# kscalelabs/kbot-joystick

Hardware: AMD Instinct MI355X
Metric: env-steps/sec (whole node), K-Bot joystick 8192 envs @1/2/4/8 MI355X (higher is better)
Workload: dtype f32; 1 GPU; kbot-headless, 8192 envs/GPU, flat ground, fixed joystick command (0.5,0,0), full iteration: 100-step rollout + PPO update (batch 512/GPU, 3 passes, LSTM hidden 256, depth 2); envs_per_gpu=8192, rollout_steps=100, batch_size_per_gpu=512, num_passes=3, hidden_size=256, deterministic_update=True, parallelism=env-sharded dp1, grad all-reduce per optimizer step

## Files before the change

kbot-joystick_amd/csrc/kbj_ctx.h:

```cpp
#pragma once
#include <hip/hip_runtime.h>
#include <string>
#include <vector>
#include <cstdio>
#include "kbj.h"

struct KbjKernelRec { int kind; double flops; hipEvent_t a, b; };
enum { KBJ_KIND_GEMM = 0 , KBJ_KIND_SEQ_FWD = 8, KBJ_KIND_SEQ_BWD = 9, KBJ_KIND_ENV_STEP = 10, KBJ_KIND_SEQ_FWD_FUSED = 11, KBJ_KIND_SEQ_FWD_OBS = 12, KBJ_KIND_LSTM_STEP = 13, KBJ_KIND_LSTM_STEP_OBS = 14,
       KBJ_KIND_GEMM_X3 = 15, KBJ_KIND_GEMM_X3_GEN = 19, KBJ_KIND_GEMM_X3_SMALL = 20, KBJ_KIND_GEMM_X3_SMALL_GEN = 21,
       KBJ_KIND_SEQ_BWD16 = 22 , KBJ_KIND_GEMM_64x128 = 23 ,
       KBJ_KIND_COUNT = 25 };
inline int kbj_kind_gemm_x3(int tm, bool a_kc, bool b_kc, bool gen) {
  if (tm == 2) return gen ? KBJ_KIND_GEMM_X3_GEN : KBJ_KIND_GEMM_X3 + (a_kc ? 2 : 0) + (b_kc ? 1 : 0);
  return gen ? KBJ_KIND_GEMM_X3_SMALL_GEN : KBJ_KIND_GEMM_X3_SMALL;
}

struct Sched {
  bool fold_actor = true;
  bool fold_critic = true;
  bool fuse_ih = true;
  bool fuse_obs = true;
  bool fused_critic_head = true;
  bool rollout_step = true;
  bool one_stream = false;
  bool debug_sync = false;
  bool deterministic = false;
  bool bwd16 = true;
  bool critic_on_caller = true;
  bool gemm_x3 = false;
};

struct KbjSettings {
  Sched sched;
  int seq_timeout_ms = 0;
  int seq_drop = 0, seq_drop_bwd = 0;
  bool seq_stamps = false; int stamp_sel = 1;
  bool seq_bstamps = false; int bstamp_sel = 0;
};

KbjSettings kbj_read_settings(const kbj_config& cfg);

struct kbj_ctx {
  int device = 0;
  hipStream_t stream = nullptr;
  hipStream_t stream2 = nullptr;
  hipEvent_t ev_fork = nullptr, ev_join = nullptr;
  hipStream_t side[2] = {nullptr, nullptr};
  hipEvent_t ev_dx[2] = {nullptr, nullptr};
  hipEvent_t ev_side[2] = {nullptr, nullptr};
  hipEvent_t ev_obs = nullptr;
  hipEvent_t ev_prefetch = nullptr;
  hipEvent_t ev_small = nullptr;
  hipEvent_t ev_actor_grad = nullptr;
  hipEvent_t ev_pool[32] = {};
  int ev_next = 0;
  kbj_model model_h;
  kbj_config cfg_h;
  KbjSettings set;
  kbj_model* model_d = nullptr;
  kbj_config* cfg_d = nullptr;
  void* pc_d = nullptr;
  float* mc_d = nullptr;
  float* ep_d = nullptr;
  float* es_d = nullptr;
  float* rcarry_d = nullptr;
  uint32_t seed = 0;
  int rollout_argmax = 0;
  float* qstate_next = nullptr;
  double* epst_part_d = nullptr;
  int epst_part_blocks = 0;
  void* nn_ws = nullptr;
  size_t nn_ws_bytes = 0;
  bool profiling = false;
  hipEvent_t ev0 = nullptr, ev1 = nullptr;
  float env_ms = 0, nn_ms = 0;
  int env_launches = 0, nn_launches = 0;
  std::vector<KbjKernelRec> krecs;
  kbj_kernel_stat kstats[KBJ_KIND_COUNT];
  std::string error;
};

extern thread_local std::string kbj_global_error;

inline int kbj_fail(kbj_ctx* ctx, const std::string& msg) {
  if (ctx) ctx->error = msg;
  kbj_global_error = msg;
  return -1;
}

#define KBJ_HIP(ctx, call)                                                                                   \
  do {                                                                                                       \
    hipError_t e_ = (call);                                                                                  \
    if (e_ != hipSuccess) return kbj_fail(ctx, std::string(#call) + ": " + hipGetErrorString(e_));           \
  } while (0)

#define KBJ_CHECK_LAUNCH(ctx, name)                                                                          \
  do {                                                                                                       \
    hipError_t e_ = hipGetLastError();                                                                       \
    if (e_ != hipSuccess) return kbj_fail(ctx, std::string("launch ") + name + ": " + hipGetErrorString(e_)); \
  } while (0)

extern thread_local kbj_ctx* kbj_prof_ctx;

struct KbjKernelTimer {
  kbj_ctx* c; hipStream_t s; hipEvent_t b = nullptr;
  KbjKernelTimer(hipStream_t st, int kind, double flops) : c(kbj_prof_ctx), s(st) {
    if (!c) return;
    hipEvent_t a;
    if (hipEventCreate(&a) != hipSuccess || hipEventCreate(&b) != hipSuccess) { c = nullptr; return; }
    c->krecs.push_back(KbjKernelRec{kind, flops, a, b});
    hipEventRecord(a, s);
  }
  ~KbjKernelTimer() { if (c) hipEventRecord(b, s); }
};

struct KbjTimed {
  kbj_ctx* ctx; bool nn;
  KbjTimed(kbj_ctx* c, bool is_nn) : ctx(c), nn(is_nn) { if (ctx->profiling) hipEventRecord(ctx->ev0, ctx->stream); }
  ~KbjTimed() {
    if (!ctx->profiling) return;
    hipEventRecord(ctx->ev1, ctx->stream);
    hipEventSynchronize(ctx->ev1);
    float ms = 0; hipEventElapsedTime(&ms, ctx->ev0, ctx->ev1);
    if (nn) { ctx->nn_ms += ms; ctx->nn_launches++; } else { ctx->env_ms += ms; ctx->env_launches++; }
  }
};
```

kbot-joystick_amd/csrc/kbj_lstm_bwd16.h:

```cpp
#pragma once
#include "kbj_lstm_seq.h"

namespace kbj {

constexpr int BWD16_ROWS = 16, BWD16_UNITS = 64, BWD16_NTH = 512;
#ifndef KBJ_BWD16_OWN_SPLIT
#define KBJ_BWD16_OWN_SPLIT 4
#endif

template <int H>
__global__ __launch_bounds__(BWD16_NTH) void lstm_seq_bwd16_kernel(SeqBwdArgs a) {
  static_assert(H % 64 == 0 && H >= 64 && H <= 256, "16 x 64 tiles: hidden sizes 64, 128, 192, 256");
  constexpr int NTH = BWD16_NTH, ROWS = BWD16_ROWS, UNITS = BWD16_UNITS;
  constexpr int NUG = H / UNITS;
  constexpr int KC = 4 * UNITS;
  constexpr int LDC = KC + 8;
  constexpr int KHALF = KC / 2, KS = KHALF / 4;
  typedef SeqK<KHALF> KK;
  __shared__ __attribute__((aligned(16))) float cbuf[2][ROWS * LDC];
  __shared__ float pbuf[2][ROWS][UNITS + 4];
  __shared__ int flag;
  const int tid = threadIdx.x, lane = tid & 63, wave = tid >> 6, nt = wave & 3, kh = wave >> 2;
  const int nblk = gridDim.x;
  const int lid = (nblk % 8 == 0) ? (int)(blockIdx.x % 8) * (nblk / 8) + (int)(blockIdx.x / 8) : (int)blockIdx.x;
  const int ug = lid % NUG, rg = lid / NUG;
  const int r0 = rg * ROWS, u0 = ug * UNITS;
  const int B = a.B, T = a.T;
  if (seq_aborted(a.err, &flag)) return;
  float wreg[NUG][KS];
#pragma unroll
  for (int j = 0; j < NUG; ++j) {
    const int p = (ug + j) % NUG;
#pragma unroll
    for (int s = 0; s < KS; ++s) {
      const int kl = KHALF * kh + KK::kidx(s, lane >> 4);
      wreg[j][s] = a.Whh[(size_t)((kl / UNITS) * H + UNITS * p + (kl % UNITS)) * H + u0 + 16 * nt + (lane & 15)];
    }
  }
  int erow[2], eunit[2];
#pragma unroll
  for (int i = 0; i < 2; ++i) { const int e = tid + NTH * i; erow[i] = e / UNITS; eunit[i] = e % UNITS; }
  float dcm[2] = {0.0f, 0.0f};
  float bsum[2][4] = {{0, 0, 0, 0}, {0, 0, 0, 0}};
  float actn[2][4], tcn[2], cprevn[2], dhan[2], kpn[2];
  int rcl[2];
#pragma unroll
  for (int i = 0; i < 2; ++i) { const int r = r0 + erow[i]; rcl[i] = r < B ? r : 0; }
  auto fetch_inputs = [&](int tt) {
    const int tq = tt < 0 ? 0 : tt;
#pragma unroll
    for (int i = 0; i < 2; ++i) {
      const size_t o1 = ((size_t)tq * B + rcl[i]) * H + u0 + eunit[i];
      const float* g = a.Gact + ((size_t)tq * B + rcl[i]) * 4 * H + u0 + eunit[i];
#pragma unroll
      for (int k = 0; k < 4; ++k) actn[i][k] = g[k * H];
      tcn[i] = a.TanhC[o1];
      cprevn[i] = a.Cm[o1];
      dhan[i] = a.dHabove[o1];
      kpn[i] = a.keep[(size_t)tq * B + rcl[i]];
    }
  };
  fetch_inputs(T - 1);
  struct Chunk { f32x4m v[2]; };
  auto chunk_load = [&](Chunk& c, const float* src, int p) {
    __amdgpu_buffer_rsrc_t rsrc = __builtin_amdgcn_make_buffer_rsrc(const_cast<float*>(src), 0, 0x7FFFFFFF, 0x00020000);
#pragma unroll
    for (int i = 0; i < 2; ++i) {
      const int q = tid + NTH * i, row = q >> 6, seg = q & 63, r = r0 + row;
      const unsigned off = (unsigned)(((size_t)(r < B ? r : 0) * 4 * H + (size_t)(seg >> 4) * H + UNITS * p + 4 * (seg & 15)) * sizeof(float));
      c.v[i] = __builtin_bit_cast(f32x4m, __builtin_amdgcn_raw_buffer_load_b128(rsrc, off, 0, 16));
    }
  };
  auto chunk_to_lds = [&](const Chunk& c, float* buf) {
#pragma unroll
    for (int i = 0; i < 2; ++i) {
      const int q = tid + NTH * i, row = q >> 6, seg = q & 63;
      *reinterpret_cast<f32x4m*>(buf + row * LDC + UNITS * (seg >> 4) + 4 * (seg & 15)) = c.v[i];
    }
  };
  auto mma = [&](const float* buf, const float* w, f32x4m& acc0, f32x4m& acc1, int jb, int je) {
    const float* p0 = buf + (lane & 15) * LDC + KHALF * kh + 4 * (lane >> 4);
#pragma unroll
    for (int j = jb; j < je; ++j) {
      const f32x4m f = *reinterpret_cast<const f32x4m*>(p0 + 16 * j);
      acc0 = __builtin_amdgcn_mfma_f32_16x16x4f32(f[0], w[4 * j + 0], acc0, 0, 0, 0);
      acc1 = __builtin_amdgcn_mfma_f32_16x16x4f32(f[1], w[4 * j + 1], acc1, 0, 0, 0);
      acc0 = __builtin_amdgcn_mfma_f32_16x16x4f32(f[2], w[4 * j + 2], acc0, 0, 0, 0);
      acc1 = __builtin_amdgcn_mfma_f32_16x16x4f32(f[3], w[4 * j + 3], acc1, 0, 0, 0);
    }
  };
  constexpr int OWN_SPLIT = NUG > 1 ? KBJ_BWD16_OWN_SPLIT : KK::NB;
  for (int t = T - 1; t >= 0; --t) {
    float dhm[2] = {0.0f, 0.0f};
    float act[2][4], tc[2], cprev[2], dha[2], kp[2];
    auto prefetch = [&]() {
#pragma unroll
      for (int i = 0; i < 2; ++i) { tc[i] = tcn[i]; cprev[i] = cprevn[i]; dha[i] = dhan[i]; kp[i] = kpn[i]; for (int k = 0; k < 4; ++k) act[i][k] = actn[i][k]; }
      fetch_inputs(t - 1);
    };
    if (t == T - 1) prefetch();
    else {
      f32x4m acc0 = {0, 0, 0, 0}, acc1 = {0, 0, 0, 0};
      mma(cbuf[0], wreg[0], acc0, acc1, 0, OWN_SPLIT);
      Chunk ch[NUG > 1 ? NUG - 1 : 1];
      if (NUG > 1) {
        if (!seq_wait(a.counters + rg * NUG, NUG, (unsigned)(T - 1 - t), a.err, &flag, a.timeout_ticks)) return;
        const float* src = a.dG + (size_t)(t + 1) * B * 4 * H;
#pragma unroll
        for (int j = 1; j < NUG; ++j) chunk_load(ch[j - 1], src, (ug + j) % NUG);
        __builtin_amdgcn_sched_barrier(0);
      }
      mma(cbuf[0], wreg[0], acc0, acc1, OWN_SPLIT, KK::NB);
      if (NUG == 1) prefetch();
#pragma unroll
      for (int j = 1; j < NUG; ++j) {
        float* buf = cbuf[j & 1];
        chunk_to_lds(ch[j - 1], buf);
        if (j == NUG - 1) prefetch();
        __syncthreads();
        mma(buf, wreg[j], acc0, acc1, 0, KK::NB);
      }
#pragma unroll
      for (int r = 0; r < 4; ++r) pbuf[kh][(lane >> 4) * 4 + r][16 * nt + (lane & 15)] = acc0[r] + acc1[r];
      __syncthreads();
#pragma unroll
      for (int i = 0; i < 2; ++i) dhm[i] = pbuf[0][erow[i]][eunit[i]] + pbuf[1][erow[i]][eunit[i]];
    }
#pragma unroll
    for (int i = 0; i < 2; ++i) {
      const int r = r0 + erow[i];
      const float ig = act[i][0], fg = act[i][1], gg = act[i][2], og = act[i][3];
      const float dh = dha[i] + kp[i] * dhm[i];
      const float dc = kp[i] * dcm[i] + dh * og * (1 - tc[i] * tc[i]);
      const float d0 = dc * gg * ig * (1 - ig), d1 = dc * cprev[i] * fg * (1 - fg), d2 = dc * ig * (1 - gg * gg), d3 = dh * tc[i] * og * (1 - og);
      float* own = cbuf[0] + erow[i] * LDC + eunit[i];
      own[0] = d0; own[UNITS] = d1; own[2 * UNITS] = d2; own[3 * UNITS] = d3;
      if (r < B) {
        float* dg = a.dG + ((size_t)t * B + r) * 4 * H + u0 + eunit[i];
        seq_store(dg, d0); seq_store(dg + H, d1); seq_store(dg + 2 * H, d2); seq_store(dg + 3 * H, d3);
        bsum[i][0] += d0; bsum[i][1] += d1; bsum[i][2] += d2; bsum[i][3] += d3;
      }
      dcm[i] = dc * fg;
    }
    seq_publish(a.counters + rg * NUG + ug, (unsigned)(T - t));
  }
  if (a.db || a.db_part) {
    __syncthreads();
#pragma unroll
    for (int i = 0; i < 2; ++i)
#pragma unroll
      for (int k = 0; k < 4; ++k) cbuf[0][erow[i] * LDC + k * UNITS + eunit[i]] = bsum[i][k];
    __syncthreads();
    if (tid < KC) {
      const int k = tid / UNITS, u = tid % UNITS;
      float s = 0;
      for (int r = 0; r < ROWS; ++r) s += cbuf[0][r * LDC + tid];
      if (a.db_part) a.db_part[(size_t)rg * 4 * H + k * H + u0 + u] = s;
      else atomicAdd(a.db + k * H + u0 + u, s);
    }
  }
}

}
```

kbot-joystick_amd/csrc/kbj_lstm_seq.h:

```cpp
#pragma once
#include <hip/hip_runtime.h>
#include <stdint.h>

namespace kbj {

typedef float f32x4m __attribute__((ext_vector_type(4)));

constexpr int SEQ_ROWS = 32;
constexpr int SEQ_UNITS = 16;
#ifdef KBJ_SEQ_BSTAMPS_BUILD
#define SEQ_BSTAMP(k) do { if (a.stamps && blockIdx.x == 0 && tid == 0) a.stamps[t * 10 + (k)] = clock64(); } while (0)
#define SEQ_BSTAMP_ON 1
#else
#define SEQ_BSTAMP(k) do { } while (0)
#define SEQ_BSTAMP_ON 0
#endif
constexpr unsigned SEQ_TIMEOUT_MS = 2000;

#ifndef KBJ_SEQ_BWD_NUM_VGPR
#define KBJ_SEQ_BWD_NUM_VGPR 88
#endif

struct SeqFwdArgs {
  float* G;
  const float* Whh;
  float* Hm;
  float* Cm;
  float* Hout;
  float* TanhC;
  const float* keep;
  unsigned* counters;
  unsigned* err;
  int T, B;
  long long* stamps;
  unsigned timeout_ticks = SEQ_TIMEOUT_MS * 100000u;
  const float* X = nullptr;
  const float* Wih = nullptr;
  const float* bias = nullptr;
  int ldx = 0, ldw = 0;
  int kx = 0;
};

struct SeqBwdArgs {
  const float* Gact;
  const float* TanhC;
  const float* Cm;
  const float* dHabove;
  const float* keep;
  const float* Whh;
  float* dG;
  unsigned* counters;
  unsigned* err;
  int T, B;
  float* db;
  float* db_part = nullptr;
  unsigned timeout_ticks = SEQ_TIMEOUT_MS * 100000u;
  long long* stamps = nullptr;
};

__device__ __forceinline__ float seq_sigmoid(float x) { return __builtin_amdgcn_rcpf(1.0f + __expf(-x)); }
__device__ __forceinline__ float seq_tanh(float x) { float xc = fminf(fmaxf(x, -15.0f), 15.0f); return 1.0f - 2.0f * __builtin_amdgcn_rcpf(1.0f + __expf(2.0f * xc)); }

__device__ __forceinline__ bool seq_wait(unsigned* flags, int nflags, unsigned target, unsigned* err, int* lds_flag, unsigned timeout_ticks) {
#ifdef KBJ_EXPERIMENT_NOWAIT
  __syncthreads();
  return true;
#endif
  if (threadIdx.x < 64) {
    unsigned spins = 0;
    unsigned long long t0 = 0;
    int ok = 1;
    const int l = threadIdx.x;
    for (;;) {
      bool mine = l >= nflags || __hip_atomic_load(flags + l, __ATOMIC_RELAXED, __HIP_MEMORY_SCOPE_AGENT) >= target;
      if (__all(mine)) break;
      __builtin_amdgcn_s_sleep(1);
      if ((++spins & 255u) == 0) {
        const unsigned long long now = wall_clock64();
        if (t0 == 0) t0 = now;
        const bool aborted = __hip_atomic_load(err, __ATOMIC_RELAXED, __HIP_MEMORY_SCOPE_AGENT) != 0;
        if (aborted || now - t0 > timeout_ticks) { ok = 0; if (l == 0) __hip_atomic_store(err, 1u, __ATOMIC_RELAXED, __HIP_MEMORY_SCOPE_AGENT); break; }
      }
    }
    if (l == 0) *lds_flag = ok;
  }
  __syncthreads();
  __builtin_amdgcn_fence(__ATOMIC_ACQUIRE, "wavefront");
  return *lds_flag != 0;
}
__device__ __forceinline__ bool seq_aborted(unsigned* err, int* lds_flag) {
  if (threadIdx.x == 0) *lds_flag = __hip_atomic_load(err, __ATOMIC_RELAXED, __HIP_MEMORY_SCOPE_AGENT) != 0;
  __syncthreads();
  const bool r = *lds_flag != 0;
  __syncthreads();
  return r;
}
__device__ __forceinline__ void seq_store(float* p, float v) { __hip_atomic_store(p, v, __ATOMIC_RELAXED, __HIP_MEMORY_SCOPE_AGENT); }
__device__ __forceinline__ void seq_publish(unsigned* my_flag, unsigned steps_done) {
#ifndef KBJ_EXPERIMENT_NODRAIN
  asm volatile("s_waitcnt vmcnt(0)" ::: "memory");
#endif
  __syncthreads();
  if (threadIdx.x == 0) __hip_atomic_store(my_flag, steps_done, __ATOMIC_RELAXED, __HIP_MEMORY_SCOPE_AGENT);
}
template <int K> struct SeqK {
  static_assert(K % 4 == 0, "row width must be a multiple of 4");
  static constexpr int NB = K / 16, REM = (K % 16) / 4, STEPS = 4 * NB + REM;
  static constexpr int LD = (K + 7) / 16 * 16 + 8;
  __host__ __device__ static constexpr int kidx(int s, int g) { return s < 4 * NB ? 16 * (s / 4) + 4 * g + (s % 4) : 16 * NB + 4 * (s - 4 * NB) + g; }
  template <bool TAIL>
  __device__ static __forceinline__ void mma(const float* lds, int lane, const float* w, f32x4m& acc0, f32x4m& acc1, int jb, int je) {
    const float* p0 = lds + (lane & 15) * LD + 4 * (lane >> 4);
    const float* p1 = p0 + 16 * LD;
#pragma unroll
    for (int j = jb; j < je; ++j) {
      const f32x4m a0 = *reinterpret_cast<const f32x4m*>(p0 + 16 * j), a1 = *reinterpret_cast<const f32x4m*>(p1 + 16 * j);
#pragma unroll
      for (int q = 0; q < 4; ++q) {
        acc0 = __builtin_amdgcn_mfma_f32_16x16x4f32(a0[q], w[4 * j + q], acc0, 0, 0, 0);
        acc1 = __builtin_amdgcn_mfma_f32_16x16x4f32(a1[q], w[4 * j + q], acc1, 0, 0, 0);
      }
    }
    if (TAIL) {
      const float* r0 = lds + (lane & 15) * LD + 16 * NB + (lane >> 4);
      const float* r1 = r0 + 16 * LD;
#pragma unroll
      for (int q = 0; q < REM; ++q) {
        acc0 = __builtin_amdgcn_mfma_f32_16x16x4f32(r0[4 * q], w[4 * NB + q], acc0, 0, 0, 0);
        acc1 = __builtin_amdgcn_mfma_f32_16x16x4f32(r1[4 * q], w[4 * NB + q], acc1, 0, 0, 0);
      }
    }
  }
};

template <int H, int NTH> struct SeqTile {
  static constexpr int NQ = SEQ_ROWS * (H / 4);
  static constexpr int NV = (NQ + NTH - 1) / NTH;
  static constexpr bool EXACT = NQ % NTH == 0;
  f32x4m v[NV];
  __device__ __forceinline__ void load(const float* src, int ld, int r0, int B) {
    typedef unsigned u32x4 __attribute__((ext_vector_type(4)));
    __amdgpu_buffer_rsrc_t rsrc = __builtin_amdgcn_make_buffer_rsrc(const_cast<float*>(src), 0, 0x7FFFFFFF, 0x00020000);
#pragma unroll
    for (int i = 0; i < NV; ++i) {
      int q = threadIdx.x + NTH * i, row = q / (H / 4), c4 = q % (H / 4), r = r0 + row;
      unsigned off = (unsigned)(((size_t)(r < B ? r : 0) * ld + 4 * c4) * sizeof(float));
      u32x4 u = __builtin_amdgcn_raw_buffer_load_b128(rsrc, off, 0, 16);
      v[i] = __builtin_bit_cast(f32x4m, u);
    }
  }
  __device__ __forceinline__ void load_plain(const float* src, int ld, int r0, int B) {
#pragma unroll
    for (int i = 0; i < NV; ++i) {
      int q = threadIdx.x + NTH * i;
      if (!EXACT && q >= NQ) q = 0;
      int row = q / (H / 4), c4 = q % (H / 4), r = r0 + row;
      v[i] = *reinterpret_cast<const f32x4m*>(src + (size_t)(r < B ? r : 0) * ld + 4 * c4);
    }
  }
  __device__ __forceinline__ void to_lds(float* lds, int r0, int B) const {
    if (r0 + SEQ_ROWS <= B) {
#pragma unroll
      for (int i = 0; i < NV; ++i) {
        int q = threadIdx.x + NTH * i, row = q / (H / 4), c4 = q % (H / 4);
        if (!EXACT && q >= NQ) continue;
        *reinterpret_cast<f32x4m*>(lds + row * SeqK<H>::LD + 4 * c4) = v[i];
      }
      return;
    }
#pragma unroll
    for (int i = 0; i < NV; ++i) {
      int q = threadIdx.x + NTH * i, row = q / (H / 4), c4 = q % (H / 4);
      if (!EXACT && q >= NQ) continue;
      *reinterpret_cast<f32x4m*>(lds + row * SeqK<H>::LD + 4 * c4) = r0 + row < B ? v[i] : f32x4m{0, 0, 0, 0};
    }
  }
  __device__ __forceinline__ void to_lds_cols(float* lds, int ldl, int r0, int B, int ncol) const {
#pragma unroll
    for (int i = 0; i < NV; ++i) {
      int q = threadIdx.x + NTH * i, row = q / (H / 4), c4 = q % (H / 4);
      if (!EXACT && q >= NQ) continue;
      f32x4m x = v[i];
#pragma unroll
      for (int j = 0; j < 4; ++j) if (r0 + row >= B || 4 * c4 + j >= ncol) x[j] = 0.0f;
      *reinterpret_cast<f32x4m*>(lds + row * ldl + 4 * c4) = x;
    }
  }
};

template <int H, int UW, bool FUSE = false, int KX = H>
__global__ __launch_bounds__(256 * UW) void lstm_seq_fwd_kernel(SeqFwdArgs a) {
  constexpr int NTH = 256 * UW, UNITS = SEQ_UNITS * UW;
  typedef SeqK<H> KH;
  typedef SeqK<KX> KXK;
  constexpr int LDH = KH::LD, KXS = KXK::STEPS, LDX = KXK::LD;
  constexpr int NUG = H / UNITS;
#ifndef KBJ_SEQ_XSPLIT_NUM
#define KBJ_SEQ_XSPLIT_NUM 4
#endif
  constexpr int XSPLIT = KXK::NB * KBJ_SEQ_XSPLIT_NUM / 8;
  __shared__ __attribute__((aligned(16))) float hs[SEQ_ROWS * LDH];
  __shared__ __attribute__((aligned(16))) float xs[FUSE ? SEQ_ROWS * LDX : 4];
  __shared__ float gbuf[4][SEQ_ROWS][UNITS + 4];
  __shared__ int flag;
  const int tid = threadIdx.x, lane = tid & 63, gate = (tid >> 6) & 3, uh = tid >> 8;
  const int nblk = gridDim.x;
  const int lid = (nblk % 8 == 0) ? (int)(blockIdx.x % 8) * (nblk / 8) + (int)(blockIdx.x / 8) : (int)blockIdx.x;
  const int ug = lid % NUG, rg = lid / NUG;
  const int r0 = rg * SEQ_ROWS, u0 = ug * UNITS;
  const int B = a.B, T = a.T;
  if (seq_aborted(a.err, &flag)) return;
  float wreg[H / 4];
  {
    const float* wrow = a.Whh + (size_t)(gate * H + u0 + SEQ_UNITS * uh + (lane & 15)) * H;
#pragma unroll
    for (int s = 0; s < H / 4; ++s) wreg[s] = wrow[KH::kidx(s, lane >> 4)];
  }
  float wxreg[FUSE ? KXS : 1];
  float bias_col = 0.0f;
  const int ldx = a.ldx ? a.ldx : H, kxv = a.kx ? a.kx : KX;
  if (FUSE) {
    const int grow = gate * H + u0 + SEQ_UNITS * uh + (lane & 15);
    const float* wrow = a.Wih + (size_t)grow * (a.ldw ? a.ldw : H);
#pragma unroll
    for (int s = 0; s < KXS; ++s) { const int k = KXK::kidx(s, lane >> 4); wxreg[s] = k < kxv ? wrow[k] : 0.0f; }
    bias_col = a.bias[grow];
  }
  int erow[2], eunit[2];
  float cm[2];
#pragma unroll
  for (int i = 0; i < 2; ++i) {
    int e = tid + NTH * i;
    erow[i] = e / UNITS; eunit[i] = e % UNITS;
    int r = r0 + erow[i];
    cm[i] = r < B ? a.Cm[(size_t)r * H + u0 + eunit[i]] : 0.0f;
  }
  float ig[2], fg[2], gg[2], og[2], tc[2], hh[2];
#ifdef KBJ_SEQ_BSTAMPS_BUILD
#define SEQ_STAMP(k) do { if (a.stamps && blockIdx.x == 0 && tid == 0) a.stamps[t * 6 + (k)] = clock64(); } while (0)
#else
#define SEQ_STAMP(k) do { } while (0)
#endif
  float gxn[2][4], kpn[2];
  int rcl[2];
#pragma unroll
  for (int i = 0; i < 2; ++i) { const int r = r0 + erow[i]; rcl[i] = r < B ? r : 0; }
  auto fetch_inputs = [&](int tt) {
    const int tq = tt < T ? tt : T - 1;
#pragma unroll
    for (int i = 0; i < 2; ++i) {
      if (!FUSE) {
        const float* g = a.G + ((size_t)tq * B + rcl[i]) * 4 * H + u0 + eunit[i];
#pragma unroll
        for (int k = 0; k < 4; ++k) gxn[i][k] = g[k * H];
      } else {
#pragma unroll
        for (int k = 0; k < 4; ++k) gxn[i][k] = 0.0f;
      }
      kpn[i] = a.keep[(size_t)tq * B + rcl[i]];
    }
  };
  fetch_inputs(0);
  if (FUSE) {
    SeqTile<KX, NTH> xt;
    xt.load_plain(a.X, ldx, r0, B);
    if (KX == H) xt.to_lds(xs, r0, B); else xt.to_lds_cols(xs, LDX, r0, B, kxv);
    __syncthreads();
  }
  for (int t = 0; t < T; ++t) {
    SEQ_STAMP(0);
    float gx[2][4], kp[2];
#pragma unroll
    for (int i = 0; i < 2; ++i) { kp[i] = kpn[i]; for (int k = 0; k < 4; ++k) gx[i][k] = gxn[i][k]; }
    f32x4m acc0 = {bias_col, bias_col, bias_col, bias_col}, acc1 = acc0;
    if (FUSE) {
      KXK::template mma<false>(xs, lane, wxreg, acc0, acc1, 0, XSPLIT);
    }
    if (t > 0) { if (!seq_wait(a.counters + rg * NUG, NUG, (unsigned)t, a.err, &flag, a.timeout_ticks)) return; }
    SEQ_STAMP(1);
    SeqTile<H, NTH> tile;
    tile.load(a.Hm + (size_t)t * B * H, H, r0, B);
    if (FUSE) {
      __builtin_amdgcn_sched_barrier(0);
      KXK::template mma<true>(xs, lane, wxreg, acc0, acc1, XSPLIT, KXK::NB);
      __builtin_amdgcn_sched_barrier(0);
    }
    tile.to_lds(hs, r0, B);
    fetch_inputs(t + 1);
    if (t > 0) {
#pragma unroll
      for (int i = 0; i < 2; ++i) {
        int r = r0 + erow[i];
        if (r >= B) continue;
        size_t o1 = ((size_t)(t - 1) * B + r) * H + u0 + eunit[i];
        float* g = a.G + ((size_t)(t - 1) * B + r) * 4 * H + u0 + eunit[i];
        g[0] = ig[i]; g[H] = fg[i]; g[2 * H] = gg[i]; g[3 * H] = og[i];
        a.Hout[o1] = hh[i]; a.TanhC[o1] = tc[i];
        a.Cm[o1 + (size_t)B * H] = cm[i];
      }
    }
    SeqTile<KX, NTH> xt;
    if (FUSE && t + 1 < T) xt.load_plain(a.X + (size_t)(t + 1) * B * ldx, ldx, r0, B);
    __syncthreads();
    SEQ_STAMP(2);
    KH::template mma<false>(hs, lane, wreg, acc0, acc1, 0, KH::NB);
#pragma unroll
    for (int r = 0; r < 4; ++r) {
      gbuf[gate][(lane >> 4) * 4 + r][SEQ_UNITS * uh + (lane & 15)] = acc0[r];
      gbuf[gate][16 + (lane >> 4) * 4 + r][SEQ_UNITS * uh + (lane & 15)] = acc1[r];
    }
    if (FUSE && t + 1 < T) { if (KX == H) xt.to_lds(xs, r0, B); else xt.to_lds_cols(xs, LDX, r0, B, kxv); }
    __syncthreads();
    SEQ_STAMP(3);
#pragma unroll
    for (int i = 0; i < 2; ++i) {
      int row = erow[i], u = eunit[i];
      ig[i] = seq_sigmoid(gbuf[0][row][u] + gx[i][0]); fg[i] = seq_sigmoid(gbuf[1][row][u] + gx[i][1]);
      gg[i] = seq_tanh(gbuf[2][row][u] + gx[i][2]); og[i] = seq_sigmoid(gbuf[3][row][u] + gx[i][3]);
      float c = fg[i] * cm[i] + ig[i] * gg[i];
      tc[i] = seq_tanh(c); hh[i] = og[i] * tc[i];
      cm[i] = c * kp[i];
      if (r0 + row < B) seq_store(a.Hm + ((size_t)(t + 1) * B + r0 + row) * H + u0 + u, hh[i] * kp[i]);
    }
    SEQ_STAMP(4);
    seq_publish(a.counters + rg * NUG + ug, (unsigned)(t + 1));
    SEQ_STAMP(5);
  }
#pragma unroll
  for (int i = 0; i < 2; ++i) {
    int r = r0 + erow[i];
    if (r >= B) continue;
    size_t o1 = ((size_t)(T - 1) * B + r) * H + u0 + eunit[i];
    float* g = a.G + ((size_t)(T - 1) * B + r) * 4 * H + u0 + eunit[i];
    g[0] = ig[i]; g[H] = fg[i]; g[2 * H] = gg[i]; g[3 * H] = og[i];
    a.Hout[o1] = hh[i]; a.TanhC[o1] = tc[i];
    a.Cm[o1 + (size_t)B * H] = cm[i];
  }
}

template <int H, int UW>
__device__ __forceinline__ void lstm_seq_bwd_body(const SeqBwdArgs a) {
  constexpr int NTH = 256 * UW, UNITS = SEQ_UNITS * UW;
  typedef SeqK<H> KH;
  constexpr int LDH = KH::LD;
  constexpr int NUG = H / UNITS;
  __shared__ __attribute__((aligned(16))) float ds[SEQ_ROWS * LDH];
  __shared__ float pbuf[4][SEQ_ROWS][UNITS + 4];
  __shared__ int flag;
  const int tid = threadIdx.x, lane = tid & 63, wave = (tid >> 6) & 3, uh = tid >> 8;
  const int nblk = gridDim.x;
  const int lid = (nblk % 8 == 0) ? (int)(blockIdx.x % 8) * (nblk / 8) + (int)(blockIdx.x / 8) : (int)blockIdx.x;
  const int ug = lid % NUG, rg = lid / NUG;
  const int r0 = rg * SEQ_ROWS, u0 = ug * UNITS;
  const int B = a.B, T = a.T;
  if (seq_aborted(a.err, &flag)) return;
  if (SEQ_BSTAMP_ON && a.stamps && tid == 0 && blockIdx.x < 256) a.stamps[T * 10 + 3 * blockIdx.x] = wall_clock64();
  constexpr int KW = H / 4;
  constexpr int KS = KW / 4;
  typedef SeqK<KW> KWK;
  static_assert(KW % 16 == 0, "the backward recurrence fetches its fragments in 16-k blocks");
  float wreg[4][KS];
#pragma unroll
  for (int c = 0; c < 4; ++c)
#pragma unroll
    for (int s = 0; s < KS; ++s) wreg[c][s] = a.Whh[(size_t)(c * H + wave * KW + KWK::kidx(s, lane >> 4)) * H + u0 + SEQ_UNITS * uh + (lane & 15)];
  int erow[2], eunit[2];
  float dcm[2] = {0.0f, 0.0f};
  float bsum[2][4] = {{0, 0, 0, 0}, {0, 0, 0, 0}};
#pragma unroll
  for (int i = 0; i < 2; ++i) { int e = tid + NTH * i; erow[i] = e / UNITS; eunit[i] = e % UNITS; }
  float actn[2][4], tcn[2], cprevn[2], dhan[2], kpn[2];
  auto fetch_inputs = [&](int tt) {
#pragma unroll
    for (int i = 0; i < 2; ++i) {
      int r = r0 + erow[i];
      bool ok = r < B && tt >= 0;
      size_t o1 = ((size_t)(ok ? tt : 0) * B + (ok ? r : 0)) * H + u0 + eunit[i];
      const float* g = a.Gact + ((size_t)(ok ? tt : 0) * B + (ok ? r : 0)) * 4 * H + u0 + eunit[i];
#pragma unroll
      for (int k = 0; k < 4; ++k) actn[i][k] = ok ? g[k * H] : 0.0f;
      tcn[i] = ok ? a.TanhC[o1] : 0.0f;
      cprevn[i] = ok ? a.Cm[o1] : 0.0f;
      dhan[i] = ok ? a.dHabove[o1] : 0.0f;
      kpn[i] = ok ? a.keep[(size_t)tt * B + r] : 0.0f;
    }
  };
  fetch_inputs(T - 1);
  if (SEQ_BSTAMP_ON && a.stamps && tid == 0 && blockIdx.x < 256) a.stamps[T * 10 + 3 * blockIdx.x + 1] = wall_clock64();
  for (int t = T - 1; t >= 0; --t) {
    const bool last = t == T - 1;
    SEQ_BSTAMP(0);
    if (SEQ_BSTAMP_ON && a.stamps && blockIdx.x == 0 && tid == 0) a.stamps[t * 10 + 9] = wall_clock64();
    float dhm[2] = {0.0f, 0.0f};
    float act[2][4], tc[2], cprev[2], dha[2], kp[2];
    auto prefetch = [&]() {
#pragma unroll
      for (int i = 0; i < 2; ++i) { tc[i] = tcn[i]; cprev[i] = cprevn[i]; dha[i] = dhan[i]; kp[i] = kpn[i]; for (int k = 0; k < 4; ++k) act[i][k] = actn[i][k]; }
      fetch_inputs(t - 1);
    };
    if (last) prefetch();
    else {
      if (!seq_wait(a.counters + rg * NUG, NUG, (unsigned)(T - 1 - t), a.err, &flag, a.timeout_ticks)) return;
      SEQ_BSTAMP(1);
      f32x4m acc0 = {0, 0, 0, 0}, acc1 = {0, 0, 0, 0};
      const float* src = a.dG + (size_t)(t + 1) * B * 4 * H;
      SeqTile<H, NTH> tile;
      tile.load(src, 4 * H, r0, B);
#pragma unroll
      for (int c = 0; c < 4; ++c) {
        float* buf = ds;
        if (c) __syncthreads();
        tile.to_lds(buf, r0, B);
        if (c < 3) tile.load(src + (c + 1) * H, 4 * H, r0, B);
        else prefetch();
        __syncthreads();
        SEQ_BSTAMP(2 + c);
        const float* a0p = buf + (lane & 15) * LDH + wave * KW + 4 * (lane >> 4);
        const float* a1p = a0p + 16 * LDH;
#pragma unroll
        for (int j = 0; j < KW / 16; ++j) {
          const f32x4m f0 = *reinterpret_cast<const f32x4m*>(a0p + 16 * j), f1 = *reinterpret_cast<const f32x4m*>(a1p + 16 * j);
#pragma unroll
          for (int q = 0; q < 4; ++q) {
            acc0 = __builtin_amdgcn_mfma_f32_16x16x4f32(f0[q], wreg[c][4 * j + q], acc0, 0, 0, 0);
            acc1 = __builtin_amdgcn_mfma_f32_16x16x4f32(f1[q], wreg[c][4 * j + q], acc1, 0, 0, 0);
          }
        }
      }
#pragma unroll
      for (int r = 0; r < 4; ++r) {
        pbuf[wave][(lane >> 4) * 4 + r][SEQ_UNITS * uh + (lane & 15)] = acc0[r];
        pbuf[wave][16 + (lane >> 4) * 4 + r][SEQ_UNITS * uh + (lane & 15)] = acc1[r];
      }
      __syncthreads();
      SEQ_BSTAMP(6);
#pragma unroll
      for (int i = 0; i < 2; ++i) dhm[i] = pbuf[0][erow[i]][eunit[i]] + pbuf[1][erow[i]][eunit[i]] + pbuf[2][erow[i]][eunit[i]] + pbuf[3][erow[i]][eunit[i]];
    }
#pragma unroll
    for (int i = 0; i < 2; ++i) {
      int r = r0 + erow[i];
      if (r >= B) continue;
      float ig = act[i][0], fg = act[i][1], gg = act[i][2], og = act[i][3];
      float dh = dha[i] + kp[i] * dhm[i];
      float dc = kp[i] * dcm[i] + dh * og * (1 - tc[i] * tc[i]);
      float* dg = a.dG + ((size_t)t * B + r) * 4 * H + u0 + eunit[i];
      float d0 = dc * gg * ig * (1 - ig), d1 = dc * cprev[i] * fg * (1 - fg), d2 = dc * ig * (1 - gg * gg), d3 = dh * tc[i] * og * (1 - og);
      seq_store(dg, d0);
      seq_store(dg + H, d1);
      seq_store(dg + 2 * H, d2);
      seq_store(dg + 3 * H, d3);
      bsum[i][0] += d0; bsum[i][1] += d1; bsum[i][2] += d2; bsum[i][3] += d3;
      dcm[i] = dc * fg;
    }
    SEQ_BSTAMP(7);
    seq_publish(a.counters + rg * NUG + ug, (unsigned)(T - t));
    SEQ_BSTAMP(8);
  }
  if (a.db || a.db_part) {
    __syncthreads();
#pragma unroll
    for (int k = 0; k < 4; ++k) {
      pbuf[k][erow[0]][eunit[0]] = bsum[0][k];
      pbuf[k][erow[1]][eunit[1]] = bsum[1][k];
    }
    __syncthreads();
    if (tid < 4 * UNITS) {
      int k = tid / UNITS, u = tid % UNITS;
      float s = 0;
      for (int r = 0; r < SEQ_ROWS; ++r) s += pbuf[k][r][u];
      if (a.db_part) a.db_part[(size_t)rg * 4 * H + k * H + u0 + u] = s;
      else atomicAdd(a.db + k * H + u0 + u, s);
    }
  }
  if (SEQ_BSTAMP_ON && a.stamps && tid == 0 && blockIdx.x < 256) a.stamps[T * 10 + 3 * blockIdx.x + 2] = wall_clock64();
}
template <int H, int UW>
__global__ __launch_bounds__(256 * UW) __attribute__((amdgpu_num_vgpr(KBJ_SEQ_BWD_NUM_VGPR))) void lstm_seq_bwd_kernel(SeqBwdArgs a) { lstm_seq_bwd_body<H, UW>(a); }
template <int H, int UW>
__global__ __launch_bounds__(256 * UW) void lstm_seq_bwd_wide_kernel(SeqBwdArgs a) { lstm_seq_bwd_body<H, UW>(a); }

struct StepArgs {
  const float* X; int ldx, kx;
  const float* Wih; int ldw;
  const float* Whh;
  const float* bias;
  const float* Hin;
  float* Hout;
  float* C;
  int M;
};
template <int H, int UW, int KX = H>
__global__ __launch_bounds__(256 * UW) void lstm_step_kernel(StepArgs a) {
  constexpr int NTH = 256 * UW, UNITS = SEQ_UNITS * UW;
  typedef SeqK<H> KH;
  typedef SeqK<KX> KXK;
  constexpr int LDH = KH::LD, KXS = KXK::STEPS, LDX = KXK::LD, NUG = H / UNITS;
  __shared__ __attribute__((aligned(16))) float hs[SEQ_ROWS * LDH];
  __shared__ __attribute__((aligned(16))) float xs[SEQ_ROWS * LDX];
  __shared__ float gbuf[4][SEQ_ROWS][UNITS + 4];
  const int tid = threadIdx.x, lane = tid & 63, gate = (tid >> 6) & 3, uh = tid >> 8;
  const int ug = blockIdx.x % NUG, chunk = blockIdx.x / NUG, nchunk = gridDim.x / NUG;
  const int u0 = ug * UNITS, M = a.M, nrg = (M + SEQ_ROWS - 1) / SEQ_ROWS;
  const int kxv = a.kx ? a.kx : KX;
  const int grow = gate * H + u0 + SEQ_UNITS * uh + (lane & 15);
  float wreg[H / 4], wxreg[KXS];
  {
    const float* wrow = a.Whh + (size_t)grow * H + 4 * (lane >> 4);
#pragma unroll
    for (int j = 0; j < KH::NB; ++j) {
      const f32x4m q = *reinterpret_cast<const f32x4m*>(wrow + 16 * j);
#pragma unroll
      for (int e = 0; e < 4; ++e) wreg[4 * j + e] = q[e];
    }
    const float* xrow = a.Wih + (size_t)grow * a.ldw;
    if (a.kx == 0 && (a.ldw & 3) == 0) {
#pragma unroll
      for (int j = 0; j < KXK::NB; ++j) {
        const f32x4m q = *reinterpret_cast<const f32x4m*>(xrow + 4 * (lane >> 4) + 16 * j);
#pragma unroll
        for (int e = 0; e < 4; ++e) wxreg[4 * j + e] = q[e];
      }
#pragma unroll
      for (int s = 4 * KXK::NB; s < KXS; ++s) wxreg[s] = xrow[KXK::kidx(s, lane >> 4)];
    } else {
#pragma unroll
      for (int s = 0; s < KXS; ++s) { const int k = KXK::kidx(s, lane >> 4); wxreg[s] = k < kxv ? xrow[k] : 0.0f; }
    }
  }
  const float bias_col = a.bias[grow];
  int erow[2], eunit[2];
#pragma unroll
  for (int i = 0; i < 2; ++i) { int e = tid + NTH * i; erow[i] = e / UNITS; eunit[i] = e % UNITS; }
  SeqTile<KX, NTH> xt;
  SeqTile<H, NTH> ht;
  float cn[2] = {0.0f, 0.0f};
  auto fetch = [&](int rg) {
    const int r0 = rg * SEQ_ROWS;
    xt.load_plain(a.X, a.ldx, r0, M);
    ht.load_plain(a.Hin, H, r0, M);
#pragma unroll
    for (int i = 0; i < 2; ++i) { int r = r0 + erow[i]; cn[i] = r < M ? a.C[(size_t)r * H + u0 + eunit[i]] : 0.0f; }
  };
  int rg = chunk;
  if (rg < nrg) fetch(rg);
  for (; rg < nrg; rg += nchunk) {
    const int r0 = rg * SEQ_ROWS;
    if (KX == H) xt.to_lds(xs, r0, M); else xt.to_lds_cols(xs, LDX, r0, M, kxv);
    ht.to_lds(hs, r0, M);
    const float cp[2] = {cn[0], cn[1]};
    __syncthreads();
    if (rg + nchunk < nrg) fetch(rg + nchunk);
    f32x4m acc0 = {bias_col, bias_col, bias_col, bias_col}, acc1 = acc0;
    KXK::template mma<true>(xs, lane, wxreg, acc0, acc1, 0, KXK::NB);
    KH::template mma<false>(hs, lane, wreg, acc0, acc1, 0, KH::NB);
#pragma unroll
    for (int r = 0; r < 4; ++r) {
      gbuf[gate][(lane >> 4) * 4 + r][SEQ_UNITS * uh + (lane & 15)] = acc0[r];
      gbuf[gate][16 + (lane >> 4) * 4 + r][SEQ_UNITS * uh + (lane & 15)] = acc1[r];
    }
    __syncthreads();
#pragma unroll
    for (int i = 0; i < 2; ++i) {
      const int row = erow[i], u = eunit[i], r = r0 + row;
      float ig = seq_sigmoid(gbuf[0][row][u]), fg = seq_sigmoid(gbuf[1][row][u]), gg = seq_tanh(gbuf[2][row][u]), og = seq_sigmoid(gbuf[3][row][u]);
      float c = fg * cp[i] + ig * gg;
      if (r < M) { a.Hout[(size_t)r * H + u0 + u] = og * seq_tanh(c); a.C[(size_t)r * H + u0 + u] = c; }
    }
  }
}

}
```

kbot-joystick_amd/csrc/kbj_nn.hip:

```cpp
#include <hip/hip_runtime.h>
#include <vector>
#include <cmath>
#include <cstdlib>
#include <algorithm>
#include <type_traits>
#include "kbj_ctx.h"
#include "kbj_gemm.h"
#include "kbj_nn_kernels.h"
#include "kbj_lstm_seq.h"
#include "kbj_lstm_bwd16.h"

using namespace kbj;

namespace {

constexpr int MAXD = KBJ_MAX_DEPTH;

struct NetOff {
  size_t w_in, b_in, w_ih[MAXD], w_hh[MAXD], b[MAXD], w_out, b_out;
  int nin, nout, ld_obs;
};

struct TrainBufs {
  float *obs, *X0, *G[MAXD], *Hm[MAXD], *Hout[MAXD], *Cm[MAXD], *TanhC[MAXD], *Out, *dOut, *dHa, *dHb, *dGl[MAXD];
};

struct ParamLayout {
  NetOff net[2];
  size_t nparams = 0, nactor = 0;
  int D = 2;
};

struct NnWs : ParamLayout {
  Sched& sched;
  explicit NnWs(Sched& s) : sched(s) {}
  int H = 0, N = 0, B = 0, T = 0;
  int Hu = 0;
  ParamLayout user;
  PadDesc* pad_desc = nullptr; int npad = 0;
  float *pparams = nullptr, *pgrad = nullptr;
  float *phc[4] = {nullptr, nullptr, nullptr, nullptr}, *pc0[4] = {nullptr, nullptr, nullptr, nullptr};
  bool padded() const { return Hu != H; }
  float* skws[4] = {nullptr, nullptr, nullptr, nullptr};
  size_t skws_cap[4] = {0, 0, 0, 0};
  float* detp[4] = {nullptr, nullptr, nullptr, nullptr};
  double* detd = nullptr;
  float *rX[4] = {nullptr, nullptr, nullptr, nullptr}, *rG[4] = {nullptr, nullptr, nullptr, nullptr}, *rOut[4] = {nullptr, nullptr, nullptr, nullptr};
  float* joint_bias_d = nullptr;
  bool mirror = false;
  int nnets = 2;
  MirrorEntry* mtab[2] = {nullptr, nullptr};
  float *rObsM[2] = {nullptr, nullptr};
  float* rH[4][MAXD] = {};
  float* tail_hc = nullptr;
  float *y_m = nullptr, *sd_m = nullptr, *value_m = nullptr, *lpf0_m = nullptr, *dy = nullptr, *dy_m = nullptr, *dvalue_m = nullptr, *zeroR = nullptr;
  TrainBufs tb[4];
  float *keep = nullptr, *act = nullptr, *logp_old = nullptr, *val_old = nullptr, *adv = nullptr, *target = nullptr;
  float *y = nullptr, *sd = nullptr, *logp = nullptr, *ent = nullptr, *value = nullptr, *dlogp = nullptr, *dvalue = nullptr, *lpf0 = nullptr;
  float *Weff = nullptr, *beff = nullptr, *Zeff[4] = {nullptr, nullptr, nullptr, nullptr};
  float* WinP[2] = {nullptr, nullptr};
  double* stats = nullptr;
  const int32_t* prefetched_idx = nullptr;
  const kbj_traj* prefetched_traj = nullptr;
  const double* ext_adv_sums = nullptr;
  unsigned* seq_counters = nullptr;
  unsigned* seq_err = nullptr;
  unsigned seq_timeout_ticks = 0;
  bool counters_clean = false;
  bool sumsq_clean = false;
  int seq_grid = 0, seq_slots = 0;
  long long* seq_stamps = nullptr;
  long long* seq_bstamps = nullptr;
  std::vector<void*> allocs;
};

NnWs* ws_of(kbj_ctx* ctx) { return reinterpret_cast<NnWs*>(ctx->nn_ws); }

ParamLayout layout_params(const kbj_config& c, int H) {
  ParamLayout p;
  const int D = p.D = c.depth;
  size_t off = 0;
  for (int n = 0; n < 2; ++n) {
    NetOff& o = p.net[n];
    o.nin = n == 0 ? KBJ_NOBS_ACTOR + c.extra_obs_actor : KBJ_NOBS_CRITIC + c.extra_obs_critic;
    o.ld_obs = KBJ_LD_OF(o.nin);
    o.nout = n == 0 ? 2 * KBJ_NU : 1;
    o.w_in = off; off += (size_t)H * o.nin;
    o.b_in = off; off += H;
    for (int l = 0; l < D; ++l) {
      o.w_ih[l] = off; off += (size_t)4 * H * H;
      o.w_hh[l] = off; off += (size_t)4 * H * H;
      o.b[l] = off; off += (size_t)4 * H;
    }
    o.w_out = off; off += (size_t)o.nout * H;
    o.b_out = off; off += o.nout;
    if (n == 0) p.nactor = off;
  }
  p.nparams = off;
  return p;
}

template <class C> auto& carry_hc(C& c, int n) { return n == 0 ? c.actor_hc_d : n == 1 ? c.critic_hc_d : n == 2 ? c.actor_mirror_hc_d : c.critic_mirror_hc_d; }
template <class T> auto& traj_carry0(T& t, int n) { return n == 0 ? t.carry0_actor_hc_d : n == 1 ? t.carry0_critic_hc_d : n == 2 ? t.carry0_actor_mirror_hc_d : t.carry0_critic_mirror_hc_d; }

void build_mirror_tables(const kbj_model& m, std::vector<MirrorEntry>& ta, std::vector<MirrorEntry>& tc, int extra_actor = 0, int extra_critic = 0) {
  auto swp = [](int i) { return i < 5 ? i + 5 : (i < 10 ? i - 5 : i); };
  tc.assign(KBJ_LD_CRITIC, MirrorEntry{0, 0.0f, 0.0f});
  for (int k = 0; k < KBJ_LD_CRITIC; ++k) tc[k].src = k;
  auto keep = [&](int k, float sgn) { tc[k] = MirrorEntry{k, sgn, 0.0f}; };
  for (int i = 0; i < KBJ_NU; ++i) {
    int s = swp(i);
    auto rng = [&](int j) { return std::fmax(m.joint_bias[j] - m.joint_lo[j], m.joint_hi[j] - m.joint_bias[j]); };
    tc[KBJ_OBS_JPOS + i] = MirrorEntry{KBJ_OBS_JPOS + s, -rng(s) / rng(i), (-m.joint_bias[s] - m.joint_bias[i]) / rng(i)};
    tc[KBJ_OBS_JVEL + i] = MirrorEntry{KBJ_OBS_JVEL + s, -1.0f, 0.0f};
    tc[KBJ_OBS_ACTFRC + i] = MirrorEntry{KBJ_OBS_ACTFRC + s, -1.0f, 0.0f};
  }
  keep(KBJ_OBS_PG, -1); keep(KBJ_OBS_PG + 1, 1); keep(KBJ_OBS_PG + 2, 1); keep(KBJ_OBS_PG + 3, -1); keep(KBJ_OBS_PG + 4, 1);
  keep(KBJ_OBS_GYRO, -1); keep(KBJ_OBS_GYRO + 1, 1); keep(KBJ_OBS_GYRO + 2, -1);
  keep(KBJ_OBS_ZEROCMD, 1);
  const float cs[16] = {1, -1, -1, 1, -1, 1, -1, -1, -1, -1, -1, -1, -1, -1, -1, -1};
  for (int k = 0; k < 16; ++k) keep(KBJ_OBS_CMD + k, cs[k]);
  ta.assign(tc.begin(), tc.begin() + KBJ_LD_ACTOR);
  for (int k = KBJ_NOBS_ACTOR; k < KBJ_LD_ACTOR; ++k) ta[k] = MirrorEntry{k, 0.0f, 0.0f};
  tc[KBJ_OBS_TOUCH] = MirrorEntry{KBJ_OBS_TOUCH + 1, 1, 0}; tc[KBJ_OBS_TOUCH + 1] = MirrorEntry{KBJ_OBS_TOUCH, 1, 0};
  const float fs[3] = {1, -1, 1};
  for (int k = 0; k < 3; ++k) { tc[KBJ_OBS_FEETPOS + k] = MirrorEntry{KBJ_OBS_FEETPOS + 3 + k, fs[k], 0}; tc[KBJ_OBS_FEETPOS + 3 + k] = MirrorEntry{KBJ_OBS_FEETPOS + k, fs[k], 0}; }
  keep(KBJ_OBS_BASEPOS, 1); keep(KBJ_OBS_BASEPOS + 1, 1); keep(KBJ_OBS_BASEPOS + 2, 1);
  keep(KBJ_OBS_BASEQUAT, 1); keep(KBJ_OBS_BASEQUAT + 1, -1); keep(KBJ_OBS_BASEQUAT + 2, -1); keep(KBJ_OBS_BASEQUAT + 3, 1);
  const float ci[10] = {1, 1, -1, 1, 1, 1, 1, -1, 1, -1}, cv[6] = {1, -1, 1, -1, 1, -1};
  for (int b = 0; b < 23; ++b) {
    for (int k = 0; k < 10; ++k) keep(KBJ_OBS_CINERT + 10 * b + k, ci[k]);
    for (int k = 0; k < 6; ++k) keep(KBJ_OBS_CVEL + 6 * b + k, cv[k]);
  }
  keep(KBJ_OBS_LINVEL, 1); keep(KBJ_OBS_LINVEL + 1, -1); keep(KBJ_OBS_LINVEL + 2, 1);
  keep(KBJ_OBS_ANGVEL, -1); keep(KBJ_OBS_ANGVEL + 1, 1); keep(KBJ_OBS_ANGVEL + 2, -1);
  keep(KBJ_OBS_HEIGHT, 1);
  for (int k = KBJ_NOBS_CRITIC; k < KBJ_LD_CRITIC; ++k) tc[k] = MirrorEntry{k, 0.0f, 0.0f};
  auto widen = [](std::vector<MirrorEntry>& t, int nobs, int extra) {
    t.resize(KBJ_LD_OF(nobs + extra));
    for (int k = nobs; k < (int)t.size(); ++k) t[k] = MirrorEntry{k, k < nobs + extra ? 1.0f : 0.0f, 0.0f};
  };
  if (extra_actor > 0) widen(ta, KBJ_NOBS_ACTOR, extra_actor);
  if (extra_critic > 0) widen(tc, KBJ_NOBS_CRITIC, extra_critic);
}

template <class T> int dalloc(kbj_ctx* ctx, NnWs& w, T** p, size_t count) {
  void* q = nullptr;
  hipError_t e = hipMalloc(&q, count * sizeof(T));
  if (e != hipSuccess) return kbj_fail(ctx, std::string("hipMalloc (nn workspace): ") + hipGetErrorString(e));
  w.allocs.push_back(q);
  *p = reinterpret_cast<T*>(q);
  return 0;
}

constexpr int g_fold_sk = 8;
#ifndef KBJ_SPLITK_WGS
#define KBJ_SPLITK_WGS 768
#endif
constexpr int g_splitk_wgs = KBJ_SPLITK_WGS;
constexpr int DETP_ROWS = 512, DETP_COLS = 4 * 512;

int lane_of(kbj_ctx* ctx, hipStream_t s) { return s == ctx->stream ? 0 : (s == ctx->stream2 ? 1 : (s == ctx->side[0] ? 2 : 3)); }
float* sk_workspace(kbj_ctx* ctx, hipStream_t s, size_t floats) {
  NnWs& w = *ws_of(ctx);
  if (!w.sched.deterministic) return nullptr;
  const int l = lane_of(ctx, s);
  if (w.skws_cap[l] < floats) {
    hipDeviceSynchronize();
    if (w.skws[l]) hipFree(w.skws[l]);
    w.skws[l] = nullptr; w.skws_cap[l] = 0;
    void* q = nullptr;
    if (hipMalloc(&q, floats * sizeof(float)) != hipSuccess) { kbj_fail(ctx, "hipMalloc (deterministic split-K workspace)"); return nullptr; }
    w.skws[l] = reinterpret_cast<float*>(q); w.skws_cap[l] = floats;
  }
  return w.skws[l];
}
float* det_partials(kbj_ctx* ctx, hipStream_t s) {
  NnWs& w = *ws_of(ctx);
  return w.sched.deterministic ? w.detp[lane_of(ctx, s)] : nullptr;
}

inline dim3 g1(size_t n, int bs = 256) { return dim3((unsigned)((n + bs - 1) / bs)); }

void linear_fwd(hipStream_t s, const float* x, int lda, const float* W, int ldw, const float* bias, float* y, int ldy, int M, int N, int K, int beta) {
  GemmArgs g{x, W, y, bias, M, N, K, lda, ldw, ldy, beta, 1, nullptr};
  gemm_launch<true, true>(s, g);
}
void linear_bwd_input(hipStream_t s, bool x3, const float* dy, int lddy, const float* W, int ldw, float* dx, int lddx, int M, int N, int K, int beta, int tile = -1) {
  GemmArgs g{dy, W, dx, nullptr, M, N, K, lddy, ldw, lddx, beta, 1, nullptr};
  g.x3 = x3;
  gemm_launch<true, false>(s, g, x3 ? -1 : tile);
}
void linear_bwd_weight(kbj_ctx* ctx, hipStream_t s, bool x3, const float* dy, int lddy, const float* x, int ldx, float* dW, int lddw, int Nout, int Nin, int R) {
  bool big = Nout >= 128 && Nin >= 128;
  int ts = big ? 128 : 64;
  int tiles = ((Nout + ts - 1) / ts) * ((Nin + ts - 1) / ts);
  int sk = std::max(2, std::min(256, g_splitk_wgs / std::max(1, tiles)));
  sk = std::max(2, std::min(sk, (R + 255) / 256));
  GemmArgs g{dy, x, dW, nullptr, Nout, Nin, R, lddy, ldx, lddw, 1, sk, nullptr};
  g.skws = sk_workspace(ctx, s, (size_t)sk * Nout * Nin);
  g.x3 = x3;
  gemm_launch<false, false>(s, g, big ? 1 : 0);
}

void linear_bwd_weight2(kbj_ctx* ctx, hipStream_t s, bool x3, const float* dy, int lddy, const float* x1, const float* x2, int ldx, float* dW1, float* dW2, int lddw, int Nout, int Nin, int R) {
  bool big = Nout >= 128 && Nin >= 128;
  int ts = big ? 128 : 64;
  if (Nin % ts != 0) {
    linear_bwd_weight(ctx, s, x3, dy, lddy, x1, ldx, dW1, lddw, Nout, Nin, R);
    linear_bwd_weight(ctx, s, x3, dy, lddy, x2, ldx, dW2, lddw, Nout, Nin, R);
    return;
  }
  int tiles = ((Nout + ts - 1) / ts) * (2 * Nin / ts);
  int sk = std::max(2, std::min(256, g_splitk_wgs / std::max(1, tiles)));
  sk = std::max(2, std::min(sk, (R + 255) / 256));
  GemmArgs g{dy, x1, dW1, nullptr, Nout, 2 * Nin, R, lddy, ldx, lddw, 1, sk, nullptr};
  g.B2 = x2; g.C2 = dW2; g.n1 = Nin;
  g.skws = sk_workspace(ctx, s, (size_t)sk * Nout * 2 * Nin);
  g.x3 = x3;
  gemm_launch<false, false>(s, g, big ? 1 : 0);
}
void colsum_acc(kbj_ctx* ctx, hipStream_t s, const float* X, int M, int N, int ld, float* out) {
  float* part = det_partials(ctx, s);
  hipLaunchKernelGGL(colsum_kernel, dim3((N + 63) / 64, DETP_ROWS), dim3(256), 0, s, X, M, N, ld, out, part);
  if (part) reduce_rows_launch(s, part, DETP_ROWS, N, out);
}

constexpr int SEQ_UW = 2;
constexpr int SEQ_FUSED_MAX_H = 256;
constexpr int SEQ_MAX_H = 512;
constexpr int SEQ_COUNTER_WORDS = 256;
constexpr int SEQ_COUNTER_TOTAL = 2 * MAXD * 4 * SEQ_COUNTER_WORDS;

template <int HC = 64, class F> bool dispatch_hidden(int H, F&& f) {
  if constexpr (HC > SEQ_MAX_H) return false;
  else return H == HC ? f(std::integral_constant<int, HC>()) : dispatch_hidden<HC + 64>(H, f);
}

int seq_fwd(kbj_ctx* ctx, hipStream_t st, int H, const SeqFwdArgs& a0) {
  SeqFwdArgs a = a0;
  a.timeout_ticks = ws_of(ctx)->seq_timeout_ticks;
  KbjKernelTimer timer(st, a.X ? (a.ldx == KBJ_LD_ACTOR ? KBJ_KIND_SEQ_FWD_OBS : KBJ_KIND_SEQ_FWD_FUSED) : KBJ_KIND_SEQ_FWD, 2.0 * a.T * a.B * 4.0 * H * (H + (a.X ? (a.kx ? a.kx : H) : 0)));
  const bool built = dispatch_hidden(H, [&](auto hc) {
    constexpr int HC = decltype(hc)::value, UW = SEQ_UW;
    int grid = (HC / (SEQ_UNITS * UW)) * ((a.B + SEQ_ROWS - 1) / SEQ_ROWS);
    if (ctx->set.seq_drop > 0 && grid > 1) { --ctx->set.seq_drop; --grid; }
    const dim3 block(256 * UW);
    if constexpr (HC <= SEQ_FUSED_MAX_H) {
      if (a.X && a.ldx == KBJ_LD_ACTOR) { hipLaunchKernelGGL((lstm_seq_fwd_kernel<HC, UW, true, KBJ_LD_ACTOR>), dim3(grid), block, 0, st, a); return true; }
      if (a.X) { hipLaunchKernelGGL((lstm_seq_fwd_kernel<HC, UW, true>), dim3(grid), block, 0, st, a); return true; }
    }
    hipLaunchKernelGGL((lstm_seq_fwd_kernel<HC, UW, false>), dim3(grid), block, 0, st, a);
    return true;
  });
  return built ? 0 : kbj_fail(ctx, "seq_fwd: the persistent LSTM kernels are built for hidden sizes 64, 128, ..., 512");
}
int seq_bwd_row_groups(int B, bool tiles16) { return tiles16 ? (B + BWD16_ROWS - 1) / BWD16_ROWS : (B + SEQ_ROWS - 1) / SEQ_ROWS; }
int seq_bwd(kbj_ctx* ctx, hipStream_t st, int H, const SeqBwdArgs& a0, bool tiles16 = false) {
  SeqBwdArgs a = a0;
  a.timeout_ticks = ws_of(ctx)->seq_timeout_ticks;
  KbjKernelTimer timer(st, tiles16 ? KBJ_KIND_SEQ_BWD16 : KBJ_KIND_SEQ_BWD, 2.0 * a.T * a.B * 4.0 * H * H);
  const bool built = dispatch_hidden(H, [&](auto hc) {
    constexpr int HC = decltype(hc)::value, UW = SEQ_UW;
    if (tiles16) {
      if constexpr (HC <= SEQ_FUSED_MAX_H) {
        int grid = (HC / BWD16_UNITS) * ((a.B + BWD16_ROWS - 1) / BWD16_ROWS);
        if (ctx->set.seq_drop_bwd > 0 && grid > 1 && HC > BWD16_UNITS) { --ctx->set.seq_drop_bwd; --grid; }
        hipLaunchKernelGGL((lstm_seq_bwd16_kernel<HC>), dim3(grid), dim3(BWD16_NTH), 0, st, a);
        return true;
      } else return false;
    }
    const dim3 grid((HC / (SEQ_UNITS * UW)) * ((a.B + SEQ_ROWS - 1) / SEQ_ROWS)), block(256 * UW);
    if constexpr (HC <= SEQ_FUSED_MAX_H) hipLaunchKernelGGL((lstm_seq_bwd_kernel<HC, UW>), grid, block, 0, st, a);
    else hipLaunchKernelGGL((lstm_seq_bwd_wide_kernel<HC, UW>), grid, block, 0, st, a);
    return true;
  });
  return built ? 0 : kbj_fail(ctx, "seq_bwd: the persistent LSTM kernels are built for hidden sizes 64, 128, ..., 512 (lstm_seq_bwd16_kernel: up to 256)");
}

template <int H> hipError_t seq_min_blocks_per_cu(int* out) {
  constexpr int threads = 256 * SEQ_UW;
  int n[4] = {0, 0, 0, 0};
  hipError_t e = hipOccupancyMaxActiveBlocksPerMultiprocessor(&n[2], lstm_seq_fwd_kernel<H, SEQ_UW, false, H>, threads, 0);
  if constexpr (H <= SEQ_FUSED_MAX_H) {
    if (e == hipSuccess) e = hipOccupancyMaxActiveBlocksPerMultiprocessor(&n[0], lstm_seq_fwd_kernel<H, SEQ_UW, true, H>, threads, 0);
    if (e == hipSuccess) e = hipOccupancyMaxActiveBlocksPerMultiprocessor(&n[1], lstm_seq_fwd_kernel<H, SEQ_UW, true, KBJ_LD_ACTOR>, threads, 0);
    if (e == hipSuccess) e = hipOccupancyMaxActiveBlocksPerMultiprocessor(&n[3], lstm_seq_bwd_kernel<H, SEQ_UW>, threads, 0);
    int n16 = 0;
    if (e == hipSuccess) e = hipOccupancyMaxActiveBlocksPerMultiprocessor(&n16, lstm_seq_bwd16_kernel<H>, BWD16_NTH, 0);
    n[3] = std::min(n[3], n16);
  } else {
    if (e == hipSuccess) e = hipOccupancyMaxActiveBlocksPerMultiprocessor(&n[3], lstm_seq_bwd_wide_kernel<H, SEQ_UW>, threads, 0);
    n[0] = n[1] = n[2];
  }
  *out = std::min(std::min(n[0], n[1]), std::min(n[2], n[3]));
  return e;
}

int lstm_step(kbj_ctx* ctx, hipStream_t st, int H, const StepArgs& a) {
  const bool obs = a.ldx == KBJ_LD_ACTOR && a.ldw == KBJ_LD_ACTOR;
  KbjKernelTimer timer(st, obs ? KBJ_KIND_LSTM_STEP_OBS : KBJ_KIND_LSTM_STEP, 2.0 * a.M * 4.0 * H * (H + (a.kx ? a.kx : H)));
  const int nug = H / (SEQ_UNITS * 2), nrg = (a.M + SEQ_ROWS - 1) / SEQ_ROWS;
  const int nch = std::max(1, std::min(nrg, 256 / nug));
  dim3 grid(nug * nch), block(512);
  const bool built = dispatch_hidden(H, [&](auto hc) {
    constexpr int HC = decltype(hc)::value;
    if constexpr (HC <= SEQ_FUSED_MAX_H) {
      if (obs) hipLaunchKernelGGL((lstm_step_kernel<HC, 2, KBJ_LD_ACTOR>), grid, block, 0, st, a);
      else hipLaunchKernelGGL((lstm_step_kernel<HC, 2>), grid, block, 0, st, a);
      return true;
    } else return false;
  });
  return built ? 0 : kbj_fail(ctx, "lstm_step: the LSTM step kernels are built for hidden_size 64, 128, 192, 256");
}

}

int kbj_nn_check_errors(kbj_ctx* ctx) {
  NnWs* w = ws_of(ctx);
  if (!w) return 0;
  if (w->seq_stamps) {
    std::vector<long long> st((size_t)w->T * 6);
    if (hipMemcpy(st.data(), w->seq_stamps, st.size() * sizeof(long long), hipMemcpyDeviceToHost) == hipSuccess && w->T > 2) {
      double d[6] = {0, 0, 0, 0, 0, 0};
      for (int t = 1; t < w->T - 1; ++t) { for (int k = 0; k < 5; ++k) d[k] += (double)(st[t * 6 + k + 1] - st[t * 6 + k]); d[5] += (double)(st[(t + 1) * 6] - st[t * 6 + 5]); }
      fprintf(stderr, "[kbj seq_fwd stamps, cycles/step] prefetch+wait %.0f stage %.0f mfma %.0f cell %.0f publish %.0f bulk-store %.0f\n",
              d[0] / (w->T - 2), d[1] / (w->T - 2), d[2] / (w->T - 2), d[3] / (w->T - 2), d[4] / (w->T - 2), d[5] / (w->T - 2));
    }
  }
  if (w->seq_bstamps) {
    std::vector<long long> st((size_t)w->T * 10 + 768);
    if (hipMemcpy(st.data(), w->seq_bstamps, st.size() * sizeof(long long), hipMemcpyDeviceToHost) == hipSuccess && w->T > 3) {
      double d[9] = {0, 0, 0, 0, 0, 0, 0, 0, 0};
      int cnt = 0;
      for (int t = w->T - 3; t >= 1; --t, ++cnt) { for (int k = 0; k < 8; ++k) d[k] += (double)(st[t * 10 + k + 1] - st[t * 10 + k]); d[8] += (double)(st[(t - 1) * 10] - st[t * 10 + 8]); }
      fprintf(stderr, "[kbj seq_bwd stamps, cycles/step] wait %.0f chunk0-staged %.0f chunk1 %.0f chunk2 %.0f chunk3 %.0f last-mfma+reduce %.0f cell %.0f publish %.0f loop %.0f\n",
              d[0] / cnt, d[1] / cnt, d[2] / cnt, d[3] / cnt, d[4] / cnt, d[5] / cnt, d[6] / cnt, d[7] / cnt, d[8] / cnt);
      double ticks = (double)(st[1 * 10] - st[(w->T - 3) * 10]), wall = (double)(st[1 * 10 + 9] - st[(w->T - 3) * 10 + 9]);
      int wall_khz = 0;
      hipDeviceGetAttribute(&wall_khz, hipDeviceAttributeWallClockRate, ctx->device);
      if (wall_khz > 0) {
        const long long* g = st.data() + (size_t)w->T * 10;
        int nwg = ((w->B + SEQ_ROWS - 1) / SEQ_ROWS) * (w->H / (SEQ_UNITS * SEQ_UW));
        if (nwg > 256) nwg = 256;
        long long e0 = g[0], e1 = g[0], l1 = g[1], x0 = g[2], x1 = g[2];
        for (int i = 1; i < nwg; ++i) { e0 = std::min(e0, g[3 * i]); e1 = std::max(e1, g[3 * i]); l1 = std::max(l1, g[3 * i + 1]); x0 = std::min(x0, g[3 * i + 2]); x1 = std::max(x1, g[3 * i + 2]); }
        const double us = 1e3 / wall_khz;
        fprintf(stderr, "[kbj seq_bwd stamps] %d workgroups: last entry +%.1f us, last loop start +%.1f us, first exit +%.1f us, last exit +%.1f us (from the first entry)\n", nwg,
                (e1 - e0) * us, (l1 - e0) * us, (x0 - e0) * us, (x1 - e0) * us);
      }
      if (wall > 0 && wall_khz > 0) fprintf(stderr, "[kbj seq_bwd stamps] %.2f us/step, stamp counter at %.0f MHz\n", wall / wall_khz * 1e3 / cnt, ticks / wall * wall_khz * 1e-3);
    }
  }
  unsigned e[2] = {0, 0};
  if (hipMemcpy(e, w->seq_err, sizeof(e), hipMemcpyDeviceToHost) != hipSuccess) return kbj_fail(ctx, "hipMemcpy seq_err");
  if (e[0] || e[1]) {
    hipMemset(w->seq_err, 0, sizeof(e));
    if (e[0]) return kbj_fail(ctx, "persistent LSTM kernel: inter-workgroup wait timed out (grid not fully resident?); the optimizer steps fed by it were skipped");
    return kbj_fail(ctx, "non-finite gradient norm: the optimizer step was skipped (parameters and moments unchanged)");
  }
  return 0;
}

void kbj_nn_drop_prefetch(kbj_ctx* ctx) {
  NnWs* w = ws_of(ctx);
  if (!w || !w->prefetched_idx) return;
  hipStreamWaitEvent(ctx->stream, ctx->ev_prefetch, 0);
  w->prefetched_idx = nullptr; w->prefetched_traj = nullptr;
}

KbjSettings kbj_read_settings(const kbj_config& c) {
  auto flag = [](const char* name, bool dflt) { const char* v = getenv(name); return v ? atoi(v) != 0 : dflt; };
  auto number = [](const char* name, int dflt) { const char* v = getenv(name); return v ? atoi(v) : dflt; };
  KbjSettings set;
  Sched& sc = set.sched;
  const bool wide = c.hidden_size > SEQ_FUSED_MAX_H;
  sc.fold_actor = flag("KBJ_FOLD_ACTOR", true); sc.fold_critic = flag("KBJ_FOLD_CRITIC", true);
  sc.fuse_ih = flag("KBJ_SEQ_FUSE", true); sc.fuse_obs = sc.fuse_ih && flag("KBJ_SEQ_FUSE_OBS", true);
  sc.fused_critic_head = flag("KBJ_FUSED_CRITIC_HEAD", true); sc.rollout_step = flag("KBJ_ROLLOUT_STEP", true);
  sc.one_stream = flag("KBJ_ONE_STREAM", false); sc.debug_sync = flag("KBJ_DEBUG", false);
  sc.deterministic = c.deterministic != 0 || flag("KBJ_DETERMINISTIC", false);
  { const char* cl = getenv("KBJ_CRITIC_LANE"); sc.critic_on_caller = !(cl && std::string(cl) == "2nd"); }
  sc.bwd16 = flag("KBJ_BWD16", true) && !wide;
  sc.gemm_x3 = (c.gemm_bf16x3 != 0 || flag("KBJ_GEMM_X3", false)) && !sc.deterministic;
  if (wide) sc.fuse_ih = sc.fuse_obs = sc.rollout_step = false;
  set.seq_drop = number("KBJ_DEBUG_DROP_SEQ_WG", 0);
  set.seq_drop_bwd = number("KBJ_DEBUG_DROP_SEQ_BWD_WG", 0);
  set.seq_timeout_ms = (set.seq_drop > 0 || set.seq_drop_bwd > 0) ? 20 : (int)SEQ_TIMEOUT_MS;
  if (getenv("KBJ_SEQ_TIMEOUT_MS")) set.seq_timeout_ms = std::max(1, std::min(30000, number("KBJ_SEQ_TIMEOUT_MS", 0)));
  set.seq_stamps = getenv("KBJ_SEQ_STAMPS") != nullptr; set.stamp_sel = number("KBJ_SEQ_STAMPS", 1);
  set.seq_bstamps = getenv("KBJ_SEQ_BSTAMPS") != nullptr; set.bstamp_sel = number("KBJ_SEQ_BSTAMPS", 0);
  return set;
}

namespace {

int nn_layouts(kbj_ctx* ctx, NnWs* w) {
  const kbj_config& c = ctx->cfg_h;
  w->Hu = c.hidden_size; w->H = (c.hidden_size + 63) / 64 * 64; w->N = c.num_envs; w->B = c.batch_size; w->T = c.rollout_len;
  if (w->B <= 0 || w->B > w->N) return kbj_fail(ctx, "kbj_create: batch_size must be in [1, num_envs]");
  static_cast<ParamLayout&>(*w) = layout_params(c, w->H);
  w->user = layout_params(c, w->Hu);
  w->mirror = c.actor_mirror_loss_scale != 0.0f || c.critic_mirror_loss_scale != 0.0f;
  w->nnets = w->mirror ? 4 : 2;
  return 0;
}

int nn_padding(kbj_ctx* ctx, NnWs* w) {
  if (!w->padded()) return 0;
  std::vector<PadDesc> pd;
  const int Hu = w->Hu, Hi = w->H;
  for (int n = 0; n < 2; ++n) {
    const NetOff &a = w->user.net[n], &b = w->net[n];
    pd.push_back(PadDesc{a.w_in, b.w_in, 1, Hu, Hi, a.nin, a.nin});
    pd.push_back(PadDesc{a.b_in, b.b_in, 1, Hu, Hi, 1, 1});
    for (int l = 0; l < w->D; ++l) {
      pd.push_back(PadDesc{a.w_ih[l], b.w_ih[l], 4, Hu, Hi, Hu, Hi});
      pd.push_back(PadDesc{a.w_hh[l], b.w_hh[l], 4, Hu, Hi, Hu, Hi});
      pd.push_back(PadDesc{a.b[l], b.b[l], 4, Hu, Hi, 1, 1});
    }
    pd.push_back(PadDesc{a.w_out, b.w_out, 1, a.nout, a.nout, Hu, Hi});
    pd.push_back(PadDesc{a.b_out, b.b_out, 1, a.nout, a.nout, 1, 1});
  }
  w->npad = (int)pd.size();
  if (dalloc(ctx, *w, &w->pad_desc, pd.size())) return -1;
  if (hipMemcpy(w->pad_desc, pd.data(), pd.size() * sizeof(PadDesc), hipMemcpyHostToDevice) != hipSuccess) return kbj_fail(ctx, "hipMemcpy pad descriptors");
  if (dalloc(ctx, *w, &w->pparams, w->nparams) || dalloc(ctx, *w, &w->pgrad, w->nparams)) return -1;
  for (int k = 0; k < w->nnets; ++k)
    if (dalloc(ctx, *w, &w->phc[k], (size_t)2 * w->D * w->N * w->H) || dalloc(ctx, *w, &w->pc0[k], (size_t)2 * w->D * w->N * w->H)) return -1;
  return 0;
}

int nn_rollout_scratch(kbj_ctx* ctx, NnWs* w) {
  const size_t N = w->N, H = w->H;
  for (int n = 0; n < w->nnets; ++n) {
    if (dalloc(ctx, *w, &w->rX[n], N * H)) return -1;
    if (dalloc(ctx, *w, &w->rG[n], N * 4 * H)) return -1;
    if (dalloc(ctx, *w, &w->rOut[n], N * 40)) return -1;
    for (int l = 0; l < w->D; ++l) if (dalloc(ctx, *w, &w->rH[n][l], N * H)) return -1;
  }
  if (ctx->cfg_h.gae_tail_value && dalloc(ctx, *w, &w->tail_hc, 2 * (size_t)w->D * N * H)) return -1;
  if (dalloc(ctx, *w, &w->joint_bias_d, KBJ_NU)) return -1;
  if (hipMemcpy(w->joint_bias_d, ctx->model_h.joint_bias, KBJ_NU * sizeof(float), hipMemcpyHostToDevice) != hipSuccess) return kbj_fail(ctx, "hipMemcpy joint_bias");
  return 0;
}

int nn_training_buffers(kbj_ctx* ctx, NnWs* w) {
  const size_t N = w->N, H = w->H, B = w->B, T = w->T, R = T * B;
  if (w->mirror) {
    std::vector<MirrorEntry> ta, tc;
    build_mirror_tables(ctx->model_h, ta, tc, ctx->cfg_h.extra_obs_actor, ctx->cfg_h.extra_obs_critic);
    if (dalloc(ctx, *w, &w->mtab[0], ta.size()) || dalloc(ctx, *w, &w->mtab[1], tc.size())) return -1;
    if (hipMemcpy(w->mtab[0], ta.data(), ta.size() * sizeof(MirrorEntry), hipMemcpyHostToDevice) != hipSuccess ||
        hipMemcpy(w->mtab[1], tc.data(), tc.size() * sizeof(MirrorEntry), hipMemcpyHostToDevice) != hipSuccess) return kbj_fail(ctx, "hipMemcpy mirror tables");
    if (dalloc(ctx, *w, &w->rObsM[0], N * w->net[0].ld_obs) || dalloc(ctx, *w, &w->rObsM[1], N * w->net[1].ld_obs)) return -1;
    float** rs[] = {&w->value_m, &w->dvalue_m, &w->zeroR};
    for (float** p : rs) if (dalloc(ctx, *w, p, R)) return -1;
    float** r20[] = {&w->y_m, &w->sd_m, &w->dy, &w->dy_m};
    for (float** p : r20) if (dalloc(ctx, *w, p, R * KBJ_NU)) return -1;
    if (dalloc(ctx, *w, &w->lpf0_m, B * KBJ_NU)) return -1;
    if (hipMemset(w->zeroR, 0, R * sizeof(float)) != hipSuccess) return kbj_fail(ctx, "hipMemset zeroR");
  }
  for (int n = 0; n < w->nnets; ++n) {
    TrainBufs& t = w->tb[n];
    if (dalloc(ctx, *w, &t.obs, R * w->net[n & 1].ld_obs)) return -1;
    if (dalloc(ctx, *w, &t.X0, R * H)) return -1;
    for (int l = 0; l < w->D; ++l) {
      if (dalloc(ctx, *w, &t.dGl[l], R * 4 * H)) return -1;
      if (dalloc(ctx, *w, &t.G[l], R * 4 * H)) return -1;
      if (dalloc(ctx, *w, &t.Hm[l], (T + 1) * B * H)) return -1;
      if (dalloc(ctx, *w, &t.Hout[l], R * H)) return -1;
      if (dalloc(ctx, *w, &t.Cm[l], (T + 1) * B * H)) return -1;
      if (dalloc(ctx, *w, &t.TanhC[l], R * H)) return -1;
    }
    if (dalloc(ctx, *w, &t.Out, R * 40)) return -1;
    if (dalloc(ctx, *w, &t.dOut, R * 40)) return -1;
    if (dalloc(ctx, *w, &t.dHa, R * H)) return -1;
    if (dalloc(ctx, *w, &t.dHb, R * H)) return -1;
  }
  float** small[] = {&w->keep, &w->logp_old, &w->val_old, &w->adv, &w->target, &w->logp, &w->ent, &w->value, &w->dlogp, &w->dvalue};
  for (float** p : small) if (dalloc(ctx, *w, p, R)) return -1;
  if (dalloc(ctx, *w, &w->act, R * KBJ_NU)) return -1;
  if (dalloc(ctx, *w, &w->y, R * KBJ_NU)) return -1;
  if (dalloc(ctx, *w, &w->sd, R * KBJ_NU)) return -1;
  if (dalloc(ctx, *w, &w->lpf0, B * KBJ_NU)) return -1;
  if (dalloc(ctx, *w, &w->stats, 16)) return -1;
  if (dalloc(ctx, *w, &w->Weff, (size_t)4 * H * w->net[0].ld_obs) || dalloc(ctx, *w, &w->beff, 4 * H)) return -1;
  for (int n = 0; n < w->nnets; ++n) if (dalloc(ctx, *w, &w->Zeff[n], 4 * H * w->net[n & 1].ld_obs)) return -1;
  for (int k = 0; k < 2; ++k) if (dalloc(ctx, *w, &w->WinP[k], H * w->net[k].ld_obs)) return -1;
  if (hipMemset(w->Weff, 0, (size_t)4 * H * w->net[0].ld_obs * sizeof(float)) != hipSuccess) return kbj_fail(ctx, "hipMemset Weff");
  if (dalloc(ctx, *w, &w->seq_counters, SEQ_COUNTER_TOTAL)) return -1;
  if (dalloc(ctx, *w, &w->seq_err, 4)) return -1;
  if (ctx->set.seq_stamps && dalloc(ctx, *w, &w->seq_stamps, (size_t)T * 6)) return -1;
  if (ctx->set.seq_bstamps && dalloc(ctx, *w, &w->seq_bstamps, (size_t)T * 10 + 768)) return -1;
  if (hipMemset(w->seq_err, 0, 4 * sizeof(unsigned)) != hipSuccess) return kbj_fail(ctx, "hipMemset seq_err");
  return 0;
}

int nn_deterministic_workspaces(kbj_ctx* ctx, NnWs* w) {
  if (!w->sched.deterministic) return 0;
  for (int l = 0; l < 4; ++l) if (dalloc(ctx, *w, &w->detp[l], (size_t)DETP_ROWS * DETP_COLS)) return -1;
  return dalloc(ctx, *w, &w->detd, 2 * 512);
}

int nn_residency_check(kbj_ctx* ctx, NnWs* w) {
  const int H = w->H, B = w->B;
  const int grid = ((B + SEQ_ROWS - 1) / SEQ_ROWS) * (H / (SEQ_UNITS * SEQ_UW));
  hipDeviceProp_t prop;
  if (hipGetDeviceProperties(&prop, ctx->device) != hipSuccess) return kbj_fail(ctx, "hipGetDeviceProperties");
  const int cus = prop.multiProcessorCount;
  int per_cu = 0;
  hipError_t oe = hipSuccess;
  if (!dispatch_hidden(H, [&](auto hc) { oe = seq_min_blocks_per_cu<decltype(hc)::value>(&per_cu); return true; }))
    return kbj_fail(ctx, "kbj_create: hidden_size above 512 (persistent LSTM kernels)");
  if (oe != hipSuccess || per_cu < 1) return kbj_fail(ctx, "kbj_create: occupancy query of the persistent LSTM kernels failed");
  const long slots = (long)per_cu * cus;
  w->seq_grid = grid; w->seq_slots = (int)slots;
  char msg[320];
  if (grid > SEQ_COUNTER_WORDS) {
    snprintf(msg, sizeof(msg), "kbj_create: a persistent LSTM launch would need %d workgroups (batch_size / 32 x hidden_size / 32), the hand-off "
             "counters hold %d per launch: lower batch_size", grid, SEQ_COUNTER_WORDS);
    return kbj_fail(ctx, msg);
  }
  if (H > SEQ_FUSED_MAX_H && 2L * grid > slots) w->sched.one_stream = true;
  if ((w->sched.one_stream ? 1L : 2L) * grid > slots) {
    snprintf(msg, sizeof(msg), "kbj_create: %s persistent LSTM launches need %ld resident workgroups, the device holds %ld "
             "(%d per CU x %d CUs): lower batch_size", w->sched.one_stream ? "the" : "two concurrent", (w->sched.one_stream ? 1L : 2L) * grid, slots, per_cu, cus);
    return kbj_fail(ctx, msg);
  }
  return 0;
}

}

int kbj_nn_create(kbj_ctx* ctx) {
  NnWs* w = new NnWs(ctx->set.sched);
  ctx->nn_ws = w;
  if (nn_layouts(ctx, w) || nn_padding(ctx, w) || nn_rollout_scratch(ctx, w) || nn_training_buffers(ctx, w) || nn_deterministic_workspaces(ctx, w)) return -1;
  int wall_khz = 0;
  if (hipDeviceGetAttribute(&wall_khz, hipDeviceAttributeWallClockRate, ctx->device) != hipSuccess || wall_khz <= 0) wall_khz = 100000;
  w->seq_timeout_ticks = (unsigned)std::min<long long>(0xFFFFFFFFll, (long long)ctx->set.seq_timeout_ms * wall_khz);
  return nn_residency_check(ctx, w);
}

void kbj_nn_destroy(kbj_ctx* ctx) {
  NnWs* w = ws_of(ctx);
  if (!w) return;
  for (void* p : w->allocs) hipFree(p);
  for (int l = 0; l < 4; ++l) if (w->skws[l]) hipFree(w->skws[l]);
  delete w;
  ctx->nn_ws = nullptr;
}


int kbj_env_step_range(kbj_ctx* ctx, hipStream_t s, int env0, int count, const float* action_d, float* aux_t_d, float* actor_next_d, float* critic_next_d,
                       float* aux_next_d, float* qstate_t_d);

namespace {

bool net_uses_step_kernel(const NnWs& w, int n) { return w.sched.rollout_step && n == 0; }
float* h_plane(NnWs& w, float* hc, int n, int l, int n0, bool partner) {
  if (!net_uses_step_kernel(w, n)) partner = false;
  return (partner ? w.rH[n][l] : hc + (size_t)(2 * l) * w.N * w.H) + (size_t)n0 * w.H;
}

const float* fold_actor_weights(kbj_ctx* ctx, hipStream_t s, const float* params_d) {
  NnWs& w = *ws_of(ctx);
  const int H = w.H;
  if (!w.sched.rollout_step || w.net[0].ld_obs != KBJ_LD_ACTOR || !w.sched.fold_actor) return nullptr;
  const NetOff& oa = w.net[0];
  GemmArgs g{params_d + oa.w_ih[0], params_d + oa.w_in, w.Weff, nullptr, 4 * H, oa.nin, H, H, oa.nin, oa.ld_obs, 0, 1, nullptr};
  gemm_launch<true, false>(s, g);
  hipLaunchKernelGGL(matvec_kernel, dim3((4 * H + 3) / 4), dim3(256), 0, s, params_d + oa.w_ih[0], params_d + oa.b_in, params_d + oa.b[0], 4 * H, H, w.beff);
  return w.Weff;
}

void repitch_input_weights(kbj_ctx* ctx, hipStream_t s, const float* params_d, int k_lo = 0, int k_hi = 2) {
  NnWs& w = *ws_of(ctx);
  for (int k = k_lo; k < k_hi; ++k) {
    const NetOff& o = w.net[k];
    if (o.nin == o.ld_obs) continue;
    hipLaunchKernelGGL(repitch_rows_kernel, g1((size_t)w.H * o.ld_obs), dim3(256), 0, s, params_d + o.w_in, w.H, o.nin, o.ld_obs, w.WinP[k]);
  }
}

int policy_nets(kbj_ctx* ctx, hipStream_t s, const float* params_d, int net_lo, int net_hi, int n0, int cnt, const float* actor_obs_d, const float* critic_obs_d,
                kbj_carry* carry, uint32_t seed, uint32_t step_index, int argmax, float* action_d, float* logp_d, float* value_d, int parity, const float* weff) {
  NnWs& w = *ws_of(ctx);
  const kbj_config& c = ctx->cfg_h;
  const int N = w.N, H = w.H;
  const bool fused_any = w.sched.rollout_step;
  const float* obs_base[2] = {actor_obs_d, critic_obs_d};
  HeadParams hp{c.min_std, c.max_std, c.var_scale, c.lpf_alpha, w.net[0].ld_obs};
  for (int n = net_lo; n < net_hi; ++n) {
    const int k = n & 1;
    float* const hc = carry_hc(*carry, n);
    const NetOff& o = w.net[k];
    const float* obs = obs_base[k] + (size_t)n0 * o.ld_obs;
    float* obs_m = n >= 2 ? w.rObsM[k] + (size_t)n0 * o.ld_obs : nullptr;
    float* X = w.rX[n] + (size_t)n0 * H;
    float* G = w.rG[n] + (size_t)n0 * 4 * H;
    float* Out = w.rOut[n] + (size_t)n0 * 40;
    if (n >= 2) {
      hipLaunchKernelGGL(mirror_rows_kernel, g1((size_t)cnt * o.ld_obs), dim3(256), 0, s, obs, obs_m, (size_t)cnt, o.ld_obs, w.mtab[k]);
      obs = obs_m;
    }
    const bool fused = fused_any && net_uses_step_kernel(w, n);
    const bool folded = fused && weff && k == 0 && o.ld_obs == KBJ_LD_ACTOR;
    if (!folded) {
      if (o.nin != o.ld_obs) linear_fwd(s, obs, o.ld_obs, w.WinP[k], o.ld_obs, params_d + o.b_in, X, H, cnt, H, o.ld_obs, 0);
      else linear_fwd(s, obs, o.ld_obs, params_d + o.w_in, o.nin, params_d + o.b_in, X, H, cnt, H, o.nin, 0);
    }
    const float* x = X;
    for (int l = 0; l < w.D; ++l) {
      float* cc = hc + (size_t)(2 * l + 1) * N * H + (size_t)n0 * H;
      if (fused) {
        const float* h_in = h_plane(w, hc, n, l, n0, parity != 0);
        float* h_out = h_plane(w, hc, n, l, n0, parity == 0);
        StepArgs sa{x, H, 0, params_d + o.w_ih[l], H, params_d + o.w_hh[l], params_d + o.b[l], h_in, h_out, cc, cnt};
        if (l == 0 && folded) { sa.X = obs; sa.ldx = o.ld_obs; sa.kx = o.nin; sa.Wih = weff; sa.ldw = o.ld_obs; sa.bias = w.beff; }
        if (lstm_step(ctx, s, H, sa)) return -1;
        x = h_out;
        continue;
      }
      float* h = hc + (size_t)(2 * l) * N * H + (size_t)n0 * H;
      {
        GemmArgs g{x, params_d + o.w_ih[l], G, params_d + o.b[l], cnt, 4 * H, 2 * H, H, H, 4 * H, 0, 1, nullptr};
        g.A2 = h; g.B2 = params_d + o.w_hh[l]; g.k1 = H;
        g.x3 = w.sched.gemm_x3 ? 1 : 0;
        gemm_launch<true, true>(s, g, (n > 0 && w.sched.rollout_step) ? 0 : -1);
      }
      CellFwdArgs2 ca;
      ca.a[0] = CellFwdArgs{G, cc, h, cc, nullptr, nullptr, nullptr, nullptr, cnt, H};
      hipLaunchKernelGGL(lstm_cell_fwd_kernel, dim3((cnt * H + 255) / 256, 1), dim3(256), 0, s, ca);
      x = h;
    }
    if (n == 3) continue;
    if (n == 0) {
      hipLaunchKernelGGL(actor_head_fused_kernel, dim3((cnt + HEAD_ENVS * HEAD_WAVES - 1) / (HEAD_ENVS * HEAD_WAVES)), dim3(64 * HEAD_WAVES), 0, s, x, H,
                         params_d + o.w_out, params_d + o.b_out, obs, carry->lpf_d + (size_t)n0 * KBJ_NU, w.joint_bias_d, hp, seed, (uint32_t)(c.env_id_offset + n0),
                         step_index, argmax, cnt, action_d + (size_t)n0 * KBJ_NU, logp_d + n0);
      continue;
    }
    if (n == 1 && o.nout == 1) {
      hipLaunchKernelGGL(critic_value_fused_kernel, g1((size_t)cnt * 32), dim3(256), 0, s, x, H, params_d + o.w_out, params_d + o.b_out, cnt, value_d + n0);
      continue;
    }
    linear_fwd(s, x, H, params_d + o.w_out, H, params_d + o.b_out, Out, 40, cnt, o.nout, H, 0);
    hipLaunchKernelGGL(actor_head_lpf_kernel, g1((size_t)cnt * KBJ_NU), dim3(256), 0, s, Out, obs, carry->lpf_mirror_d + (size_t)n0 * KBJ_NU, w.joint_bias_d, c.lpf_alpha, cnt, w.net[0].ld_obs);
  }
  return 0;
}

void carry_reset_nets(kbj_ctx* ctx, hipStream_t s, int net_lo, int net_hi, int n0, int cnt, kbj_carry* carry, const float* done_d, int done_stride, int parity) {
  NnWs& w = *ws_of(ctx);
  float* lpf[4] = {carry->lpf_d, nullptr, carry->lpf_mirror_d, nullptr};
  const bool partner = parity != 0 && w.sched.rollout_step;
  for (int k = net_lo; k < net_hi; ++k) {
    float* const hc = carry_hc(*carry, k);
    CarryPlanes cp;
    cp.n = 2 * w.D;
    for (int l = 0; l < w.D; ++l) {
      cp.p[2 * l] = h_plane(w, hc, k, l, n0, partner);
      cp.p[2 * l + 1] = hc + (size_t)(2 * l + 1) * w.N * w.H + (size_t)n0 * w.H;
    }
    hipLaunchKernelGGL(carry_reset_kernel, dim3((cnt + 3) / 4), dim3(256), 0, s, cp, cnt, w.H, lpf[k] ? lpf[k] + (size_t)n0 * KBJ_NU : nullptr, done_d + (size_t)n0 * done_stride, done_stride);
  }
}

int carry_h_home(kbj_ctx* ctx, hipStream_t s, int net_lo, int net_hi, kbj_carry* carry) {
  NnWs& w = *ws_of(ctx);
  for (int k = net_lo; k < net_hi; ++k)
    for (int l = 0; l < w.D && net_uses_step_kernel(w, k); ++l)
      KBJ_HIP(ctx, hipMemcpyAsync(carry_hc(*carry, k) + (size_t)(2 * l) * w.N * w.H, w.rH[k][l], (size_t)w.N * w.H * sizeof(float), hipMemcpyDeviceToDevice, s));
  return 0;
}

void pad_params(kbj_ctx* ctx, hipStream_t s, const float* user, float* internal) {
  NnWs& w = *ws_of(ctx);
  hipLaunchKernelGGL(pad_params_kernel, g1(w.nparams), dim3(256), 0, s, w.pad_desc, w.npad, const_cast<float*>(user), internal, w.nparams, 0);
}
void unpad_params(kbj_ctx* ctx, hipStream_t s, const float* internal, float* user) {
  NnWs& w = *ws_of(ctx);
  hipLaunchKernelGGL(pad_params_kernel, g1(w.nparams), dim3(256), 0, s, w.pad_desc, w.npad, user, const_cast<float*>(internal), w.nparams, 1);
}
void repitch_hc(kbj_ctx* ctx, hipStream_t s, const float* src, float* dst, int ws, int wd) {
  NnWs& w = *ws_of(ctx);
  const size_t rows = (size_t)2 * w.D * w.N;
  hipLaunchKernelGGL(repitch_pad_kernel, g1(rows * wd), dim3(256), 0, s, src, dst, rows, ws, wd);
}
kbj_carry pad_carry(kbj_ctx* ctx, hipStream_t s, const kbj_carry& c) {
  NnWs& w = *ws_of(ctx);
  kbj_carry p = c;
  for (int k = 0; k < 4; ++k)
    if (carry_hc(c, k) && w.phc[k]) { repitch_hc(ctx, s, carry_hc(c, k), w.phc[k], w.Hu, w.H); carry_hc(p, k) = w.phc[k]; }
  return p;
}
void unpad_carry(kbj_ctx* ctx, hipStream_t s, const kbj_carry& c) {
  NnWs& w = *ws_of(ctx);
  for (int k = 0; k < 4; ++k)
    if (carry_hc(c, k) && w.phc[k]) repitch_hc(ctx, s, w.phc[k], carry_hc(c, k), w.H, w.Hu);
}
kbj_traj pad_traj_carry0(kbj_ctx* ctx, hipStream_t s, const kbj_traj& tr) {
  NnWs& w = *ws_of(ctx);
  kbj_traj p = tr;
  for (int k = 0; k < 4; ++k)
    if (traj_carry0(tr, k) && w.pc0[k]) { repitch_hc(ctx, s, traj_carry0(tr, k), w.pc0[k], w.Hu, w.H); traj_carry0(p, k) = w.pc0[k]; }
  return p;
}

int critic_tail(kbj_ctx* ctx, hipStream_t s, const float* params_d, const float* critic_obs_d, const float* critic_hc_d, int hc_width, float* value_d) {
  NnWs& w = *ws_of(ctx);
  if (hc_width == w.H) KBJ_HIP(ctx, hipMemcpyAsync(w.tail_hc, critic_hc_d, (size_t)2 * w.D * w.N * w.H * sizeof(float), hipMemcpyDeviceToDevice, s));
  else repitch_hc(ctx, s, critic_hc_d, w.tail_hc, hc_width, w.H);
  kbj_carry sc = {};
  sc.critic_hc_d = w.tail_hc;
  return policy_nets(ctx, s, params_d, 1, 2, 0, w.N, nullptr, critic_obs_d, &sc, 0, 0, 0, nullptr, nullptr, value_d, 0, nullptr);
}

int policy_step_body(kbj_ctx* ctx, const float* params_d, const float* actor_obs_d, const float* critic_obs_d, kbj_carry* carry, uint32_t seed,
                     uint32_t step_index, int argmax, float* action_d, float* logp_d, float* value_d) {
  NnWs& w = *ws_of(ctx);
  kbj_nn_drop_prefetch(ctx);
  KbjTimed timed(ctx, true);
  repitch_input_weights(ctx, ctx->stream, params_d);
  if (policy_nets(ctx, ctx->stream, params_d, 0, w.nnets, 0, w.N, actor_obs_d, critic_obs_d, carry, seed, step_index, argmax, action_d, logp_d, value_d, 0,
                  fold_actor_weights(ctx, ctx->stream, params_d))) return -1;
  if (w.sched.rollout_step && carry_h_home(ctx, ctx->stream, 0, w.nnets, carry)) return -1;
  KBJ_CHECK_LAUNCH(ctx, "kbj_policy_step");
  return 0;
}

int rollout_body(kbj_ctx* ctx, const float* params_d, kbj_carry* carry, uint32_t seed, uint32_t first_step_index, kbj_traj* tr) {
  NnWs& w = *ws_of(ctx);
  const int N = w.N, H = w.H, T = tr->T;
  hipStream_t s = ctx->stream;
  kbj_nn_drop_prefetch(ctx);
  size_t la = w.net[0].ld_obs, lc = w.net[1].ld_obs, lx = KBJ_AUX_SIZE;
  KBJ_HIP(ctx, hipMemcpyAsync(tr->actor_obs_d, tr->actor_obs_d + (size_t)T * N * la, N * la * sizeof(float), hipMemcpyDeviceToDevice, s));
  KBJ_HIP(ctx, hipMemcpyAsync(tr->critic_obs_d, tr->critic_obs_d + (size_t)T * N * lc, N * lc * sizeof(float), hipMemcpyDeviceToDevice, s));
  KBJ_HIP(ctx, hipMemcpyAsync(tr->aux_d, tr->aux_d + (size_t)T * N * lx, N * lx * sizeof(float), hipMemcpyDeviceToDevice, s));
  size_t hcb = (size_t)2 * w.D * N * H * sizeof(float);
  KBJ_HIP(ctx, hipMemcpyAsync(tr->carry0_actor_hc_d, carry->actor_hc_d, hcb, hipMemcpyDeviceToDevice, s));
  KBJ_HIP(ctx, hipMemcpyAsync(tr->carry0_critic_hc_d, carry->critic_hc_d, hcb, hipMemcpyDeviceToDevice, s));
  KBJ_HIP(ctx, hipMemcpyAsync(tr->carry0_lpf_d, carry->lpf_d, (size_t)N * KBJ_NU * sizeof(float), hipMemcpyDeviceToDevice, s));
  if (w.mirror) {
    if (!tr->carry0_actor_mirror_hc_d || !tr->carry0_critic_mirror_hc_d || !tr->carry0_lpf_mirror_d || !carry->actor_mirror_hc_d || !carry->critic_mirror_hc_d || !carry->lpf_mirror_d)
      return kbj_fail(ctx, "kbj_rollout: the mirror losses are enabled, carry and trajectory need the mirror-branch arrays");
    KBJ_HIP(ctx, hipMemcpyAsync(tr->carry0_actor_mirror_hc_d, carry->actor_mirror_hc_d, hcb, hipMemcpyDeviceToDevice, s));
    KBJ_HIP(ctx, hipMemcpyAsync(tr->carry0_critic_mirror_hc_d, carry->critic_mirror_hc_d, hcb, hipMemcpyDeviceToDevice, s));
    KBJ_HIP(ctx, hipMemcpyAsync(tr->carry0_lpf_mirror_d, carry->lpf_mirror_d, (size_t)N * KBJ_NU * sizeof(float), hipMemcpyDeviceToDevice, s));
  }
  const char* pipe_env = getenv("KBJ_ROLLOUT_PIPELINE");
  const bool serial = pipe_env && atoi(pipe_env) == 0;
  hipStream_t cs = serial ? s : ctx->side[0];
  const float* weff = fold_actor_weights(ctx, s, params_d);
  repitch_input_weights(ctx, s, params_d);
  if (!serial) {
    KBJ_HIP(ctx, hipEventRecord(ctx->ev_fork, s));
    KBJ_HIP(ctx, hipStreamWaitEvent(cs, ctx->ev_fork, 0));
  }
  for (int t = 0; t < T; ++t) {
    const float* ao = tr->actor_obs_d + (size_t)t * N * la;
    const float* co = tr->critic_obs_d + (size_t)t * N * lc;
    float* aux_t = tr->aux_d + (size_t)t * N * lx;
    float* act = tr->action_d + (size_t)t * N * KBJ_NU;
    if (policy_nets(ctx, s, params_d, 0, 1, 0, N, ao, co, carry, seed, first_step_index + (uint32_t)t, ctx->rollout_argmax, act, tr->logp_d + (size_t)t * N, tr->value_d + (size_t)t * N, t & 1, weff)) return -1;
    if (policy_nets(ctx, cs, params_d, 1, w.nnets, 0, N, ao, co, carry, seed, first_step_index + (uint32_t)t, 0, act, tr->logp_d + (size_t)t * N, tr->value_d + (size_t)t * N, t & 1, weff)) return -1;
    int rc = kbj_env_step_range(ctx, s, 0, N, act, aux_t, tr->actor_obs_d + (size_t)(t + 1) * N * la, tr->critic_obs_d + (size_t)(t + 1) * N * lc,
                                tr->aux_d + (size_t)(t + 1) * N * lx, tr->qstate_d ? tr->qstate_d + (size_t)t * N * KBJ_QSTATE_SIZE : nullptr);
    if (rc) return rc;
    carry_reset_nets(ctx, s, 0, 1, 0, N, carry, aux_t + KBJ_AUX_DONE, KBJ_AUX_SIZE, (t + 1) & 1);
    if (!serial) {
      KBJ_HIP(ctx, hipEventRecord(ctx->ev_side[0], s));
      KBJ_HIP(ctx, hipStreamWaitEvent(cs, ctx->ev_side[0], 0));
    }
    carry_reset_nets(ctx, cs, 1, w.nnets, 0, N, carry, aux_t + KBJ_AUX_DONE, KBJ_AUX_SIZE, (t + 1) & 1);
  }
  if (ctx->cfg_h.gae_tail_value && tr->value_tail_d && critic_tail(ctx, cs, params_d, tr->critic_obs_d + (size_t)T * N * lc, carry->critic_hc_d, H, tr->value_tail_d)) return -1;
  KBJ_CHECK_LAUNCH(ctx, "kbj_rollout");
  if (!serial) {
    KBJ_HIP(ctx, hipEventRecord(ctx->ev_side[0], cs));
    KBJ_HIP(ctx, hipStreamWaitEvent(s, ctx->ev_side[0], 0));
  }
  if (w.sched.rollout_step && (T & 1) && carry_h_home(ctx, s, 0, w.nnets, carry)) return -1;
  return kbj_rewards(ctx, tr->aux_d, T, tr->reward_d, tr->reward_comps_d);
}

}

extern "C" {

int kbj_mirror_table(const void* model_blob, size_t model_bytes, int critic, int32_t* src_h, float* mul_h, float* add_h) {
  if (!model_blob || !src_h || !mul_h || !add_h || model_bytes != sizeof(kbj_model)) return kbj_fail(nullptr, "kbj_mirror_table: bad argument");
  std::vector<MirrorEntry> ta, tc;
  build_mirror_tables(*reinterpret_cast<const kbj_model*>(model_blob), ta, tc);
  const std::vector<MirrorEntry>& t = critic ? tc : ta;
  for (size_t k = 0; k < t.size(); ++k) { src_h[k] = t[k].src; mul_h[k] = t[k].mul; add_h[k] = t[k].add; }
  return (int)t.size();
}

size_t kbj_param_count(const kbj_config* cfg) { return layout_params(*cfg, cfg->hidden_size).nparams; }
size_t kbj_actor_param_count(const kbj_config* cfg) { return layout_params(*cfg, cfg->hidden_size).nactor; }

int kbj_init_params(kbj_ctx* ctx, uint32_t seed, float* params_d) {
  if (!ctx || !params_d) return kbj_fail(ctx, "kbj_init_params: null argument");
  KBJ_HIP(ctx, hipSetDevice(ctx->device));
  NnWs& w = *ws_of(ctx);
  const ParamLayout& u = w.user;
  int H = w.Hu;
  uint32_t leaf = 0;
  auto fill = [&](size_t off, size_t n, int fan_in) {
    hipLaunchKernelGGL(init_uniform_kernel, g1(n), dim3(256), 0, ctx->stream, params_d + off, n, 1.0f / std::sqrt((float)fan_in), seed, leaf++);
  };
  for (int n = 0; n < 2; ++n) {
    const NetOff& o = u.net[n];
    fill(o.w_in, (size_t)H * o.nin, o.nin); fill(o.b_in, H, o.nin);
    for (int l = 0; l < w.D; ++l) { fill(o.w_ih[l], (size_t)4 * H * H, H); fill(o.w_hh[l], (size_t)4 * H * H, H); fill(o.b[l], (size_t)4 * H, H); }
    fill(o.w_out, (size_t)o.nout * H, H); fill(o.b_out, o.nout, H);
  }
  KBJ_CHECK_LAUNCH(ctx, "init_uniform_kernel");
  return 0;
}

int kbj_policy_step(kbj_ctx* ctx, const float* params_d, const float* actor_obs_d, const float* critic_obs_d, kbj_carry* carry, uint32_t seed,
                    uint32_t step_index, int argmax, float* action_d, float* logp_d, float* value_d) {
  if (!ctx || !params_d || !actor_obs_d || !critic_obs_d || !carry || !action_d || !logp_d || !value_d) return kbj_fail(ctx, "kbj_policy_step: null argument");
  KBJ_HIP(ctx, hipSetDevice(ctx->device));
  NnWs& w = *ws_of(ctx);
  if (w.mirror && (!carry->actor_mirror_hc_d || !carry->critic_mirror_hc_d || !carry->lpf_mirror_d))
    return kbj_fail(ctx, "kbj_policy_step: the mirror losses are enabled, the carry needs the mirror-branch arrays");
  if (!w.padded()) return policy_step_body(ctx, params_d, actor_obs_d, critic_obs_d, carry, seed, step_index, argmax, action_d, logp_d, value_d);
  pad_params(ctx, ctx->stream, params_d, w.pparams);
  kbj_carry pc = pad_carry(ctx, ctx->stream, *carry);
  const int rc = policy_step_body(ctx, w.pparams, actor_obs_d, critic_obs_d, &pc, seed, step_index, argmax, action_d, logp_d, value_d);
  unpad_carry(ctx, ctx->stream, *carry);
  return rc;
}

int kbj_carry_reset(kbj_ctx* ctx, kbj_carry* carry, const float* done_d, int done_stride) {
  if (!ctx || !carry || !done_d) return kbj_fail(ctx, "kbj_carry_reset: null argument");
  KBJ_HIP(ctx, hipSetDevice(ctx->device));
  NnWs& w = *ws_of(ctx);
  if (w.mirror && (!carry->actor_mirror_hc_d || !carry->critic_mirror_hc_d || !carry->lpf_mirror_d)) return kbj_fail(ctx, "kbj_carry_reset: mirror-branch carry arrays are NULL");
  kbj_carry pc = w.padded() ? pad_carry(ctx, ctx->stream, *carry) : *carry;
  carry_reset_nets(ctx, ctx->stream, 0, w.nnets, 0, w.N, &pc, done_d, done_stride, 0);
  if (w.padded()) unpad_carry(ctx, ctx->stream, *carry);
  KBJ_CHECK_LAUNCH(ctx, "carry_reset_kernel");
  return 0;
}

int kbj_critic_value(kbj_ctx* ctx, const float* params_d, const float* critic_obs_d, const kbj_carry* carry, float* value_d) {
  if (!ctx || !params_d || !critic_obs_d || !carry || !carry->critic_hc_d || !value_d) return kbj_fail(ctx, "kbj_critic_value: null argument");
  KBJ_HIP(ctx, hipSetDevice(ctx->device));
  NnWs& w = *ws_of(ctx);
  if (!w.tail_hc) return kbj_fail(ctx, "kbj_critic_value: the context was created with kbj_config.gae_tail_value = 0 (the carry copy it steps is allocated for 1 only)");
  kbj_nn_drop_prefetch(ctx);
  const float* p = params_d;
  if (w.padded()) { pad_params(ctx, ctx->stream, params_d, w.pparams); p = w.pparams; }
  repitch_input_weights(ctx, ctx->stream, p, 1, 2);
  if (critic_tail(ctx, ctx->stream, p, critic_obs_d, carry->critic_hc_d, w.Hu, value_d)) return -1;
  KBJ_CHECK_LAUNCH(ctx, "kbj_critic_value");
  return 0;
}

int kbj_rollout(kbj_ctx* ctx, const float* params_d, kbj_carry* carry, uint32_t seed, uint32_t first_step_index, kbj_traj* tr) {
  if (!ctx || !params_d || !carry || !tr) return kbj_fail(ctx, "kbj_rollout: null argument");
  KBJ_HIP(ctx, hipSetDevice(ctx->device));
  NnWs& w = *ws_of(ctx);
  if (tr->N != w.N || tr->T <= 0) return kbj_fail(ctx, "kbj_rollout: trajectory shape does not match the context");
  if (!w.padded()) return rollout_body(ctx, params_d, carry, seed, first_step_index, tr);
  const size_t ub = (size_t)2 * w.D * w.N * w.Hu * sizeof(float);
  for (int k = 0; k < w.nnets; ++k) {
    if (!traj_carry0(*tr, k) || !carry_hc(*carry, k)) return kbj_fail(ctx, "kbj_rollout: carry / trajectory start-carry array is NULL");
    KBJ_HIP(ctx, hipMemcpyAsync(traj_carry0(*tr, k), carry_hc(*carry, k), ub, hipMemcpyDeviceToDevice, ctx->stream));
  }
  pad_params(ctx, ctx->stream, params_d, w.pparams);
  kbj_carry pc = pad_carry(ctx, ctx->stream, *carry);
  kbj_traj pt = *tr;
  for (int k = 0; k < 4; ++k) traj_carry0(pt, k) = w.pc0[k];
  const int rc = rollout_body(ctx, w.pparams, &pc, seed, first_step_index, &pt);
  unpad_carry(ctx, ctx->stream, *carry);
  return rc;
}

int kbj_gae(kbj_ctx* ctx, const kbj_traj* tr, float* adv_d, float* target_d) {
  if (!ctx || !tr || !adv_d || !target_d) return kbj_fail(ctx, "kbj_gae: null argument");
  KBJ_HIP(ctx, hipSetDevice(ctx->device));
  const kbj_config& c = ctx->cfg_h;
  if (c.gae_tail_value && !tr->value_tail_d)
    return kbj_fail(ctx, "kbj_gae: kbj_config.gae_tail_value = 1 needs kbj_traj.value_tail_d (kbj_rollout / kbj_critic_value fill it), it is NULL");
  kbj_nn_drop_prefetch(ctx);
  if (c.gae_bootstrap_truncation || c.gae_tail_value) {
    hipLaunchKernelGGL(gae_boundary_kernel, g1(tr->N, 64), dim3(64), 0, ctx->stream, tr->value_d, tr->reward_d, tr->aux_d, c.gae_tail_value ? tr->value_tail_d : nullptr,
                       tr->T, tr->N, c.gamma, c.lam, (int)c.gae_bootstrap_truncation, adv_d, target_d);
    KBJ_CHECK_LAUNCH(ctx, "gae_boundary_kernel");
    return 0;
  }
  hipLaunchKernelGGL(gae_kernel, g1(tr->N, 64), dim3(64), 0, ctx->stream, tr->value_d, tr->reward_d, tr->aux_d, tr->T, tr->N, c.gamma, c.lam, adv_d, target_d);
  KBJ_CHECK_LAUNCH(ctx, "gae_kernel");
  return 0;
}

}

namespace {

int head_gathers(kbj_ctx* ctx, hipStream_t st, const kbj_traj* tr, const int32_t* idx) {
  NnWs& w = *ws_of(ctx);
  const int T = tr->T, N = tr->N, H = w.H, B = w.B, R = T * B, D = w.D;
  const int lda = w.net[0].ld_obs;
  if (lda % 4 == 0 && ((size_t)tr->actor_obs_d & 15) == 0)
    hipLaunchKernelGGL(gather_rows4_kernel, g1((size_t)R * (lda / 4)), dim3(256), 0, st, reinterpret_cast<const float4*>(tr->actor_obs_d), idx, T, N, B, lda / 4, lda / 4, lda / 4,
                       reinterpret_cast<float4*>(w.tb[0].obs));
  else hipLaunchKernelGGL(gather_rows_kernel, g1((size_t)R * lda), dim3(256), 0, st, tr->actor_obs_d, idx, T, N, B, lda, lda, lda, w.tb[0].obs);
  GatherSmallArgs gs{tr->action_d, nullptr, nullptr, nullptr, nullptr, tr->aux_d, w.act, w.logp_old, w.val_old, w.adv, w.target, w.keep};
  hipLaunchKernelGGL(gather_small_kernel, g1((size_t)R), dim3(256), 0, st, gs, idx, T, N, B, KBJ_NU + 4, KBJ_NU + 5);
  if (w.mirror && (!traj_carry0(*tr, 2) || !traj_carry0(*tr, 3) || !tr->carry0_lpf_mirror_d))
    return kbj_fail(ctx, "PPO pass: the mirror losses are enabled, the trajectory needs the mirror-branch carries");
  GatherCarryArgs gc;
  gc.nplanes = 0;
  for (int n = 0; n < w.nnets; ++n)
    for (int l = 0; l < D; ++l) {
      gc.src[gc.nplanes] = traj_carry0(*tr, n) + (size_t)(2 * l) * N * H; gc.dst[gc.nplanes++] = w.tb[n].Hm[l];
      gc.src[gc.nplanes] = traj_carry0(*tr, n) + (size_t)(2 * l + 1) * N * H; gc.dst[gc.nplanes++] = w.tb[n].Cm[l];
    }
  gc.nlpf = 0;
  gc.src[gc.nplanes] = tr->carry0_lpf_d; gc.dst[gc.nplanes] = w.lpf0; gc.nlpf++;
  if (w.mirror) { gc.src[gc.nplanes + 1] = tr->carry0_lpf_mirror_d; gc.dst[gc.nplanes + 1] = w.lpf0_m; gc.nlpf++; }
  hipLaunchKernelGGL(gather_carry_kernel, dim3((B * H + 255) / 256, gc.nplanes + gc.nlpf), dim3(256), 0, st, gc, idx, B, H);
  return 0;
}

int ppo_forward_nets(kbj_ctx* ctx, const float* params_d, const kbj_traj* tr, const int32_t* idx, const float* adv_d, const float* target_d, float* grad_d,
                     bool grad, hipStream_t ns[2]) {
  NnWs& w = *ws_of(ctx);
  const Sched& sc = w.sched;
  const int T = tr->T, N = tr->N, H = w.H, B = w.B, R = T * B, D = w.D;
  ns[0] = (sc.one_stream || !sc.critic_on_caller) ? ctx->stream : ctx->stream2;
  ns[1] = (sc.one_stream || sc.critic_on_caller) ? ctx->stream : ctx->stream2;
  hipStream_t s = ns[0];
  if (!w.counters_clean) KBJ_HIP(ctx, hipMemsetAsync(w.seq_counters, 0, SEQ_COUNTER_TOTAL * sizeof(unsigned), ctx->stream));
  w.counters_clean = false;
  KBJ_HIP(ctx, hipEventRecord(ctx->ev_fork, ctx->stream));
  KBJ_HIP(ctx, hipStreamWaitEvent(ctx->stream2, ctx->ev_fork, 0));
  if (sc.fold_actor) {
    const NetOff& oa = w.net[0];
    GemmArgs g{params_d + oa.w_ih[0], params_d + oa.w_in, w.Weff, nullptr, 4 * H, oa.nin, H, H, oa.nin, oa.ld_obs, 0, 1, nullptr};
    gemm_launch<true, false>(s, g);
    hipLaunchKernelGGL(matvec_kernel, dim3((4 * H + 3) / 4), dim3(256), 0, s, params_d + oa.w_ih[0], params_d + oa.b_in, params_d + oa.b[0], 4 * H, H, w.beff);
  }
  auto gather = [&](hipStream_t st, const float* src, int wdt, int lds, float* dst, int ldd) {
    if (wdt % 4 == 0 && lds % 4 == 0 && ldd % 4 == 0 && ((size_t)src & 15) == 0 && ((size_t)dst & 15) == 0)
      hipLaunchKernelGGL(gather_rows4_kernel, g1((size_t)R * (wdt / 4)), dim3(256), 0, st, reinterpret_cast<const float4*>(src), idx, T, N, B, wdt / 4, lds / 4, ldd / 4,
                         reinterpret_cast<float4*>(dst));
    else hipLaunchKernelGGL(gather_rows_kernel, g1((size_t)R * wdt), dim3(256), 0, st, src, idx, T, N, B, wdt, lds, ldd, dst);
  };
  const bool gather_late = !sc.one_stream && !w.mirror && sc.fold_actor;
  if (!gather_late) gather(ns[1], tr->critic_obs_d, w.net[1].ld_obs, w.net[1].ld_obs, w.tb[1].obs, w.net[1].ld_obs);
  GatherSmallArgs gs{tr->action_d, grad ? tr->logp_d : nullptr, grad ? tr->value_d : nullptr, adv_d, target_d, tr->aux_d, w.act, w.logp_old, w.val_old, w.adv, w.target, w.keep};
  const bool pending = w.prefetched_idx != nullptr;
  const bool prefetched = pending && w.prefetched_idx == idx && w.prefetched_traj == tr && !sc.one_stream;
  w.prefetched_idx = nullptr; w.prefetched_traj = nullptr;
  if (pending) KBJ_HIP(ctx, hipStreamWaitEvent(s, ctx->ev_prefetch, 0));
  if (!prefetched && head_gathers(ctx, s, tr, idx)) return -1;
  {
    hipStream_t sm = sc.one_stream ? s : ctx->side[0];
    if (!sc.one_stream) KBJ_HIP(ctx, hipStreamWaitEvent(sm, ctx->ev_fork, 0));
    hipLaunchKernelGGL(gather_small_kernel, g1((size_t)R * (KBJ_NU + 4)), dim3(256), 0, sm, gs, idx, T, N, B, 0, KBJ_NU + 4);
    if (grad) {
      KBJ_HIP(ctx, hipMemsetAsync(w.stats, 0, 16 * sizeof(double), sm));
#ifndef KBJ_NO_TAIL_CLEAN
      w.sumsq_clean = true;
#endif
      if (w.ext_adv_sums) {
        KBJ_HIP(ctx, hipMemcpyAsync(w.stats, w.ext_adv_sums, 2 * sizeof(double), hipMemcpyDeviceToDevice, sm));
        KBJ_HIP(ctx, hipMemcpyAsync(w.stats + 11, w.ext_adv_sums + 2, sizeof(double), hipMemcpyDeviceToDevice, sm));
      } else {
        hipLaunchKernelGGL(adv_stats_kernel, dim3(32), dim3(256), 0, sm, w.adv, R, w.stats, sc.deterministic ? w.detd : (double*)nullptr);
        if (sc.deterministic) reduce_double_launch(sm, w.detd, 32, 2, w.stats);
      }
      KBJ_HIP(ctx, hipMemsetAsync(grad_d, 0, w.nparams * sizeof(float), sm));
      if (sc.fold_actor)
        for (int n = 0; n < w.nnets; ++n)
          if ((n & 1) == 0 || sc.fold_critic) KBJ_HIP(ctx, hipMemsetAsync(w.Zeff[n], 0, (size_t)4 * H * w.net[n & 1].ld_obs * sizeof(float), sm));
    }
    if (!sc.one_stream) KBJ_HIP(ctx, hipEventRecord(ctx->ev_small, sm));
  }
  KBJ_HIP(ctx, hipEventRecord(ctx->ev_join, ns[0]));
  if (w.mirror)
    for (int k = 0; k < 2; ++k)
      hipLaunchKernelGGL(mirror_rows_kernel, g1((size_t)R * w.net[k].ld_obs), dim3(256), 0, ns[k], w.tb[k].obs, w.tb[2 + k].obs, (size_t)R, w.net[k].ld_obs, w.mtab[k]);
  const int stamp_sel = ctx->set.stamp_sel;
  const int stamp_net = (stamp_sel - 1) & 1, stamp_layer = ((stamp_sel - 1) >> 1) & 1;
  const bool fuse_ih = sc.fuse_ih;
  const bool fuse_obs = sc.fuse_obs && w.net[0].ld_obs == KBJ_LD_ACTOR;
  for (int n = 0; n < w.nnets; ++n) {
    const NetOff& o = w.net[n & 1];
    if (sc.fold_actor && (n & 1) == 0) continue;
    if (n < 2) hipLaunchKernelGGL(repitch_rows_kernel, g1((size_t)H * o.ld_obs), dim3(256), 0, ns[n & 1], params_d + o.w_in, H, o.nin, o.ld_obs, w.WinP[n & 1]);
    if (n == 1 && gather_late) {
      GemmArgs g{tr->critic_obs_d, w.WinP[1], w.tb[1].X0, params_d + o.b_in, R, H, o.ld_obs, o.ld_obs, o.ld_obs, H, 0, 1, nullptr};
      g.a_idx = idx; g.a_B = B; g.a_N = N;
      g.x3 = sc.gemm_x3 ? 1 : 0;
      gemm_launch<true, true>(ns[1], g, sc.gemm_x3 ? -1 : 2);
      KBJ_HIP(ctx, hipStreamWaitEvent(ctx->side[1], ctx->ev_join, 0));
      KBJ_HIP(ctx, hipStreamWaitEvent(ctx->side[1], ctx->ev_small, 0));
      if (grad) gather(ctx->side[1], tr->critic_obs_d, w.net[1].ld_obs, w.net[1].ld_obs, w.tb[1].obs, w.net[1].ld_obs);
      KBJ_HIP(ctx, hipEventRecord(ctx->ev_obs, ctx->side[1]));
      continue;
    }
    linear_fwd(ns[n & 1], w.tb[n].obs, o.ld_obs, w.WinP[n & 1], o.ld_obs, params_d + o.b_in, w.tb[n].X0, H, R, H, o.ld_obs, 0);
  }
  if (!sc.one_stream) KBJ_HIP(ctx, hipStreamWaitEvent(ns[1], ctx->ev_join, 0));
  for (int l = 0; l < D; ++l) {
    for (int n = 0; n < w.nnets; ++n) {
      const NetOff& o = w.net[n & 1];
      TrainBufs& t = w.tb[n];
      if (sc.fold_actor && (n & 1) == 0 && l == 0) { if (!fuse_obs) linear_fwd(ns[0], t.obs, o.ld_obs, w.Weff, o.ld_obs, w.beff, t.G[0], 4 * H, R, 4 * H, o.nin, 0); }
      else if (!fuse_ih) linear_fwd(ns[n & 1], l == 0 ? t.X0 : t.Hout[l - 1], H, params_d + o.w_ih[l], H, params_d + o.b[l], t.G[l], 4 * H, R, 4 * H, H, 0);
    }
    for (int n = 0; n < w.nnets; ++n) {
      const NetOff& o = w.net[n & 1];
      TrainBufs& t = w.tb[n];
      SeqFwdArgs fa{t.G[l], params_d + o.w_hh[l], t.Hm[l], t.Cm[l], t.Hout[l], t.TanhC[l], w.keep, w.seq_counters + SEQ_COUNTER_WORDS * (4 * l + n), w.seq_err, T, B, (n == stamp_net && l == stamp_layer) ? w.seq_stamps : nullptr};
      if (sc.fold_actor && (n & 1) == 0 && l == 0) {
        if (fuse_obs) { fa.X = t.obs; fa.ldx = o.ld_obs; fa.Wih = w.Weff; fa.ldw = o.ld_obs; fa.bias = w.beff; fa.kx = o.nin; }
      } else if (fuse_ih) {
        fa.X = l == 0 ? t.X0 : t.Hout[l - 1]; fa.Wih = params_d + o.w_ih[l]; fa.bias = params_d + o.b[l];
      }
      if (seq_fwd(ctx, ns[n & 1], H, fa)) return -1;
    }
  }
  if (!sc.one_stream) {
    KBJ_HIP(ctx, hipStreamWaitEvent(ns[0], ctx->ev_small, 0));
    KBJ_HIP(ctx, hipStreamWaitEvent(ns[1], gather_late ? ctx->ev_obs : ctx->ev_small, 0));
  }
  return 0;
}

int ppo_forward_body(kbj_ctx* ctx, const float* params_d, const kbj_traj* tr, const int32_t* env_idx_d, kbj_ppo_vars* out) {
  NnWs& w = *ws_of(ctx);
  const kbj_config& c = ctx->cfg_h;
  const int T = tr->T, H = w.H, B = w.B, R = T * B, D = w.D;
  hipStream_t ns[2];
  if (ppo_forward_nets(ctx, params_d, tr, env_idx_d, nullptr, nullptr, nullptr, false, ns)) return -1;
  hipStream_t s = ns[0];
  for (int n = 0; n < 2; ++n) {
    const NetOff& o = w.net[n];
    linear_fwd(ns[n], w.tb[n].Hout[D - 1], H, params_d + o.w_out, H, params_d + o.b_out, w.tb[n].Out, 40, R, o.nout, H, 0);
  }
  HeadParams hp{c.min_std, c.max_std, c.var_scale, c.lpf_alpha, w.net[0].ld_obs};
  hipLaunchKernelGGL(actor_head_pre_kernel, g1((size_t)R * KBJ_NU), dim3(256), 0, s, w.tb[0].Out, w.tb[0].obs, w.joint_bias_d, hp, R, w.y, w.sd);
  hipLaunchKernelGGL(actor_head_train_fwd_kernel, g1((size_t)B * KBJ_NU, 64), dim3(64), 0, s, w.keep, w.lpf0, hp, T, B, w.y);
  hipLaunchKernelGGL(gaussian_logp_kernel, g1(R), dim3(256), 0, s, w.y, w.sd, w.act, R, out->logp_d, out->entropy_d ? out->entropy_d : w.ent);
  if (out->action_std_d) KBJ_HIP(ctx, hipMemcpyAsync(out->action_std_d, w.sd, (size_t)R * KBJ_NU * sizeof(float), hipMemcpyDeviceToDevice, s));
  if (out->action_mean_d) KBJ_HIP(ctx, hipMemcpyAsync(out->action_mean_d, w.y, (size_t)R * KBJ_NU * sizeof(float), hipMemcpyDeviceToDevice, s));
  hipLaunchKernelGGL(critic_value_kernel, g1(R), dim3(256), 0, ns[1], w.tb[1].Out, 40, R, out->value_d);
  if (!w.sched.one_stream) {
    KBJ_HIP(ctx, hipEventRecord(ctx->ev_join, ctx->stream2));
    KBJ_HIP(ctx, hipStreamWaitEvent(ctx->stream, ctx->ev_join, 0));
  }
  hipLaunchKernelGGL(poison_vars_kernel, dim3(1), dim3(1), 0, ctx->stream, w.seq_err, out->logp_d, out->value_d);
  KBJ_CHECK_LAUNCH(ctx, "kbj_ppo_forward");
  if (w.sched.debug_sync) return kbj_synchronize(ctx);
  return 0;
}

int ppo_grad_body(kbj_ctx* ctx, const float* params_d, const kbj_traj* tr, const int32_t* env_idx_d, const float* adv_d, const float* target_d,
                  float* grad_d, float* metrics_d) {
  NnWs& w = *ws_of(ctx);
  const kbj_config& c = ctx->cfg_h;
  const Sched& sc = w.sched;
  const int T = tr->T, H = w.H, B = w.B, R = T * B, D = w.D;
  KbjTimed timed(ctx, true);
  const bool one_stream = sc.one_stream, fold_actor = sc.fold_actor, fold_critic = sc.fold_critic;
  hipStream_t ns[2];
  if (ppo_forward_nets(ctx, params_d, tr, env_idx_d, adv_d, target_d, grad_d, true, ns)) return -1;
  hipStream_t s = ns[0];
  const int bstamp_sel = ctx->set.bstamp_sel;
  const bool fused_critic_head = sc.fused_critic_head && !w.mirror && w.net[1].nout == 1;
  for (int n = 0; n < w.nnets; ++n) {
    const NetOff& o = w.net[n & 1];
    if (n == 1 && fused_critic_head) continue;
    linear_fwd(ns[n & 1], w.tb[n].Hout[D - 1], H, params_d + o.w_out, H, params_d + o.b_out, w.tb[n].Out, 40, R, o.nout, H, 0);
  }
  HeadParams hp{c.min_std, c.max_std, c.var_scale, c.lpf_alpha, w.net[0].ld_obs};
  PpoParams pp{c.clip_param, c.value_clip, c.value_loss_coef, c.entropy_coef, c.log_ratio_clip, c.adv_eps};
  hipLaunchKernelGGL(actor_head_pre_kernel, g1((size_t)R * KBJ_NU), dim3(256), 0, s, w.tb[0].Out, w.tb[0].obs, w.joint_bias_d, hp, R, w.y, w.sd);
  hipLaunchKernelGGL(actor_head_train_fwd_kernel, g1((size_t)B * KBJ_NU, 64), dim3(64), 0, s, w.keep, w.lpf0, hp, T, B, w.y);
  hipLaunchKernelGGL(gaussian_logp_kernel, g1(R), dim3(256), 0, s, w.y, w.sd, w.act, R, w.logp, w.ent);
  hipLaunchKernelGGL(ppo_loss_kernel, g1(R), dim3(256), 0, s, w.logp, w.value, w.ent, w.logp_old, w.val_old, w.adv, w.target, w.stats, pp, R, w.dlogp, w.dvalue,
                     w.stats + 2, one_stream ? 0 : 1);
  if (fused_critic_head) {
    const NetOff& oc = w.net[1];
    TrainBufs& tc = w.tb[1];
    const dim3 grid(2048), block(256);
    const bool built = dispatch_hidden(H, [&](auto hc) {
      hipLaunchKernelGGL((critic_head_kernel<decltype(hc)::value / 64>), grid, block, 0, ns[1], tc.Hout[D - 1], params_d + oc.w_out, params_d + oc.b_out, w.val_old, w.target,
                         pp, R, w.value, w.dvalue, tc.dOut, tc.dHa, w.stats + 2);
      return true;
    });
    if (!built) return kbj_fail(ctx, "kbj_ppo_grad: critic_head_kernel is built for hidden sizes 64, 128, ..., 512");
    if (one_stream) hipLaunchKernelGGL(ppo_loss_kernel, g1(R), dim3(256), 0, s, w.logp, w.value, w.ent, w.logp_old, w.val_old, w.adv, w.target, w.stats, pp, R, w.dlogp, w.dvalue,
                                       w.stats + 2, 1);
  } else {
    hipLaunchKernelGGL(critic_value_kernel, g1(R), dim3(256), 0, ns[1], w.tb[1].Out, 40, R, w.value);
    hipLaunchKernelGGL(ppo_loss_kernel, g1(R), dim3(256), 0, ns[1], w.logp, w.value, w.ent, w.logp_old, w.val_old, w.adv, w.target, w.stats, pp, R, w.dlogp, w.dvalue,
                       w.stats + 2, one_stream ? 3 : 2);
  }
  if (w.mirror) {
    hipLaunchKernelGGL(actor_head_pre_kernel, g1((size_t)R * KBJ_NU), dim3(256), 0, s, w.tb[2].Out, w.tb[2].obs, w.joint_bias_d, hp, R, w.y_m, w.sd_m);
    hipLaunchKernelGGL(actor_head_train_fwd_kernel, g1((size_t)B * KBJ_NU, 64), dim3(64), 0, s, w.keep, w.lpf0_m, hp, T, B, w.y_m);
    hipLaunchKernelGGL(mirror_loss_kernel, g1(R), dim3(256), 0, s, w.y, w.y_m, w.value, w.value_m, c.actor_mirror_loss_scale, c.critic_mirror_loss_scale, R, w.dy, w.dy_m,
                       w.dvalue, w.dvalue_m, w.stats + 2, one_stream ? 0 : 1);
    hipLaunchKernelGGL(critic_value_kernel, g1(R), dim3(256), 0, ns[1], w.tb[3].Out, 40, R, w.value_m);
    hipLaunchKernelGGL(mirror_loss_kernel, g1(R), dim3(256), 0, ns[1], w.y, w.y_m, w.value, w.value_m, c.actor_mirror_loss_scale, c.critic_mirror_loss_scale, R, w.dy, w.dy_m,
                       w.dvalue, w.dvalue_m, w.stats + 2, one_stream ? 3 : 2);
  }
  const bool critic_fork_recorded = !one_stream && fused_critic_head;
  hipEvent_t ev_critic_loss = critic_fork_recorded ? ctx->ev_side[1] : ctx->ev_pool[ctx->ev_next++ & 31];
  if (!one_stream) hipEventRecord(ev_critic_loss, ns[1]);
  hipLaunchKernelGGL(actor_head_bwd_pre_kernel, g1((size_t)R * KBJ_NU), dim3(256), 0, s, w.tb[0].Out, w.y, w.sd, w.act, w.dlogp,
                     w.mirror ? w.dy : (const float*)nullptr, -c.entropy_coef / (float)R, hp, R, w.tb[0].dOut);
  hipLaunchKernelGGL(actor_head_train_bwd_kernel, g1((size_t)B * KBJ_NU, 64), dim3(64), 0, s, w.keep, hp, T, B, w.tb[0].dOut);
  if (!fused_critic_head) KBJ_HIP(ctx, hipMemcpy2DAsync(w.tb[1].dOut, 40 * sizeof(float), w.dvalue, sizeof(float), sizeof(float), R, hipMemcpyDeviceToDevice, ns[1]));
  if (w.mirror) {
    hipLaunchKernelGGL(actor_head_bwd_pre_kernel, g1((size_t)R * KBJ_NU), dim3(256), 0, s, w.tb[2].Out, w.y_m, w.sd_m, w.y_m, w.zeroR, w.dy_m, 0.0f, hp, R, w.tb[2].dOut);
    hipLaunchKernelGGL(actor_head_train_bwd_kernel, g1((size_t)B * KBJ_NU, 64), dim3(64), 0, s, w.keep, hp, T, B, w.tb[2].dOut);
    KBJ_HIP(ctx, hipMemcpy2DAsync(w.tb[3].dOut, 40 * sizeof(float), w.dvalue_m, sizeof(float), sizeof(float), R, hipMemcpyDeviceToDevice, ns[1]));
  }
  auto side_of = [&](int n) { return one_stream ? ns[n & 1] : ctx->side[n & 1]; };
  auto fork_side = [&](int n) { if (!one_stream) { hipEventRecord(ctx->ev_side[n & 1], ns[n & 1]); hipStreamWaitEvent(ctx->side[n & 1], ctx->ev_side[n & 1], 0); } };
  float *dh_above[4], *dx_out[4];
  for (int n = 0; n < w.nnets; ++n) {
    const NetOff& o = w.net[n & 1];
    TrainBufs& t = w.tb[n];
    if (!(n == 1 && fused_critic_head)) linear_bwd_input(ns[n & 1], sc.gemm_x3, t.dOut, 40, params_d + o.w_out, H, t.dHa, H, R, H, o.nout, 0);
    if (n == 1 && critic_fork_recorded) hipStreamWaitEvent(ctx->side[1], ctx->ev_side[1], 0);
    else fork_side(n);
    linear_bwd_weight(ctx, side_of(n), sc.gemm_x3, t.dOut, 40, t.Hout[D - 1], H, grad_d + o.w_out, H, o.nout, H, R);
    colsum_acc(ctx, side_of(n), t.dOut, R, o.nout, 40, grad_d + o.b_out);
    dh_above[n] = t.dHa; dx_out[n] = t.dHb;
  }
  auto fold_bias_terms = [&](int k, hipStream_t st) {
    const NetOff& oa = w.net[k];
    float* part = det_partials(ctx, st);
    hipLaunchKernelGGL(matvec_t_acc_kernel, dim3((H + 63) / 64, 16), dim3(256), 0, st, params_d + oa.w_ih[0], grad_d + oa.b[0], 4 * H, H, grad_d + oa.b_in, part);
    if (part) reduce_rows_launch(st, part, 16, H, grad_d + oa.b_in);
    hipLaunchKernelGGL(outer_acc_kernel, g1((size_t)4 * H * H), dim3(256), 0, st, grad_d + oa.w_ih[0], grad_d + oa.b[0], params_d + oa.b_in, 4 * H, H);
  };
  bool bias_done[2] = {false, false};
  struct PendingDW { int n, l; };
  std::vector<PendingDW> pending_dw;
  auto launch_dw_pair = [&](hipStream_t st, int n, int l) {
    const NetOff& o = w.net[n & 1];
    TrainBufs& t = w.tb[n];
    linear_bwd_weight2(ctx, st, sc.gemm_x3, t.dGl[l], 4 * H, t.Hm[l], l == 0 ? t.X0 : t.Hout[l - 1], H, grad_d + o.w_hh[l], grad_d + o.w_ih[l], H, 4 * H, H, R);
  };
  for (int l = D - 1; l >= 0; --l) {
    for (int n = 0; n < w.nnets; ++n) {
      const NetOff& o = w.net[n & 1];
      TrainBufs& t = w.tb[n];
      SeqBwdArgs ba{t.G[l], t.TanhC[l], t.Cm[l], dh_above[n], w.keep, params_d + o.w_hh[l], t.dGl[l], w.seq_counters + SEQ_COUNTER_WORDS * (4 * (D + l) + n), w.seq_err, T, B, grad_d + o.b[l]};
      ba.db_part = det_partials(ctx, ns[n & 1]);
      if (w.seq_bstamps && bstamp_sel == 1 + n + 2 * l) ba.stamps = w.seq_bstamps;
      const bool tiles16 = sc.bwd16;
      if (seq_bwd(ctx, ns[n & 1], H, ba, tiles16)) return -1;
      if (ba.db_part) reduce_rows_launch(ns[n & 1], ba.db_part, seq_bwd_row_groups(B, tiles16), 4 * H, grad_d + o.b[l]);
    }
    const bool tail_on_own_lane = l == 0 && !w.mirror && fold_actor;
    for (const PendingDW& p : pending_dw) {
      if (one_stream) { launch_dw_pair(ns[p.n & 1], p.n, p.l); continue; }
      if (tail_on_own_lane && ((p.n & 1) == 0 || fold_critic)) continue;
      hipStream_t ws = side_of(p.n);
      hipEventRecord(ctx->ev_dx[p.n & 1], ns[p.n & 1]);
      hipStreamWaitEvent(ws, ctx->ev_dx[p.n & 1], 0);
      launch_dw_pair(ws, p.n, p.l);
    }
    for (int n = 0; n < w.nnets; ++n) {
      const NetOff& o = w.net[n & 1];
      TrainBufs& t = w.tb[n];
      hipStream_t s = ns[n & 1], ws = side_of(n);
      const bool folded = fold_actor && l == 0 && ((n & 1) == 0 || fold_critic);
      const bool own_lane = l == 0 && !w.mirror && folded;
      if (folded) {
        if (own_lane) ws = s;
        else fork_side(n);
        float* Z = w.Zeff[n];
        const int ts = H % 128 == 0 ? 128 : 64;
        int sk = std::max(2, std::min(g_splitk_wgs / ((4 * H / ts) * (H / ts + (o.nin + ts - 1) / ts)), (R + 255) / 256));
        GemmArgs g{t.dGl[0], t.Hm[0], grad_d + o.w_hh[0], nullptr, 4 * H, H + o.nin, R, 4 * H, H, H, 1, sk, nullptr};
        g.B2 = t.obs; g.C2 = Z; g.n1 = H; g.ldb2 = o.ld_obs; g.ldc2 = o.ld_obs;
        g.skws = sk_workspace(ctx, ws, (size_t)sk * 4 * H * (H + o.nin));
        g.x3 = sc.gemm_x3;
        gemm_launch<false, false>(ws, g, ts == 128 ? 1 : 0);
        GemmArgs g1a{params_d + o.w_ih[0], Z, grad_d + o.w_in, nullptr, H, o.nin, 4 * H, H, o.ld_obs, o.nin, 1, g_fold_sk, nullptr};
        g1a.skws = sk_workspace(ctx, ws, (size_t)g_fold_sk * H * o.nin);
        gemm_launch<false, false>(ws, g1a);
        GemmArgs g2a{Z, params_d + o.w_in, grad_d + o.w_ih[0], nullptr, 4 * H, H, o.nin, o.ld_obs, o.nin, H, 1, 1, nullptr};
        gemm_launch<true, true>(ws, g2a);
        if (own_lane && n < 2) { fold_bias_terms(n, ws); bias_done[n] = true; }
        if (own_lane && !one_stream)
          for (const PendingDW& p : pending_dw) if (p.n == n && p.l > l) launch_dw_pair(s, p.n, p.l);
        continue;
      }
      linear_bwd_input(s, sc.gemm_x3, t.dGl[l], 4 * H, params_d + o.w_ih[l], H, dx_out[n], H, R, H, 4 * H, 0, H <= 256 ? 2 : -1);
      if (l > 0) pending_dw.push_back(PendingDW{n, l});
      else {
        fork_side(n);
        launch_dw_pair(ws, n, l);
      }
      std::swap(dh_above[n], dx_out[n]);
    }
    pending_dw.erase(std::remove_if(pending_dw.begin(), pending_dw.end(), [&](const PendingDW& p) { return p.l > l; }), pending_dw.end());
  }
  for (int n = 0; n < w.nnets; ++n) {
    const NetOff& o = w.net[n & 1];
    TrainBufs& t = w.tb[n];
    hipStream_t s = ns[n & 1];
    if (!(fold_actor && ((n & 1) == 0 || fold_critic))) {
      linear_bwd_weight(ctx, s, sc.gemm_x3, dh_above[n], H, t.obs, o.ld_obs, grad_d + o.w_in, o.nin, H, o.nin, R);
      colsum_acc(ctx, s, dh_above[n], R, H, H, grad_d + o.b_in);
    }
    if (!one_stream) {
      hipStream_t joiner = ((n & 1) == 1 && sc.critic_on_caller && bias_done[1]) ? ns[0] : s;
      hipEventRecord(ctx->ev_side[n & 1], ctx->side[n & 1]); hipStreamWaitEvent(joiner, ctx->ev_side[n & 1], 0);
    }
  }
  if (fold_actor && !bias_done[0]) fold_bias_terms(0, ns[0]);
  if (!one_stream) hipStreamWaitEvent(ns[0], ev_critic_loss, 0);
  hipLaunchKernelGGL(ppo_metrics_kernel, dim3(1), dim3(1), 0, ns[0], w.stats + 2, w.stats, pp, R, metrics_d);
  if (one_stream) {
    if (fold_actor && fold_critic && !bias_done[1]) fold_bias_terms(1, ns[1]);
    hipLaunchKernelGGL(lane_tail_kernel, dim3(2 * MAXD * 4), dim3(SEQ_COUNTER_WORDS), 0, ctx->stream, w.seq_counters, -1, w.seq_err, grad_d, grad_d + w.nactor);
    KBJ_HIP(ctx, hipEventRecord(ctx->ev_actor_grad, ctx->stream));
  } else {
    hipLaunchKernelGGL(lane_tail_kernel, dim3(2 * MAXD * 4), dim3(SEQ_COUNTER_WORDS), 0, ns[0], w.seq_counters, 0, w.seq_err, grad_d, (float*)nullptr);
    KBJ_HIP(ctx, hipEventRecord(ctx->ev_actor_grad, ns[0]));
    if (fold_actor && fold_critic && !bias_done[1]) fold_bias_terms(1, ns[1]);
    hipLaunchKernelGGL(lane_tail_kernel, dim3(2 * MAXD * 4), dim3(SEQ_COUNTER_WORDS), 0, ns[1], w.seq_counters, 1, w.seq_err, grad_d + w.nactor, (float*)nullptr);
    KBJ_HIP(ctx, hipEventRecord(ctx->ev_join, ctx->stream2));
    KBJ_HIP(ctx, hipStreamWaitEvent(ctx->stream, ctx->ev_join, 0));
  }
#ifndef KBJ_NO_TAIL_CLEAN
  w.counters_clean = true;
#endif
  KBJ_CHECK_LAUNCH(ctx, "kbj_ppo_grad");
  if (sc.debug_sync) return kbj_synchronize(ctx);
  return 0;
}

}

extern "C" {

int kbj_ppo_forward(kbj_ctx* ctx, const float* params_d, const kbj_traj* tr, const int32_t* env_idx_d, int B, kbj_ppo_vars* out) {
  if (!ctx || !params_d || !tr || !env_idx_d || !out || !out->logp_d || !out->value_d) return kbj_fail(ctx, "kbj_ppo_forward: null argument");
  KBJ_HIP(ctx, hipSetDevice(ctx->device));
  NnWs& w = *ws_of(ctx);
  if (B != w.B) return kbj_fail(ctx, "kbj_ppo_forward: B must equal config.batch_size");
  if (tr->T != w.T || tr->N != w.N) return kbj_fail(ctx, "kbj_ppo_forward: trajectory shape does not match the context");
  if (!w.padded()) return ppo_forward_body(ctx, params_d, tr, env_idx_d, out);
  pad_params(ctx, ctx->stream, params_d, w.pparams);
  kbj_traj pt = pad_traj_carry0(ctx, ctx->stream, *tr);
  return ppo_forward_body(ctx, w.pparams, &pt, env_idx_d, out);
}

int kbj_ppo_grad(kbj_ctx* ctx, const float* params_d, const kbj_traj* tr, const int32_t* env_idx_d, int B, const float* adv_d, const float* target_d,
                 float* grad_d, float* metrics_d) {
  if (!ctx || !params_d || !tr || !env_idx_d || !adv_d || !target_d || !grad_d || !metrics_d) return kbj_fail(ctx, "kbj_ppo_grad: null argument");
  KBJ_HIP(ctx, hipSetDevice(ctx->device));
  NnWs& w = *ws_of(ctx);
  if (B != w.B) return kbj_fail(ctx, "kbj_ppo_grad: B must equal config.batch_size");
  if (tr->T != w.T || tr->N != w.N) return kbj_fail(ctx, "kbj_ppo_grad: trajectory shape does not match the context");
  if (!w.padded()) return ppo_grad_body(ctx, params_d, tr, env_idx_d, adv_d, target_d, grad_d, metrics_d);
  hipStream_t s = ctx->stream;
  pad_params(ctx, s, params_d, w.pparams);
  kbj_traj pt = pad_traj_carry0(ctx, s, *tr);
  const int rc = ppo_grad_body(ctx, w.pparams, &pt, env_idx_d, adv_d, target_d, w.pgrad, metrics_d);
  if (rc) return rc;
  unpad_params(ctx, s, w.pgrad, grad_d);
  KBJ_HIP(ctx, hipEventRecord(ctx->ev_actor_grad, s));
  KBJ_CHECK_LAUNCH(ctx, "pad_params_kernel");
  return 0;
}

int kbj_ppo_prefetch(kbj_ctx* ctx, const kbj_traj* traj, const int32_t* env_idx_d) {
  if (!ctx || !ctx->nn_ws || !traj || !env_idx_d) return kbj_fail(ctx, "kbj_ppo_prefetch: null argument");
  KBJ_HIP(ctx, hipSetDevice(ctx->device));
  NnWs& w = *ws_of(ctx);
  if (traj->T != w.T || traj->N != w.N) return kbj_fail(ctx, "kbj_ppo_prefetch: trajectory shape does not match the context");
  if (w.sched.one_stream || w.padded()) return 0;
  hipStream_t lane = ctx->side[1];
  KBJ_HIP(ctx, hipEventRecord(ctx->ev_fork, ctx->stream));
  KBJ_HIP(ctx, hipStreamWaitEvent(lane, ctx->ev_fork, 0));
  if (head_gathers(ctx, lane, traj, env_idx_d)) return -1;
  KBJ_HIP(ctx, hipEventRecord(ctx->ev_prefetch, lane));
  w.prefetched_idx = env_idx_d; w.prefetched_traj = traj;
  KBJ_CHECK_LAUNCH(ctx, "kbj_ppo_prefetch");
  return 0;
}

int kbj_recurrence_residency(kbj_ctx* ctx, int* grid_wgs, int* concurrent, int* slots) {
  if (!ctx || !ctx->nn_ws || !grid_wgs || !concurrent || !slots) return kbj_fail(ctx, "kbj_recurrence_residency: null argument");
  const NnWs& w = *ws_of(ctx);
  *grid_wgs = w.seq_grid; *concurrent = w.sched.one_stream ? 1 : 2; *slots = w.seq_slots;
  return 0;
}

int kbj_set_rollout_argmax(kbj_ctx* ctx, int argmax) {
  if (!ctx) return kbj_fail(nullptr, "kbj_set_rollout_argmax: null ctx");
  ctx->rollout_argmax = argmax != 0;
  return 0;
}

int kbj_set_advantage_sums(kbj_ctx* ctx, const double* sums_d) {
  if (!ctx || !ctx->nn_ws) return kbj_fail(ctx, "kbj_set_advantage_sums: null ctx");
  ws_of(ctx)->ext_adv_sums = sums_d;
  return 0;
}

int kbj_stream_wait_actor_grad(kbj_ctx* ctx, void* hip_stream) {
  if (!ctx) return kbj_fail(nullptr, "kbj_stream_wait_actor_grad: null ctx");
  KBJ_HIP(ctx, hipSetDevice(ctx->device));
  KBJ_HIP(ctx, hipStreamWaitEvent((hipStream_t)hip_stream, ctx->ev_actor_grad, 0));
  return 0;
}

int kbj_set_learning_rate(kbj_ctx* ctx, float learning_rate) {
  if (!ctx || !std::isfinite(learning_rate)) return kbj_fail(ctx, "kbj_set_learning_rate: bad argument");
  ctx->cfg_h.learning_rate = learning_rate;
  return 0;
}

int kbj_adamw_step(kbj_ctx* ctx, float* params_d, float* m_d, float* v_d, const float* grad_d, int64_t step, float grad_scale) {
  if (!ctx || !params_d || !m_d || !v_d || !grad_d || step < 1) return kbj_fail(ctx, "kbj_adamw_step: bad argument");
  KBJ_HIP(ctx, hipSetDevice(ctx->device));
  NnWs& w = *ws_of(ctx);
  const kbj_config& c = ctx->cfg_h;
  hipStream_t s = ctx->stream;
  double* sumsq = w.stats + 10;
  if (!w.sumsq_clean) KBJ_HIP(ctx, hipMemsetAsync(sumsq, 0, sizeof(double), s));
  w.sumsq_clean = false;
  double* part = w.sched.deterministic ? w.detd : nullptr;
  hipLaunchKernelGGL(sumsq_kernel, dim3(512), dim3(256), 0, s, grad_d, w.user.nparams, grad_scale, sumsq, part);
  if (part) reduce_double_launch(s, part, 512, 1, sumsq);
  AdamParams ap{c.learning_rate, c.adam_b1, c.adam_b2, c.adam_eps, c.weight_decay, c.max_grad_norm,
                (float)(1.0 - std::pow((double)c.adam_b1, (double)step)), (float)(1.0 - std::pow((double)c.adam_b2, (double)step)), grad_scale};
  hipLaunchKernelGGL(adamw_kernel, g1(w.user.nparams), dim3(256), 0, s, params_d, m_d, v_d, grad_d, w.user.nparams, sumsq, ap, w.seq_err);
  KBJ_CHECK_LAUNCH(ctx, "adamw_kernel");
  return 0;
}

}
```

kbot-joystick_amd/csrc/kbj_nn_kernels.h:

```cpp
#pragma once
#include <hip/hip_runtime.h>
#include <stdint.h>
#include "kbj_model.h"

namespace kbj {

constexpr float kLog2Pi = 1.8378770664093453f;

__device__ __forceinline__ float sigmoidf_(float x) { return __builtin_amdgcn_rcpf(1.0f + __expf(-x)); }
__device__ __forceinline__ float tanhf_(float x) { float xc = fminf(fmaxf(x, -15.0f), 15.0f); return 1.0f - 2.0f * __builtin_amdgcn_rcpf(1.0f + __expf(2.0f * xc)); }
__device__ __forceinline__ float softplusf_(float x) { return x > 20.0f ? x : log1pf(expf(x)); }

struct CellFwdArgs {
  float* G; const float* c_prev; float* h_out; float* c_out; float* hm_next; float* cm_next; float* tanhc; const float* keep;
  int M, H;
};
struct CellFwdArgs2 { CellFwdArgs a[2]; };
__global__ void lstm_cell_fwd_kernel(CellFwdArgs2 args) {
  const CellFwdArgs& a = args.a[blockIdx.y];
  int idx = blockIdx.x * blockDim.x + threadIdx.x;
  if (idx >= a.M * a.H) return;
  int m = idx / a.H, u = idx - m * a.H;
  float* g = a.G + (size_t)m * 4 * a.H;
  float i = sigmoidf_(g[u]), f = sigmoidf_(g[a.H + u]), gg = tanhf_(g[2 * a.H + u]), o = sigmoidf_(g[3 * a.H + u]);
  float c = f * a.c_prev[idx] + i * gg;
  float tc = tanhf_(c), h = o * tc;
  g[u] = i; g[a.H + u] = f; g[2 * a.H + u] = gg; g[3 * a.H + u] = o;
  a.h_out[idx] = h;
  a.c_out[idx] = c;
  if (a.hm_next) { float k = a.keep[m]; a.hm_next[idx] = h * k; a.cm_next[idx] = c * k; a.tanhc[idx] = tc; }
}

__device__ __forceinline__ uint32_t nn_rotl32(uint32_t x, int r) { return (x << r) | (x >> (32 - r)); }
__device__ __forceinline__ void nn_threefry(uint32_t k0, uint32_t k1, uint32_t c0, uint32_t c1, uint32_t& o0, uint32_t& o1) {
  const int rot[8] = {13, 15, 26, 6, 17, 29, 16, 24};
  uint32_t ks[3] = {k0, k1, k0 ^ k1 ^ 0x1BD11BDAu};
  uint32_t x0 = c0 + ks[0], x1 = c1 + ks[1];
#pragma unroll
  for (int g = 0; g < 5; ++g) {
#pragma unroll
    for (int r = 0; r < 4; ++r) { x0 += x1; x1 = nn_rotl32(x1, rot[(g & 1) * 4 + r]); x1 ^= x0; }
    x0 += ks[(g + 1) % 3]; x1 += ks[(g + 2) % 3] + (uint32_t)(g + 1);
  }
  o0 = x0; o1 = x1;
}

struct HeadParams { float min_std, max_std, var_scale, alpha; int ld_obs; };
constexpr int HEAD_ENVS = 16;
constexpr int HEAD_WAVES = 4;
typedef float head_f32x4 __attribute__((ext_vector_type(4)));
__global__ __launch_bounds__(64 * HEAD_WAVES) void actor_head_fused_kernel(const float* __restrict__ hin , int H, const float* __restrict__ Wout ,
                                                                          const float* __restrict__ bout, const float* __restrict__ obs ,
                                                                          float* __restrict__ lpf, const float* __restrict__ joint_bias, HeadParams hp, uint32_t seed,
                                                                          uint32_t env_off, uint32_t step, int argmax, int N, float* __restrict__ action,
                                                                          float* __restrict__ logp) {
  __shared__ float outs[HEAD_WAVES][HEAD_ENVS][49];
  __shared__ float lps[HEAD_WAVES][HEAD_ENVS][KBJ_NU + 1];
  const int lane = threadIdx.x & 63, wv = threadIdx.x >> 6, g = lane >> 4, c = lane & 15;
  const int n0 = (blockIdx.x * HEAD_WAVES + wv) * HEAD_ENVS;
  if (n0 < N) {
    const float* arow = hin + (size_t)min(n0 + c, N - 1) * H + 4 * g;
    const float* brow[3] = {Wout + (size_t)c * H + 4 * g, Wout + (size_t)(16 + c) * H + 4 * g, Wout + (size_t)min(32 + c, 2 * KBJ_NU - 1) * H + 4 * g};
    head_f32x4 acc[3] = {{0, 0, 0, 0}, {0, 0, 0, 0}, {0, 0, 0, 0}};
    for (int k = 0; k < H; k += 16) {
      const head_f32x4 a = *reinterpret_cast<const head_f32x4*>(arow + k);
#pragma unroll
      for (int t = 0; t < 3; ++t) {
        const head_f32x4 b = *reinterpret_cast<const head_f32x4*>(brow[t] + k);
#pragma unroll
        for (int q = 0; q < 4; ++q) acc[t] = __builtin_amdgcn_mfma_f32_16x16x4f32(a[q], b[q], acc[t], 0, 0, 0);
      }
    }
#pragma unroll
    for (int t = 0; t < 3; ++t)
#pragma unroll
      for (int r = 0; r < 4; ++r) outs[wv][4 * g + r][16 * t + c] = acc[t][r];
  }
  __syncthreads();
  if (n0 < N) {
    for (int item = lane; item < HEAD_ENVS * KBJ_NU; item += 64) {
      const int e = item / KBJ_NU, j = item - e * KBJ_NU, n = n0 + e;
      float lp = 0;
      if (n < N) {
        const float om = outs[wv][e][j] + bout[j], os = outs[wv][e][KBJ_NU + j] + bout[KBJ_NU + j];
        float mean = om + joint_bias[j] + (j >= 10 ? obs[(size_t)n * hp.ld_obs + KBJ_OBS_CMD + 6 + (j - 10)] : 0.0f);
        float sd = fminf((softplusf_(os) + hp.min_std) * hp.var_scale, hp.max_std);
        float y0 = lpf[n * KBJ_NU + j];
        float y = y0 + hp.alpha * (mean - y0);
        lpf[n * KBJ_NU + j] = y;
        float a = y;
        if (!argmax) {
          uint32_t b0, b1;
          nn_threefry(seed ^ ((uint32_t)KBJ_RNG_ACTION * 0x9E3779B9u), env_off + (uint32_t)n, step, (uint32_t)j, b0, b1);
          float u1 = (float)((b0 >> 8) + 1u) * (1.0f / 16777216.0f), u2 = (float)(b1 >> 8) * (1.0f / 16777216.0f);
          a = y + sd * (sqrtf(-2.0f * logf(u1)) * cosf(6.283185307179586f * u2));
        }
        action[n * KBJ_NU + j] = a;
        float z = (a - y) / sd;
        lp = -0.5f * z * z - logf(sd) - 0.5f * kLog2Pi;
      }
      lps[wv][e][j] = lp;
    }
  }
  __syncthreads();
  if (n0 < N && lane < HEAD_ENVS && n0 + lane < N) {
    float lp = 0;
#pragma unroll
    for (int j = 0; j < KBJ_NU; ++j) lp += lps[wv][lane][j];
    logp[n0 + lane] = lp;
  }
}

__global__ __launch_bounds__(256) void critic_value_fused_kernel(const float* __restrict__ hin , int H, const float* __restrict__ wout ,
                                                                 const float* __restrict__ bout, int N, float* __restrict__ value) {
  const int tid = blockIdx.x * blockDim.x + threadIdx.x, n = tid >> 5, j = tid & 31;
  float acc = 0;
  if (n < N)
    for (int c = j; c < H / 4; c += 32) {
      const float4 h = *reinterpret_cast<const float4*>(hin + (size_t)n * H + 4 * c), w = *reinterpret_cast<const float4*>(wout + 4 * c);
      acc = fmaf(h.x, w.x, acc); acc = fmaf(h.y, w.y, acc); acc = fmaf(h.z, w.z, acc); acc = fmaf(h.w, w.w, acc);
    }
  for (int o = 16; o > 0; o >>= 1) acc += __shfl_xor(acc, o);
  if (n < N && j == 0) value[n] = acc + bout[0];
}

__global__ void critic_value_kernel(const float* __restrict__ out, int ld, int N, float* __restrict__ value) {
  int n = blockIdx.x * blockDim.x + threadIdx.x;
  if (n < N) value[n] = out[(size_t)n * ld];
}

struct CarryPlanes { float* p[2 * KBJ_MAX_DEPTH]; int n; };
__global__ void carry_reset_kernel(CarryPlanes hc, int cnt, int H, float* __restrict__ lpf, const float* __restrict__ done, int stride) {
  const int row = blockIdx.x * (blockDim.x >> 6) + (threadIdx.x >> 6), lane = threadIdx.x & 63;
  if (row >= cnt || done[(size_t)row * stride] == 0.0f) return;
  for (int p = 0; p < hc.n; ++p)
    for (int k = lane; k < H; k += 64) hc.p[p][(size_t)row * H + k] = 0.0f;
  if (lpf && lane < KBJ_NU) lpf[(size_t)row * KBJ_NU + lane] = 0.0f;
}

__global__ void gather_rows_kernel(const float* __restrict__ src, const int* __restrict__ idx, int T, int N, int B, int w, int ld_src, int ld_dst, float* __restrict__ dst) {
  size_t i = (size_t)blockIdx.x * blockDim.x + threadIdx.x;
  size_t total = (size_t)T * B * w;
  if (i >= total) return;
  int k = i % w;
  size_t r = i / w;
  int b = r % B, t = r / B;
  dst[r * ld_dst + k] = src[((size_t)t * N + idx[b]) * ld_src + k];
}
__global__ void gather_rows4_kernel(const float4* __restrict__ src, const int* __restrict__ idx, int T, int N, int B, int w4, int ld_src4, int ld_dst4, float4* __restrict__ dst) {
  size_t i = (size_t)blockIdx.x * blockDim.x + threadIdx.x;
  size_t total = (size_t)T * B * w4;
  if (i >= total) return;
  int k = i % w4;
  size_t r = i / w4;
  int b = r % B, t = r / B;
  dst[r * ld_dst4 + k] = src[((size_t)t * N + idx[b]) * ld_src4 + k];
}
__global__ void gather_keep_kernel(const float* __restrict__ aux, const int* __restrict__ idx, int T, int N, int B, float* __restrict__ keep) {
  int i = blockIdx.x * blockDim.x + threadIdx.x;
  if (i >= T * B) return;
  int b = i % B, t = i / B;
  keep[i] = aux[((size_t)t * N + idx[b]) * KBJ_AUX_SIZE + KBJ_AUX_DONE] != 0 ? 0.0f : 1.0f;
}

struct GatherSmallArgs {
  const float *action, *logp, *value, *adv, *target, *aux;
  float *action_o, *logp_o, *value_o, *adv_o, *target_o, *keep_o;
};
__global__ void gather_small_kernel(GatherSmallArgs a, const int* __restrict__ idx, int T, int N, int B, int c0, int c1) {
  const int W = c1 - c0;
  size_t i = (size_t)blockIdx.x * blockDim.x + threadIdx.x;
  if (i >= (size_t)T * B * W) return;
  size_t r = i / W;
  int c = c0 + (int)(i - r * W), b = (int)(r % B);
  size_t src = (r / B) * N + idx[b];
  if (c < KBJ_NU) a.action_o[r * KBJ_NU + c] = a.action[src * KBJ_NU + c];
  else if (c == KBJ_NU) { if (a.logp) a.logp_o[r] = a.logp[src]; }
  else if (c == KBJ_NU + 1) { if (a.value) a.value_o[r] = a.value[src]; }
  else if (c == KBJ_NU + 2) { if (a.adv) a.adv_o[r] = a.adv[src]; }
  else if (c == KBJ_NU + 3) { if (a.target) a.target_o[r] = a.target[src]; }
  else a.keep_o[r] = a.aux[src * KBJ_AUX_SIZE + KBJ_AUX_DONE] != 0 ? 0.0f : 1.0f;
}
struct GatherCarryArgs { const float* src[8 * KBJ_MAX_DEPTH + 2]; float* dst[8 * KBJ_MAX_DEPTH + 2]; int nplanes, nlpf; };
__global__ void gather_carry_kernel(GatherCarryArgs a, const int* __restrict__ idx, int B, int H) {
  int p = blockIdx.y;
  int w = p < a.nplanes ? H : KBJ_NU;
  int i = blockIdx.x * blockDim.x + threadIdx.x;
  if (i >= B * w) return;
  int b = i / w, k = i - b * w;
  a.dst[p][i] = a.src[p][(size_t)idx[b] * w + k];
}

__global__ void actor_head_pre_kernel(const float* __restrict__ out, const float* __restrict__ obs, const float* __restrict__ joint_bias, HeadParams hp,
                                      int R, float* __restrict__ y, float* __restrict__ sd) {
  size_t i = (size_t)blockIdx.x * blockDim.x + threadIdx.x;
  if (i >= (size_t)R * KBJ_NU) return;
  size_t r = i / KBJ_NU;
  int j = (int)(i - r * KBJ_NU);
  y[i] = out[r * 40 + j] + joint_bias[j] + (j >= 10 ? obs[r * hp.ld_obs + KBJ_OBS_CMD + 6 + (j - 10)] : 0.0f);
  sd[i] = fminf((softplusf_(out[r * 40 + KBJ_NU + j]) + hp.min_std) * hp.var_scale, hp.max_std);
}
__global__ void actor_head_train_fwd_kernel(const float* __restrict__ keep, const float* __restrict__ lpf0, HeadParams hp, int T, int B, float* __restrict__ y) {
  int i = blockIdx.x * blockDim.x + threadIdx.x;
  if (i >= B * KBJ_NU) return;
  int b = i / KBJ_NU, j = i % KBJ_NU;
  float state = lpf0[i];
  constexpr int U = 10;
  for (int t0 = 0; t0 < T; t0 += U) {
    float mean[U], kp[U];
#pragma unroll
    for (int u = 0; u < U; ++u) {
      int t = t0 + u;
      if (t < T) { size_t r = (size_t)t * B + b; mean[u] = y[r * KBJ_NU + j]; kp[u] = keep[r]; }
    }
#pragma unroll
    for (int u = 0; u < U; ++u) {
      int t = t0 + u;
      if (t < T) {
        float yy = state + hp.alpha * (mean[u] - state);
        y[((size_t)t * B + b) * KBJ_NU + j] = yy;
        state = yy * kp[u];
      }
    }
  }
}
__global__ void gaussian_logp_kernel(const float* __restrict__ y, const float* __restrict__ sd, const float* __restrict__ act, int R,
                                     float* __restrict__ logp, float* __restrict__ ent) {
  int r = blockIdx.x * blockDim.x + threadIdx.x;
  if (r >= R) return;
  float lp = 0, en = 0;
  for (int j = 0; j < KBJ_NU; ++j) {
    float s = sd[(size_t)r * KBJ_NU + j], z = (act[(size_t)r * KBJ_NU + j] - y[(size_t)r * KBJ_NU + j]) / s;
    lp += -0.5f * z * z - logf(s) - 0.5f * kLog2Pi;
    en += 0.5f + 0.5f * kLog2Pi + logf(s);
  }
  logp[r] = lp; ent[r] = en;
}

__global__ void adv_stats_kernel(const float* __restrict__ adv, int R, double* __restrict__ stats, double* __restrict__ part) {
  __shared__ double s1[256], s2[256];
  double a = 0, b = 0;
  for (int i = blockIdx.x * 256 + threadIdx.x; i < R; i += 256 * gridDim.x) { double v = adv[i]; a += v; b += v * v; }
  s1[threadIdx.x] = a; s2[threadIdx.x] = b;
  __syncthreads();
  for (int o = 128; o > 0; o >>= 1) { if (threadIdx.x < o) { s1[threadIdx.x] += s1[threadIdx.x + o]; s2[threadIdx.x] += s2[threadIdx.x + o]; } __syncthreads(); }
  if (threadIdx.x == 0) {
    if (part) { part[2 * blockIdx.x] = s1[0]; part[2 * blockIdx.x + 1] = s2[0]; }
    else { atomicAdd(&stats[0], s1[0]); atomicAdd(&stats[1], s2[0]); }
  }
}
constexpr int RD_CHUNK = 1024;
__global__ __launch_bounds__(256) void reduce_double_kernel(const double* __restrict__ part, int nblocks, int w, double* __restrict__ out) {
  __shared__ double stage[RD_CHUNK];
  const int tid = threadIdx.x;
  if (nblocks <= 0) return;
  const int rows = RD_CHUNK / w;
  const size_t total = (size_t)nblocks * w;
  double v[RD_CHUNK / 256];
  auto fetch = [&](int b0) {
    const size_t base = (size_t)b0 * w;
#pragma unroll
    for (int i = 0; i < RD_CHUNK / 256; ++i) { const size_t e = base + tid + 256 * i; v[i] = part[e < total ? e : total - 1]; }
  };
  fetch(0);
  const double o0 = tid < w ? out[tid] : 0.0;
  double s = 0;
  for (int b0 = 0; b0 < nblocks; b0 += rows) {
#pragma unroll
    for (int i = 0; i < RD_CHUNK / 256; ++i) stage[tid + 256 * i] = v[i];
    __syncthreads();
    if (b0 + rows < nblocks) fetch(b0 + rows);
    if (tid < w) {
      const int m = nblocks - b0 < rows ? nblocks - b0 : rows;
      int r = 0;
      for (; r + 8 <= m; r += 8) {
        double x[8];
#pragma unroll
        for (int i = 0; i < 8; ++i) x[i] = stage[(r + i) * w + tid];
#pragma unroll
        for (int i = 0; i < 8; ++i) s += x[i];
      }
      for (; r < m; ++r) s += stage[r * w + tid];
    }
    __syncthreads();
  }
  if (tid < w) out[tid] = o0 + s;
}
inline void reduce_double_launch(hipStream_t s, const double* part, int nblocks, int w, double* out) {
  hipLaunchKernelGGL(reduce_double_kernel, dim3(1), dim3(256), 0, s, part, nblocks, w, out);
}
struct PpoParams { float clip, vclip, vcoef, ecoef, lrclip, adv_eps; };
__global__ void ppo_loss_kernel(const float* __restrict__ logp, const float* __restrict__ value, const float* __restrict__ ent,
                                const float* __restrict__ logp_old, const float* __restrict__ value_old, const float* __restrict__ adv,
                                const float* __restrict__ target, const double* __restrict__ stats, PpoParams pp, int R,
                                float* __restrict__ dlogp, float* __restrict__ dvalue, double* __restrict__ macc, int part) {
  __shared__ double red[6][256];
  int r = blockIdx.x * blockDim.x + threadIdx.x;
  double m[6] = {0, 0, 0, 0, 0, 0};
  const float inv = 1.0f / R;
  if (r < R && (part & 1)) {
    const double cnt = stats[11] > 0 ? stats[11] : (double)R;
    const double mean_d = stats[0] / cnt, var_d = fmax(stats[1] / cnt - mean_d * mean_d, 0.0);
    float a;
    if (mean_d * mean_d <= 64.0 * var_d) {
      float mean = (float)mean_d;
      float var = fmaxf((float)(stats[1] / cnt) - mean * mean, 0.0f);
      a = (adv[r] - mean) / (sqrtf(var) + pp.adv_eps);
    } else {
      a = (float)(((double)adv[r] - mean_d) / (sqrt(var_d) + (double)pp.adv_eps));
    }
    float d = logp[r] - logp_old[r];
    float dcl = fminf(fmaxf(d, -pp.lrclip), pp.lrclip);
    float ratio = expf(dcl);
    float rc = fminf(fmaxf(ratio, 1 - pp.clip), 1 + pp.clip);
    float s1 = ratio * a, s2 = rc * a;
    bool unclipped = s1 <= s2;
    float surr = unclipped ? s1 : s2;
    dlogp[r] = (unclipped && fabsf(d) < pp.lrclip) ? -inv * a * ratio : 0.0f;
    m[0] = -surr; m[2] = ent[r]; m[3] = fabsf(ratio - 1) > pp.clip ? 1.0 : 0.0; m[4] = -d;
  }
  if (r < R && (part & 2)) {
    float v = value[r], vo = value_old[r], tg = target[r];
    float dv = v - vo, dvc = fminf(fmaxf(dv, -pp.vclip), pp.vclip), vcl = vo + dvc;
    float e1 = (v - tg) * (v - tg), e2 = (vcl - tg) * (vcl - tg);
    float gv = e1 >= e2 ? (v - tg) : ((fabsf(dv) < pp.vclip) ? (vcl - tg) : 0.0f);
    dvalue[r] = pp.vcoef * inv * gv;
    m[1] = 0.5f * fmaxf(e1, e2);
  }
  for (int k = 0; k < 6; ++k) red[k][threadIdx.x] = m[k];
  __syncthreads();
  for (int o = 128; o > 0; o >>= 1) { if (threadIdx.x < o) for (int k = 0; k < 5; ++k) red[k][threadIdx.x] += red[k][threadIdx.x + o]; __syncthreads(); }
  if (threadIdx.x == 0) for (int k = 0; k < 5; ++k) if (k == 1 ? (part & 2) : (part & 1)) atomicAdd(&macc[k], red[k][0]);
}
template <int VPL>
__global__ void critic_head_kernel(const float* __restrict__ h, const float* __restrict__ w_out, const float* __restrict__ b_out,
                                   const float* __restrict__ value_old, const float* __restrict__ target, PpoParams pp, int R,
                                   float* __restrict__ value, float* __restrict__ dvalue, float* __restrict__ dout, float* __restrict__ dh,
                                   double* __restrict__ macc) {
  constexpr int H = 64 * VPL;
  __shared__ double red[4];
  const int lane = threadIdx.x & 63, wv = threadIdx.x >> 6;
  float wreg[VPL];
#pragma unroll
  for (int j = 0; j < VPL; ++j) wreg[j] = w_out[lane * VPL + j];
  const float bias = b_out[0], inv = 1.0f / R;
  double m1 = 0;
  for (int r = blockIdx.x * 4 + wv; r < R; r += gridDim.x * 4) {
    float x[VPL], s = 0;
#pragma unroll
    for (int j = 0; j < VPL; ++j) { x[j] = h[(size_t)r * H + lane * VPL + j]; s += x[j] * wreg[j]; }
#pragma unroll
    for (int o = 32; o > 0; o >>= 1) s += __shfl_xor(s, o);
    const float v = s + bias, vo = value_old[r], tg = target[r];
    const float dv = v - vo, dvc = fminf(fmaxf(dv, -pp.vclip), pp.vclip), vcl = vo + dvc;
    const float e1 = (v - tg) * (v - tg), e2 = (vcl - tg) * (vcl - tg);
    const float gv = e1 >= e2 ? (v - tg) : ((fabsf(dv) < pp.vclip) ? (vcl - tg) : 0.0f);
    const float dval = pp.vcoef * inv * gv;
#pragma unroll
    for (int j = 0; j < VPL; ++j) dh[(size_t)r * H + lane * VPL + j] = dval * wreg[j];
    if (lane == 0) { value[r] = v; dvalue[r] = dval; dout[(size_t)r * 40] = dval; m1 += 0.5f * fmaxf(e1, e2); }
  }
  if (lane == 0) red[wv] = m1;
  __syncthreads();
  if (threadIdx.x == 0) atomicAdd(&macc[1], red[0] + red[1] + red[2] + red[3]);
}
__global__ void ppo_metrics_kernel(const double* __restrict__ macc, const double* __restrict__ stats, PpoParams pp, int R, float* __restrict__ metrics) {
  double pol = macc[0] / R, vl = macc[1] / R, en = macc[2] / R, ma = macc[5] / R, mc = macc[6] / R;
  const double cnt = stats[11] > 0 ? stats[11] : (double)R;
  double mean = stats[0] / cnt, var = stats[1] / cnt - mean * mean;
  metrics[0] = (float)(pol + pp.vcoef * vl - pp.ecoef * en + ma + mc);
  metrics[8] = (float)ma; metrics[9] = (float)mc;
  metrics[1] = (float)pol; metrics[2] = (float)vl; metrics[3] = (float)en; metrics[4] = (float)(macc[3] / R); metrics[5] = (float)(macc[4] / R);
  metrics[6] = (float)mean; metrics[7] = (float)sqrt(var > 0 ? var : 0);
}

struct MirrorEntry { int src; float mul, add; };
__global__ void mirror_rows_kernel(const float* __restrict__ in, float* __restrict__ out, size_t rows, int ld, const MirrorEntry* __restrict__ tab) {
  size_t i = (size_t)blockIdx.x * blockDim.x + threadIdx.x;
  if (i >= rows * ld) return;
  size_t r = i / ld;
  int k = (int)(i - r * ld);
  MirrorEntry e = tab[k];
  out[i] = e.mul * in[r * ld + e.src] + e.add;
}
__global__ void actor_head_lpf_kernel(const float* __restrict__ out, const float* __restrict__ obs, float* __restrict__ lpf,
                                      const float* __restrict__ joint_bias, float alpha, int N, int ld_obs) {
  int i = blockIdx.x * blockDim.x + threadIdx.x;
  if (i >= N * KBJ_NU) return;
  int n = i / KBJ_NU, j = i % KBJ_NU;
  float mean = out[n * 40 + j] + joint_bias[j] + (j >= 10 ? obs[(size_t)n * ld_obs + KBJ_OBS_CMD + 6 + (j - 10)] : 0.0f);
  float y0 = lpf[i];
  lpf[i] = y0 + alpha * (mean - y0);
}
__global__ void mirror_loss_kernel(const float* __restrict__ y, const float* __restrict__ ym, const float* __restrict__ v, const float* __restrict__ vm,
                                   float sa, float sc, int R, float* __restrict__ dy, float* __restrict__ dym, float* __restrict__ dvalue,
                                   float* __restrict__ dvalue_m, double* __restrict__ macc, int part) {
  int r = blockIdx.x * blockDim.x + threadIdx.x;
  if (r >= R) return;
  float ca = sa / (20.0f * R), la = 0;
  if (part & 1) for (int i = 0; i < KBJ_NU; ++i) {
    int s = i < 5 ? i + 5 : (i < 10 ? i - 5 : i);
    float e = y[(size_t)r * KBJ_NU + i] + ym[(size_t)r * KBJ_NU + s];
    la += e * e;
    dy[(size_t)r * KBJ_NU + i] = 2 * ca * e;
    dym[(size_t)r * KBJ_NU + s] = 2 * ca * e;
  }
  if (part & 1) atomicAdd(&macc[5], (double)(sa * la / 20.0f));
  if (part & 2) {
    float ev = v[r] - vm[r];
    float gv = 2 * sc / R * ev;
    dvalue[r] += gv;
    dvalue_m[r] = -gv;
    atomicAdd(&macc[6], (double)(sc * ev * ev));
  }
}

__global__ void actor_head_bwd_pre_kernel(const float* __restrict__ out, const float* __restrict__ y, const float* __restrict__ sd,
                                          const float* __restrict__ act, const float* __restrict__ dlogp, const float* __restrict__ dy_extra, float dent,
                                          HeadParams hp, int R, float* __restrict__ dout) {
  size_t i = (size_t)blockIdx.x * blockDim.x + threadIdx.x;
  if (i >= (size_t)R * KBJ_NU) return;
  size_t r = i / KBJ_NU;
  int j = (int)(i - r * KBJ_NU);
  float s = sd[i], z = (act[i] - y[i]) / s;
  float gl = dlogp[r];
  dout[r * 40 + j] = gl * (z / s) + (dy_extra ? dy_extra[i] : 0.0f);
  float gs = gl * ((z * z - 1.0f) / s) + dent / s;
  float raw = out[r * 40 + KBJ_NU + j];
  float pre = (softplusf_(raw) + hp.min_std) * hp.var_scale;
  dout[r * 40 + KBJ_NU + j] = pre < hp.max_std ? gs * hp.var_scale * sigmoidf_(raw) : 0.0f;
}
__global__ void actor_head_train_bwd_kernel(const float* __restrict__ keep, HeadParams hp, int T, int B, float* __restrict__ dout) {
  int i = blockIdx.x * blockDim.x + threadIdx.x;
  if (i >= B * KBJ_NU) return;
  int b = i / KBJ_NU, j = i % KBJ_NU;
  float gcarry = 0;
  constexpr int U = 10;
  for (int t1 = T - 1; t1 >= 0; t1 -= U) {
    float gdir[U], kp[U];
#pragma unroll
    for (int u = 0; u < U; ++u) {
      int t = t1 - u;
      if (t >= 0) { size_t r = (size_t)t * B + b; gdir[u] = dout[r * 40 + j]; kp[u] = keep[r]; }
    }
#pragma unroll
    for (int u = 0; u < U; ++u) {
      int t = t1 - u;
      if (t >= 0) {
        float gy = gdir[u] + kp[u] * gcarry;
        dout[((size_t)t * B + b) * 40 + j] = hp.alpha * gy;
        gcarry = (1 - hp.alpha) * gy;
      }
    }
  }
}

__global__ void matvec_kernel(const float* __restrict__ W, const float* __restrict__ x, const float* __restrict__ add, int M, int K, float* __restrict__ y) {
  int m = blockIdx.x * 4 + (threadIdx.x >> 6), l = threadIdx.x & 63;
  if (m >= M) return;
  float s = 0;
  for (int k = l; k < K; k += 64) s += W[(size_t)m * K + k] * x[k];
  for (int o = 32; o > 0; o >>= 1) s += __shfl_xor(s, o);
  if (l == 0) y[m] = s + (add ? add[m] : 0.0f);
}
__global__ void matvec_t_acc_kernel(const float* __restrict__ W, const float* __restrict__ x, int K, int N, float* __restrict__ y, float* __restrict__ part) {
  __shared__ float red[4][64];
  int n = blockIdx.x * 64 + (threadIdx.x & 63), ph = threadIdx.x >> 6;
  float s = 0;
  if (n < N) for (int k = ph + 4 * blockIdx.y; k < K; k += 4 * gridDim.y) s += W[(size_t)k * N + n] * x[k];
  red[ph][threadIdx.x & 63] = s;
  __syncthreads();
  if (ph == 0 && n < N) {
    const float v = red[0][threadIdx.x] + red[1][threadIdx.x] + red[2][threadIdx.x] + red[3][threadIdx.x];
    if (part) part[(size_t)blockIdx.y * N + n] = v; else atomicAdd(&y[n], v);
  }
}

__global__ void repitch_rows_kernel(const float* __restrict__ src, int rows, int cols, int ld_dst, float* __restrict__ dst) {
  const int i = blockIdx.x * blockDim.x + threadIdx.x;
  if (i >= rows * ld_dst) return;
  const int r = i / ld_dst, c = i - r * ld_dst;
  dst[i] = c < cols ? src[(size_t)r * cols + c] : 0.0f;
}

__global__ void outer_acc_kernel(float* __restrict__ C, const float* __restrict__ u, const float* __restrict__ v, int M, int N) {
  size_t i = (size_t)blockIdx.x * blockDim.x + threadIdx.x;
  if (i >= (size_t)M * N) return;
  C[i] += u[i / N] * v[i % N];
}

constexpr int RR_ROWS = 64;
__global__ __launch_bounds__(256) void reduce_rows_kernel(const float* __restrict__ part, int nparts, int n, float* __restrict__ out) {
  __shared__ float tile[RR_ROWS][64];
  const int cl = threadIdx.x & 63, ph = threadIdx.x >> 6, c = blockIdx.x * 64 + cl;
  if (nparts <= 0) return;
  const int cc = c < n ? c : n - 1;
  float v[RR_ROWS / 4];
  auto fetch = [&](int p0) {
#pragma unroll
    for (int i = 0; i < RR_ROWS / 4; ++i) { const int p = p0 + ph + 4 * i; v[i] = part[(size_t)(p < nparts ? p : nparts - 1) * n + cc]; }
  };
  fetch(0);
  const float o0 = out[cc];
  float s = 0.0f;
  for (int p0 = 0; p0 < nparts; p0 += RR_ROWS) {
#pragma unroll
    for (int i = 0; i < RR_ROWS / 4; ++i) tile[ph + 4 * i][cl] = v[i];
    __syncthreads();
    if (p0 + RR_ROWS < nparts) fetch(p0 + RR_ROWS);
    if (ph == 0) {
      const int m = nparts - p0 < RR_ROWS ? nparts - p0 : RR_ROWS;
      int r = 0;
      for (; r + 8 <= m; r += 8) {
        float x[8];
#pragma unroll
        for (int i = 0; i < 8; ++i) x[i] = tile[r + i][cl];
#pragma unroll
        for (int i = 0; i < 8; ++i) s += x[i];
      }
      for (; r < m; ++r) s += tile[r][cl];
    }
    __syncthreads();
  }
  if (ph == 0 && c < n) out[c] = o0 + s;
}
inline void reduce_rows_launch(hipStream_t s, const float* part, int nparts, int n, float* out) {
  hipLaunchKernelGGL(reduce_rows_kernel, dim3((unsigned)((n + 63) / 64)), dim3(256), 0, s, part, nparts, n, out);
}
__global__ void colsum_kernel(const float* __restrict__ X, int M, int N, int ld, float* __restrict__ out, float* __restrict__ part) {
  __shared__ float red[4][64];
  int c = blockIdx.x * 64 + (threadIdx.x & 63), ph = threadIdx.x >> 6;
  float s = 0;
  if (c < N) for (int m = ph + 4 * blockIdx.y; m < M; m += 4 * gridDim.y) s += X[(size_t)m * ld + c];
  red[ph][threadIdx.x & 63] = s;
  __syncthreads();
  if (ph == 0 && c < N) {
    const float v = red[0][threadIdx.x] + red[1][threadIdx.x] + red[2][threadIdx.x] + red[3][threadIdx.x];
    if (part) part[(size_t)blockIdx.y * N + c] = v; else atomicAdd(&out[c], v);
  }
}

__global__ void gae_kernel(const float* __restrict__ value, const float* __restrict__ reward, const float* __restrict__ aux, int T, int N,
                           float gamma, float lam, float* __restrict__ adv, float* __restrict__ target) {
  int n = blockIdx.x * blockDim.x + threadIdx.x;
  if (n >= N) return;
  float last = 0;
  for (int t = T - 1; t >= 0; --t) {
    size_t r = (size_t)t * N + n;
    float keep = aux[r * KBJ_AUX_SIZE + KBJ_AUX_DONE] != 0 ? 0.0f : 1.0f;
    float v = value[r], vn = t + 1 < T ? value[r + N] : v;
    float delta = reward[r] + gamma * vn * keep - v;
    last = delta + gamma * lam * keep * last;
    adv[r] = last; target[r] = last + v;
  }
}
__global__ void gae_boundary_kernel(const float* __restrict__ value, const float* __restrict__ reward, const float* __restrict__ aux,
                                    const float* __restrict__ value_tail, int T, int N, float gamma, float lam, int boot_trunc,
                                    float* __restrict__ adv, float* __restrict__ target) {
  int n = blockIdx.x * blockDim.x + threadIdx.x;
  if (n >= N) return;
  float last = 0;
  for (int t = T - 1; t >= 0; --t) {
    size_t r = (size_t)t * N + n;
    const float d = aux[r * KBJ_AUX_SIZE + KBJ_AUX_DONE];
    const float v = value[r];
    if (d != 0) {
      last = (d > 0 && boot_trunc) ? reward[r] + gamma * v - v : reward[r] - v;
    } else if (t + 1 < T) {
      last = reward[r] + gamma * value[r + N] - v + gamma * lam * last;
    } else {
      const float vn = value_tail ? value_tail[n] : v;
      last = reward[r] + gamma * vn - v;
    }
    adv[r] = last; target[r] = last + v;
  }
}

__global__ void sumsq_kernel(const float* __restrict__ g, size_t n, float scale, double* __restrict__ out, double* __restrict__ part) {
  __shared__ double red[256];
  double s = 0;
  for (size_t i = (size_t)blockIdx.x * 256 + threadIdx.x; i < n; i += (size_t)gridDim.x * 256) { double v = (double)g[i] * scale; s += v * v; }
  red[threadIdx.x] = s;
  __syncthreads();
  for (int o = 128; o > 0; o >>= 1) { if (threadIdx.x < o) red[threadIdx.x] += red[threadIdx.x + o]; __syncthreads(); }
  if (threadIdx.x == 0) { if (part) part[blockIdx.x] = red[0]; else atomicAdd(out, red[0]); }
}
struct AdamParams { float lr, b1, b2, eps, wd, max_norm, bc1, bc2, gscale; };
__global__ void lane_tail_kernel(unsigned* __restrict__ counters, int lane, const unsigned* __restrict__ err, float* __restrict__ g0, float* __restrict__ g1) {
  const int net = blockIdx.x & 3;
  if (blockIdx.x == 0 && threadIdx.x == 0 && err[0]) { g0[0] = __int_as_float(0x7FC00000); if (g1) g1[0] = __int_as_float(0x7FC00000); }
  if (lane >= 0 && (net & 1) != lane) return;
  counters[(size_t)blockIdx.x * blockDim.x + threadIdx.x] = 0u;
}
__global__ void poison_vars_kernel(const unsigned* __restrict__ err, float* __restrict__ logp, float* __restrict__ value) {
  if (err[0]) { logp[0] = __int_as_float(0x7FC00000); value[0] = __int_as_float(0x7FC00000); }
}
__global__ void adamw_kernel(float* __restrict__ p, float* __restrict__ m, float* __restrict__ v, const float* __restrict__ g, size_t n,
                             const double* __restrict__ sumsq, AdamParams ap, unsigned* __restrict__ err) {
  size_t i = (size_t)blockIdx.x * blockDim.x + threadIdx.x;
  if (i >= n) return;
  const double ss = *sumsq;
  if (!(ss <= 1.0e300) || err[0]) {
    if (i == 0) err[1] = 1u;
    return;
  }
  float norm = (float)sqrt(ss);
  float clip = fminf(ap.max_norm / (norm + 1e-6f), 1.0f);
  float gi = g[i] * ap.gscale * clip;
  float mi = ap.b1 * m[i] + (1 - ap.b1) * gi, vi = ap.b2 * v[i] + (1 - ap.b2) * gi * gi;
  m[i] = mi; v[i] = vi;
  float mh = mi / ap.bc1, vh = vi / ap.bc2;
  p[i] -= ap.lr * (mh / (sqrtf(vh) + ap.eps) + ap.wd * p[i]);
}

struct PadDesc { unsigned long long uoff, ioff; int nblk, rows_u, rows_i, cols_u, cols_i; };

__global__ void pad_params_kernel(const PadDesc* __restrict__ desc, int nd, float* user, float* internal, size_t n_internal, int to_user) {
  const size_t i = (size_t)blockIdx.x * blockDim.x + threadIdx.x;
  if (i >= n_internal) return;
  int d = 0;
  while (d + 1 < nd && desc[d + 1].ioff <= i) ++d;
  const PadDesc t = desc[d];
  const size_t local = i - t.ioff;
  const int c = (int)(local % t.cols_i), r = (int)((local / t.cols_i) % t.rows_i), b = (int)(local / ((size_t)t.cols_i * t.rows_i));
  const bool real = r < t.rows_u && c < t.cols_u;
  const size_t u = t.uoff + ((size_t)b * t.rows_u + r) * t.cols_u + c;
  if (to_user) { if (real) user[u] = internal[i]; }
  else internal[i] = real ? user[u] : 0.0f;
}

__global__ void repitch_pad_kernel(const float* __restrict__ src, float* __restrict__ dst, size_t rows, int ws, int wd) {
  const size_t i = (size_t)blockIdx.x * blockDim.x + threadIdx.x;
  if (i >= rows * wd) return;
  const size_t r = i / wd; const int c = (int)(i % wd);
  dst[i] = c < ws ? src[r * ws + c] : 0.0f;
}

__global__ void init_uniform_kernel(float* __restrict__ p, size_t n, float bound, uint32_t seed, uint32_t leaf) {
  size_t i = (size_t)blockIdx.x * blockDim.x + threadIdx.x;
  if (i >= n) return;
  uint32_t b0, b1;
  nn_threefry(seed ^ ((uint32_t)KBJ_RNG_INIT * 0x9E3779B9u), leaf, (uint32_t)(i >> 32), (uint32_t)i, b0, b1);
  float u = (float)(b0 >> 8) * (1.0f / 16777216.0f);
  p[i] = fmaf(2 * bound, u, -bound);
}

}
```

Measured before the change: 2.342 million env-steps/s.

## Fold deterministic partial-sum reductions into producer kernels via last-block-arrives counters

In deterministic mode, reductions such as colsum, matvec bias fold, the LSTM backward bias gradient, adv stats and the grad sumsq each wrote partial sums and then needed a separate reduce kernel launch. Now each producing kernel stores its partials with agent-scope stores, increments a per-group atomic counter, and the last arriving block does the fixed-order combine in place. This removes many small serial reduce launches per optimizer step while keeping the summation order fixed. In exchange it adds counter workspaces, extra LDS staging in the producer kernels (which may lower occupancy), and a tail of serial work inside the last block.

```diff
diff --git a/kbot-joystick_amd/csrc/kbj_ctx.h b/kbot-joystick_amd/csrc/kbj_ctx.h
--- a/kbot-joystick_amd/csrc/kbj_ctx.h
+++ b/kbot-joystick_amd/csrc/kbj_ctx.h
@@ -25,6 +25,7 @@
   bool one_stream = false;
   bool debug_sync = false;
   bool deterministic = false;
+  bool det_combine = true;
   bool bwd16 = true;
   bool critic_on_caller = true;
   bool gemm_x3 = false;
diff --git a/kbot-joystick_amd/csrc/kbj_lstm_bwd16.h b/kbot-joystick_amd/csrc/kbj_lstm_bwd16.h
--- a/kbot-joystick_amd/csrc/kbj_lstm_bwd16.h
+++ b/kbot-joystick_amd/csrc/kbj_lstm_bwd16.h
@@ -1,5 +1,6 @@
 #pragma once
 #include "kbj_lstm_seq.h"
+#include "kbj_nn_kernels.h"
 
 namespace kbj {
 
@@ -155,8 +156,18 @@
       const int k = tid / UNITS, u = tid % UNITS;
       float s = 0;
       for (int r = 0; r < ROWS; ++r) s += cbuf[0][r * LDC + tid];
-      if (a.db_part) a.db_part[(size_t)rg * 4 * H + k * H + u0 + u] = s;
+      if (a.db_part) seq_store(a.db_part + (size_t)rg * 4 * H + k * H + u0 + u, s);
       else atomicAdd(a.db + k * H + u0 + u, s);
+    }
+    if (a.db_part && a.db_counters) {
+      const int nrg = (B + ROWS - 1) / ROWS;
+      if (det_arrive_last(a.db_counters + ug, (unsigned)nrg, &flag)) {
+        static_assert(2 * ROWS * LDC >= 2 * RR_ROWS * 64 && NTH == 512, "two 64 x 64 staging tiles in the chunk buffers, one per half of the workgroup");
+        const int half = tid >> 8;
+        float (*tile)[64] = reinterpret_cast<float (*)[64]>(&cbuf[0][0]) + half * RR_ROWS;
+#pragma unroll 1
+        for (int pass = 0; pass < 2; ++pass) det_combine_rows64<true>(a.db_part, nrg, 4 * H, (2 * pass + half) * H + u0, a.db, tile, tid & 255);
+      }
     }
   }
 }
diff --git a/kbot-joystick_amd/csrc/kbj_lstm_seq.h b/kbot-joystick_amd/csrc/kbj_lstm_seq.h
--- a/kbot-joystick_amd/csrc/kbj_lstm_seq.h
+++ b/kbot-joystick_amd/csrc/kbj_lstm_seq.h
@@ -54,6 +54,7 @@
   int T, B;
   float* db;
   float* db_part = nullptr;
+  unsigned* db_counters = nullptr;
   unsigned timeout_ticks = SEQ_TIMEOUT_MS * 100000u;
   long long* stamps = nullptr;
 };
diff --git a/kbot-joystick_amd/csrc/kbj_nn.hip b/kbot-joystick_amd/csrc/kbj_nn.hip
--- a/kbot-joystick_amd/csrc/kbj_nn.hip
+++ b/kbot-joystick_amd/csrc/kbj_nn.hip
@@ -45,6 +45,8 @@
   size_t skws_cap[4] = {0, 0, 0, 0};
   float* detp[4] = {nullptr, nullptr, nullptr, nullptr};
   double* detd = nullptr;
+  unsigned* detc[4] = {nullptr, nullptr, nullptr, nullptr};
+  unsigned* detc_d = nullptr;
   float *rX[4] = {nullptr, nullptr, nullptr, nullptr}, *rG[4] = {nullptr, nullptr, nullptr, nullptr}, *rOut[4] = {nullptr, nullptr, nullptr, nullptr};
   float* joint_bias_d = nullptr;
   bool mirror = false;
@@ -179,6 +181,10 @@
   NnWs& w = *ws_of(ctx);
   return w.sched.deterministic ? w.detp[lane_of(ctx, s)] : nullptr;
 }
+unsigned* det_counters(kbj_ctx* ctx, hipStream_t s) {
+  NnWs& w = *ws_of(ctx);
+  return w.sched.deterministic && w.sched.det_combine ? w.detc[lane_of(ctx, s)] : nullptr;
+}
 
 inline dim3 g1(size_t n, int bs = 256) { return dim3((unsigned)((n + bs - 1) / bs)); }
 
@@ -222,15 +228,19 @@
 }
 void colsum_acc(kbj_ctx* ctx, hipStream_t s, const float* X, int M, int N, int ld, float* out) {
   float* part = det_partials(ctx, s);
-  hipLaunchKernelGGL(colsum_kernel, dim3((N + 63) / 64, DETP_ROWS), dim3(256), 0, s, X, M, N, ld, out, part);
-  if (part) reduce_rows_launch(s, part, DETP_ROWS, N, out);
+  unsigned* cnt = det_counters(ctx, s);
+  hipLaunchKernelGGL(colsum_kernel, dim3((N + 63) / 64, DETP_ROWS), dim3(256), 0, s, X, M, N, ld, out, part, cnt);
+  if (part && !cnt) reduce_rows_launch(s, part, DETP_ROWS, N, out);
 }
 
 constexpr int SEQ_UW = 2;
 constexpr int SEQ_FUSED_MAX_H = 256;
 constexpr int SEQ_MAX_H = 512;
 constexpr int SEQ_COUNTER_WORDS = 256;
-constexpr int SEQ_COUNTER_TOTAL = 2 * MAXD * 4 * SEQ_COUNTER_WORDS;
+constexpr int SEQ_COUNTER_BLOCKS = (2 * MAXD + 1) * 4;
+constexpr int SEQ_COUNTER_TOTAL = SEQ_COUNTER_BLOCKS * SEQ_COUNTER_WORDS;
+constexpr int SEQ_DB_GROUPS = SEQ_FUSED_MAX_H / 64;
+static_assert(MAXD * SEQ_DB_GROUPS <= SEQ_COUNTER_WORDS, "the bias-combine counters of a net fit one counter block");
 
 template <int HC = 64, class F> bool dispatch_hidden(int H, F&& f) {
   if constexpr (HC > SEQ_MAX_H) return false;
@@ -380,6 +390,7 @@
   sc.fused_critic_head = flag("KBJ_FUSED_CRITIC_HEAD", true); sc.rollout_step = flag("KBJ_ROLLOUT_STEP", true);
   sc.one_stream = flag("KBJ_ONE_STREAM", false); sc.debug_sync = flag("KBJ_DEBUG", false);
   sc.deterministic = c.deterministic != 0 || flag("KBJ_DETERMINISTIC", false);
+  sc.det_combine = flag("KBJ_DET_COMBINE", true);
   { const char* cl = getenv("KBJ_CRITIC_LANE"); sc.critic_on_caller = !(cl && std::string(cl) == "2nd"); }
   sc.bwd16 = flag("KBJ_BWD16", true) && !wide;
   sc.gemm_x3 = (c.gemm_bf16x3 != 0 || flag("KBJ_GEMM_X3", false)) && !sc.deterministic;
@@ -500,7 +511,13 @@
 int nn_deterministic_workspaces(kbj_ctx* ctx, NnWs* w) {
   if (!w->sched.deterministic) return 0;
   for (int l = 0; l < 4; ++l) if (dalloc(ctx, *w, &w->detp[l], (size_t)DETP_ROWS * DETP_COLS)) return -1;
-  return dalloc(ctx, *w, &w->detd, 2 * 512);
+  if (dalloc(ctx, *w, &w->detd, 2 * 512)) return -1;
+  constexpr int groups = DETP_COLS / 64;
+  if (dalloc(ctx, *w, &w->detc[0], 4 * groups + 2)) return -1;
+  if (hipMemset(w->detc[0], 0, (4 * groups + 2) * sizeof(unsigned)) != hipSuccess) return kbj_fail(ctx, "hipMemset detc");
+  for (int l = 1; l < 4; ++l) w->detc[l] = w->detc[0] + l * groups;
+  w->detc_d = w->detc[0] + 4 * groups;
+  return 0;
 }
 
 int nn_residency_check(kbj_ctx* ctx, NnWs* w) {
@@ -977,8 +994,9 @@
         KBJ_HIP(ctx, hipMemcpyAsync(w.stats, w.ext_adv_sums, 2 * sizeof(double), hipMemcpyDeviceToDevice, sm));
         KBJ_HIP(ctx, hipMemcpyAsync(w.stats + 11, w.ext_adv_sums + 2, sizeof(double), hipMemcpyDeviceToDevice, sm));
       } else {
-        hipLaunchKernelGGL(adv_stats_kernel, dim3(32), dim3(256), 0, sm, w.adv, R, w.stats, sc.deterministic ? w.detd : (double*)nullptr);
-        if (sc.deterministic) reduce_double_launch(sm, w.detd, 32, 2, w.stats);
+        unsigned* cnt = sc.deterministic && sc.det_combine ? w.detc_d : nullptr;
+        hipLaunchKernelGGL(adv_stats_kernel, dim3(32), dim3(256), 0, sm, w.adv, R, w.stats, sc.deterministic ? w.detd : (double*)nullptr, cnt);
+        if (sc.deterministic && !cnt) reduce_double_launch(sm, w.detd, 32, 2, w.stats);
       }
       KBJ_HIP(ctx, hipMemsetAsync(grad_d, 0, w.nparams * sizeof(float), sm));
       if (sc.fold_actor)
@@ -1146,8 +1164,9 @@
   auto fold_bias_terms = [&](int k, hipStream_t st) {
     const NetOff& oa = w.net[k];
     float* part = det_partials(ctx, st);
-    hipLaunchKernelGGL(matvec_t_acc_kernel, dim3((H + 63) / 64, 16), dim3(256), 0, st, params_d + oa.w_ih[0], grad_d + oa.b[0], 4 * H, H, grad_d + oa.b_in, part);
-    if (part) reduce_rows_launch(st, part, 16, H, grad_d + oa.b_in);
+    unsigned* cnt = det_counters(ctx, st);
+    hipLaunchKernelGGL(matvec_t_acc_kernel, dim3((H + 63) / 64, 16), dim3(256), 0, st, params_d + oa.w_ih[0], grad_d + oa.b[0], 4 * H, H, grad_d + oa.b_in, part, cnt);
+    if (part && !cnt) reduce_rows_launch(st, part, 16, H, grad_d + oa.b_in);
     hipLaunchKernelGGL(outer_acc_kernel, g1((size_t)4 * H * H), dim3(256), 0, st, grad_d + oa.w_ih[0], grad_d + oa.b[0], params_d + oa.b_in, 4 * H, H);
   };
   bool bias_done[2] = {false, false};
@@ -1166,8 +1185,9 @@
       ba.db_part = det_partials(ctx, ns[n & 1]);
       if (w.seq_bstamps && bstamp_sel == 1 + n + 2 * l) ba.stamps = w.seq_bstamps;
       const bool tiles16 = sc.bwd16;
+      if (ba.db_part && sc.det_combine && tiles16) ba.db_counters = w.seq_counters + SEQ_COUNTER_WORDS * (4 * 2 * MAXD + n) + l * SEQ_DB_GROUPS;
       if (seq_bwd(ctx, ns[n & 1], H, ba, tiles16)) return -1;
-      if (ba.db_part) reduce_rows_launch(ns[n & 1], ba.db_part, seq_bwd_row_groups(B, tiles16), 4 * H, grad_d + o.b[l]);
+      if (ba.db_part && !ba.db_counters) reduce_rows_launch(ns[n & 1], ba.db_part, seq_bwd_row_groups(B, tiles16), 4 * H, grad_d + o.b[l]);
     }
     const bool tail_on_own_lane = l == 0 && !w.mirror && fold_actor;
     for (const PendingDW& p : pending_dw) {
@@ -1233,13 +1253,13 @@
   hipLaunchKernelGGL(ppo_metrics_kernel, dim3(1), dim3(1), 0, ns[0], w.stats + 2, w.stats, pp, R, metrics_d);
   if (one_stream) {
     if (fold_actor && fold_critic && !bias_done[1]) fold_bias_terms(1, ns[1]);
-    hipLaunchKernelGGL(lane_tail_kernel, dim3(2 * MAXD * 4), dim3(SEQ_COUNTER_WORDS), 0, ctx->stream, w.seq_counters, -1, w.seq_err, grad_d, grad_d + w.nactor);
+    hipLaunchKernelGGL(lane_tail_kernel, dim3(SEQ_COUNTER_BLOCKS), dim3(SEQ_COUNTER_WORDS), 0, ctx->stream, w.seq_counters, -1, w.seq_err, grad_d, grad_d + w.nactor);
     KBJ_HIP(ctx, hipEventRecord(ctx->ev_actor_grad, ctx->stream));
   } else {
-    hipLaunchKernelGGL(lane_tail_kernel, dim3(2 * MAXD * 4), dim3(SEQ_COUNTER_WORDS), 0, ns[0], w.seq_counters, 0, w.seq_err, grad_d, (float*)nullptr);
+    hipLaunchKernelGGL(lane_tail_kernel, dim3(SEQ_COUNTER_BLOCKS), dim3(SEQ_COUNTER_WORDS), 0, ns[0], w.seq_counters, 0, w.seq_err, grad_d, (float*)nullptr);
     KBJ_HIP(ctx, hipEventRecord(ctx->ev_actor_grad, ns[0]));
     if (fold_actor && fold_critic && !bias_done[1]) fold_bias_terms(1, ns[1]);
-    hipLaunchKernelGGL(lane_tail_kernel, dim3(2 * MAXD * 4), dim3(SEQ_COUNTER_WORDS), 0, ns[1], w.seq_counters, 1, w.seq_err, grad_d + w.nactor, (float*)nullptr);
+    hipLaunchKernelGGL(lane_tail_kernel, dim3(SEQ_COUNTER_BLOCKS), dim3(SEQ_COUNTER_WORDS), 0, ns[1], w.seq_counters, 1, w.seq_err, grad_d + w.nactor, (float*)nullptr);
     KBJ_HIP(ctx, hipEventRecord(ctx->ev_join, ctx->stream2));
     KBJ_HIP(ctx, hipStreamWaitEvent(ctx->stream, ctx->ev_join, 0));
   }
@@ -1344,8 +1364,9 @@
   if (!w.sumsq_clean) KBJ_HIP(ctx, hipMemsetAsync(sumsq, 0, sizeof(double), s));
   w.sumsq_clean = false;
   double* part = w.sched.deterministic ? w.detd : nullptr;
-  hipLaunchKernelGGL(sumsq_kernel, dim3(512), dim3(256), 0, s, grad_d, w.user.nparams, grad_scale, sumsq, part);
-  if (part) reduce_double_launch(s, part, 512, 1, sumsq);
+  unsigned* cnt = part && w.sched.det_combine ? w.detc_d + 1 : nullptr;
+  hipLaunchKernelGGL(sumsq_kernel, dim3(512), dim3(256), 0, s, grad_d, w.user.nparams, grad_scale, sumsq, part, cnt);
+  if (part && !cnt) reduce_double_launch(s, part, 512, 1, sumsq);
   AdamParams ap{c.learning_rate, c.adam_b1, c.adam_b2, c.adam_eps, c.weight_decay, c.max_grad_norm,
                 (float)(1.0 - std::pow((double)c.adam_b1, (double)step)), (float)(1.0 - std::pow((double)c.adam_b2, (double)step)), grad_scale};
   hipLaunchKernelGGL(adamw_kernel, g1(w.user.nparams), dim3(256), 0, s, params_d, m_d, v_d, grad_d, w.user.nparams, sumsq, ap, w.seq_err);
diff --git a/kbot-joystick_amd/csrc/kbj_nn_kernels.h b/kbot-joystick_amd/csrc/kbj_nn_kernels.h
--- a/kbot-joystick_amd/csrc/kbj_nn_kernels.h
+++ b/kbot-joystick_amd/csrc/kbj_nn_kernels.h
@@ -2,6 +2,7 @@
 #include <hip/hip_runtime.h>
 #include <stdint.h>
 #include "kbj_model.h"
+#include "kbj_lstm_seq.h"
 
 namespace kbj {
 
@@ -237,21 +238,68 @@
   logp[r] = lp; ent[r] = en;
 }
 
-__global__ void adv_stats_kernel(const float* __restrict__ adv, int R, double* __restrict__ stats, double* __restrict__ part) {
-  __shared__ double s1[256], s2[256];
-  double a = 0, b = 0;
-  for (int i = blockIdx.x * 256 + threadIdx.x; i < R; i += 256 * gridDim.x) { double v = adv[i]; a += v; b += v * v; }
-  s1[threadIdx.x] = a; s2[threadIdx.x] = b;
-  __syncthreads();
-  for (int o = 128; o > 0; o >>= 1) { if (threadIdx.x < o) { s1[threadIdx.x] += s1[threadIdx.x + o]; s2[threadIdx.x] += s2[threadIdx.x + o]; } __syncthreads(); }
+template <bool SC1, class T> __device__ __forceinline__ T det_load(const T* p) {
+  if constexpr (SC1) return __hip_atomic_load(p, __ATOMIC_RELAXED, __HIP_MEMORY_SCOPE_AGENT);
+  else return *p;
+}
+__device__ __forceinline__ void det_store(float* p, float v) { seq_store(p, v); }
+__device__ __forceinline__ void det_store(double* p, double v) { __hip_atomic_store(p, v, __ATOMIC_RELAXED, __HIP_MEMORY_SCOPE_AGENT); }
+__device__ __forceinline__ bool det_arrive_last(unsigned* counter, unsigned n, int* lds_flag) {
+  asm volatile("s_waitcnt vmcnt(0)" ::: "memory");
+  __syncthreads();
   if (threadIdx.x == 0) {
-    if (part) { part[2 * blockIdx.x] = s1[0]; part[2 * blockIdx.x + 1] = s2[0]; }
-    else { atomicAdd(&stats[0], s1[0]); atomicAdd(&stats[1], s2[0]); }
-  }
+    const bool last = __hip_atomic_fetch_add(counter, 1u, __ATOMIC_RELAXED, __HIP_MEMORY_SCOPE_AGENT) == n - 1;
+    if (last) __hip_atomic_store(counter, 0u, __ATOMIC_RELAXED, __HIP_MEMORY_SCOPE_AGENT);
+    *lds_flag = last;
+  }
+  __syncthreads();
+  return *lds_flag != 0;
+}
+constexpr int RR_ROWS = 64;
+template <bool SC1>
+__device__ __forceinline__ void det_combine_rows64(const float* __restrict__ part, int nparts, int n, int c0, float* __restrict__ out, float (*tile)[64], int t) {
+  const int cl = t & 63, ph = t >> 6, c = c0 + cl;
+  if (nparts <= 0) return;
+  const int cc = c < n ? c : n - 1;
+  float v[RR_ROWS / 4];
+  auto fetch = [&](int p0) {
+#pragma unroll
+    for (int i = 0; i < RR_ROWS / 4; ++i) { const int p = p0 + ph + 4 * i; v[i] = det_load<SC1>(part + (size_t)(p < nparts ? p : nparts - 1) * n + cc); }
+  };
+  fetch(0);
+  const float o0 = out[cc];
+  float s = 0.0f;
+  for (int p0 = 0; p0 < nparts; p0 += RR_ROWS) {
+#pragma unroll
+    for (int i = 0; i < RR_ROWS / 4; ++i) tile[ph + 4 * i][cl] = v[i];
+    __syncthreads();
+    if (p0 + RR_ROWS < nparts) fetch(p0 + RR_ROWS);
+    if (ph == 0) {
+      const int m = nparts - p0 < RR_ROWS ? nparts - p0 : RR_ROWS;
+      int r = 0;
+      for (; r + 8 <= m; r += 8) {
+        float x[8];
+#pragma unroll
+        for (int i = 0; i < 8; ++i) x[i] = tile[r + i][cl];
+#pragma unroll
+        for (int i = 0; i < 8; ++i) s += x[i];
+      }
+      for (; r < m; ++r) s += tile[r][cl];
+    }
+    __syncthreads();
+  }
+  if (ph == 0 && c < n) out[c] = o0 + s;
+}
+__global__ __launch_bounds__(256) void reduce_rows_kernel(const float* __restrict__ part, int nparts, int n, float* __restrict__ out) {
+  __shared__ float tile[RR_ROWS][64];
+  det_combine_rows64<false>(part, nparts, n, blockIdx.x * 64, out, tile, threadIdx.x);
+}
+inline void reduce_rows_launch(hipStream_t s, const float* part, int nparts, int n, float* out) {
+  hipLaunchKernelGGL(reduce_rows_kernel, dim3((unsigned)((n + 63) / 64)), dim3(256), 0, s, part, nparts, n, out);
 }
 constexpr int RD_CHUNK = 1024;
-__global__ __launch_bounds__(256) void reduce_double_kernel(const double* __restrict__ part, int nblocks, int w, double* __restrict__ out) {
-  __shared__ double stage[RD_CHUNK];
+template <bool SC1>
+__device__ __forceinline__ void det_combine_double(const double* __restrict__ part, int nblocks, int w, double* __restrict__ out, double* stage) {
   const int tid = threadIdx.x;
   if (nblocks <= 0) return;
   const int rows = RD_CHUNK / w;
@@ -260,7 +308,7 @@
   auto fetch = [&](int b0) {
     const size_t base = (size_t)b0 * w;
 #pragma unroll
-    for (int i = 0; i < RD_CHUNK / 256; ++i) { const size_t e = base + tid + 256 * i; v[i] = part[e < total ? e : total - 1]; }
+    for (int i = 0; i < RD_CHUNK / 256; ++i) { const size_t e = base + tid + 256 * i; v[i] = det_load<SC1>(part + (e < total ? e : total - 1)); }
   };
   fetch(0);
   const double o0 = tid < w ? out[tid] : 0.0;
@@ -286,8 +334,28 @@
   }
   if (tid < w) out[tid] = o0 + s;
 }
+__global__ __launch_bounds__(256) void reduce_double_kernel(const double* __restrict__ part, int nblocks, int w, double* __restrict__ out) {
+  __shared__ double stage[RD_CHUNK];
+  det_combine_double<false>(part, nblocks, w, out, stage);
+}
 inline void reduce_double_launch(hipStream_t s, const double* part, int nblocks, int w, double* out) {
   hipLaunchKernelGGL(reduce_double_kernel, dim3(1), dim3(256), 0, s, part, nblocks, w, out);
+}
+
+__global__ void adv_stats_kernel(const float* __restrict__ adv, int R, double* __restrict__ stats, double* __restrict__ part, unsigned* __restrict__ counter = nullptr) {
+  __shared__ double s1[256], s2[256];
+  __shared__ double stage[RD_CHUNK];
+  __shared__ int last;
+  double a = 0, b = 0;
+  for (int i = blockIdx.x * 256 + threadIdx.x; i < R; i += 256 * gridDim.x) { double v = adv[i]; a += v; b += v * v; }
+  s1[threadIdx.x] = a; s2[threadIdx.x] = b;
+  __syncthreads();
+  for (int o = 128; o > 0; o >>= 1) { if (threadIdx.x < o) { s1[threadIdx.x] += s1[threadIdx.x + o]; s2[threadIdx.x] += s2[threadIdx.x + o]; } __syncthreads(); }
+  if (threadIdx.x == 0) {
+    if (part) { det_store(part + 2 * blockIdx.x, s1[0]); det_store(part + 2 * blockIdx.x + 1, s2[0]); }
+    else { atomicAdd(&stats[0], s1[0]); atomicAdd(&stats[1], s2[0]); }
+  }
+  if (part && counter && det_arrive_last(counter, gridDim.x, &last)) det_combine_double<true>(part, (int)gridDim.x, 2, stats, stage);
 }
 struct PpoParams { float clip, vclip, vcoef, ecoef, lrclip, adv_eps; };
 __global__ void ppo_loss_kernel(const float* __restrict__ logp, const float* __restrict__ value, const float* __restrict__ ent,
@@ -463,8 +531,11 @@
   for (int o = 32; o > 0; o >>= 1) s += __shfl_xor(s, o);
   if (l == 0) y[m] = s + (add ? add[m] : 0.0f);
 }
-__global__ void matvec_t_acc_kernel(const float* __restrict__ W, const float* __restrict__ x, int K, int N, float* __restrict__ y, float* __restrict__ part) {
+__global__ void matvec_t_acc_kernel(const float* __restrict__ W, const float* __restrict__ x, int K, int N, float* __restrict__ y, float* __restrict__ part,
+                                                           unsigned* __restrict__ counters = nullptr) {
   __shared__ float red[4][64];
+  __shared__ float tile[RR_ROWS][64];
+  __shared__ int last;
   int n = blockIdx.x * 64 + (threadIdx.x & 63), ph = threadIdx.x >> 6;
   float s = 0;
   if (n < N) for (int k = ph + 4 * blockIdx.y; k < K; k += 4 * gridDim.y) s += W[(size_t)k * N + n] * x[k];
@@ -472,8 +543,9 @@
   __syncthreads();
   if (ph == 0 && n < N) {
     const float v = red[0][threadIdx.x] + red[1][threadIdx.x] + red[2][threadIdx.x] + red[3][threadIdx.x];
-    if (part) part[(size_t)blockIdx.y * N + n] = v; else atomicAdd(&y[n], v);
-  }
+    if (part) det_store(part + (size_t)blockIdx.y * N + n, v); else atomicAdd(&y[n], v);
+  }
+  if (part && counters && det_arrive_last(counters + blockIdx.x, gridDim.y, &last)) det_combine_rows64<true>(part, (int)gridDim.y, N, blockIdx.x * 64, y, tile, threadIdx.x);
 }
 
 __global__ void repitch_rows_kernel(const float* __restrict__ src, int rows, int cols, int ld_dst, float* __restrict__ dst) {
@@ -489,46 +561,10 @@
   C[i] += u[i / N] * v[i % N];
 }
 
-constexpr int RR_ROWS = 64;
-__global__ __launch_bounds__(256) void reduce_rows_kernel(const float* __restrict__ part, int nparts, int n, float* __restrict__ out) {
+__global__ void colsum_kernel(const float* __restrict__ X, int M, int N, int ld, float* __restrict__ out, float* __restrict__ part, unsigned* __restrict__ counters = nullptr) {
+  __shared__ float red[4][64];
   __shared__ float tile[RR_ROWS][64];
-  const int cl = threadIdx.x & 63, ph = threadIdx.x >> 6, c = blockIdx.x * 64 + cl;
-  if (nparts <= 0) return;
-  const int cc = c < n ? c : n - 1;
-  float v[RR_ROWS / 4];
-  auto fetch = [&](int p0) {
-#pragma unroll
-    for (int i = 0; i < RR_ROWS / 4; ++i) { const int p = p0 + ph + 4 * i; v[i] = part[(size_t)(p < nparts ? p : nparts - 1) * n + cc]; }
-  };
-  fetch(0);
-  const float o0 = out[cc];
-  float s = 0.0f;
-  for (int p0 = 0; p0 < nparts; p0 += RR_ROWS) {
-#pragma unroll
-    for (int i = 0; i < RR_ROWS / 4; ++i) tile[ph + 4 * i][cl] = v[i];
-    __syncthreads();
-    if (p0 + RR_ROWS < nparts) fetch(p0 + RR_ROWS);
-    if (ph == 0) {
-      const int m = nparts - p0 < RR_ROWS ? nparts - p0 : RR_ROWS;
-      int r = 0;
-      for (; r + 8 <= m; r += 8) {
-        float x[8];
-#pragma unroll
-        for (int i = 0; i < 8; ++i) x[i] = tile[r + i][cl];
-#pragma unroll
-        for (int i = 0; i < 8; ++i) s += x[i];
-      }
-      for (; r < m; ++r) s += tile[r][cl];
-    }
-    __syncthreads();
-  }
-  if (ph == 0 && c < n) out[c] = o0 + s;
-}
-inline void reduce_rows_launch(hipStream_t s, const float* part, int nparts, int n, float* out) {
-  hipLaunchKernelGGL(reduce_rows_kernel, dim3((unsigned)((n + 63) / 64)), dim3(256), 0, s, part, nparts, n, out);
-}
-__global__ void colsum_kernel(const float* __restrict__ X, int M, int N, int ld, float* __restrict__ out, float* __restrict__ part) {
-  __shared__ float red[4][64];
+  __shared__ int last;
   int c = blockIdx.x * 64 + (threadIdx.x & 63), ph = threadIdx.x >> 6;
   float s = 0;
   if (c < N) for (int m = ph + 4 * blockIdx.y; m < M; m += 4 * gridDim.y) s += X[(size_t)m * ld + c];
@@ -536,8 +572,9 @@
   __syncthreads();
   if (ph == 0 && c < N) {
     const float v = red[0][threadIdx.x] + red[1][threadIdx.x] + red[2][threadIdx.x] + red[3][threadIdx.x];
-    if (part) part[(size_t)blockIdx.y * N + c] = v; else atomicAdd(&out[c], v);
-  }
+    if (part) det_store(part + (size_t)blockIdx.y * N + c, v); else atomicAdd(&out[c], v);
+  }
+  if (part && counters && det_arrive_last(counters + blockIdx.x, gridDim.y, &last)) det_combine_rows64<true>(part, (int)gridDim.y, N, blockIdx.x * 64, out, tile, threadIdx.x);
 }
 
 __global__ void gae_kernel(const float* __restrict__ value, const float* __restrict__ reward, const float* __restrict__ aux, int T, int N,
@@ -576,14 +613,17 @@
   }
 }
 
-__global__ void sumsq_kernel(const float* __restrict__ g, size_t n, float scale, double* __restrict__ out, double* __restrict__ part) {
+__global__ void sumsq_kernel(const float* __restrict__ g, size_t n, float scale, double* __restrict__ out, double* __restrict__ part, unsigned* __restrict__ counter = nullptr) {
   __shared__ double red[256];
+  __shared__ double stage[RD_CHUNK];
+  __shared__ int last;
   double s = 0;
   for (size_t i = (size_t)blockIdx.x * 256 + threadIdx.x; i < n; i += (size_t)gridDim.x * 256) { double v = (double)g[i] * scale; s += v * v; }
   red[threadIdx.x] = s;
   __syncthreads();
   for (int o = 128; o > 0; o >>= 1) { if (threadIdx.x < o) red[threadIdx.x] += red[threadIdx.x + o]; __syncthreads(); }
-  if (threadIdx.x == 0) { if (part) part[blockIdx.x] = red[0]; else atomicAdd(out, red[0]); }
+  if (threadIdx.x == 0) { if (part) det_store(part + blockIdx.x, red[0]); else atomicAdd(out, red[0]); }
+  if (part && counter && det_arrive_last(counter, gridDim.x, &last)) det_combine_double<true>(part, (int)gridDim.x, 1, out, stage);
 }
 struct AdamParams { float lr, b1, b2, eps, wd, max_norm, bc1, bc2, gscale; };
 __global__ void lane_tail_kernel(unsigned* __restrict__ counters, int lane, const unsigned* __restrict__ err, float* __restrict__ g0, float* __restrict__ g1) {
```

New measurement: 2.344 million env-steps/s, median of 2. About the same (+0.1%).
